# LimpBunion22/VIT-FPGA

Measured on AMD Instinct MI355X. Metric: images/sec ViT-B/16 224x224, batch 512 per GPU, higher is better.
Workload: dtype bf16; 1 GPU; vit_base 224x224x3 inference, 512 images per GPU resident in HBM, random-init weights (seed 0); global_batch=512, per_gpu_batch=512

## Files before the change

### include/vithip.h

```cpp
#ifndef VITHIP_H
#define VITHIP_H

#include <stddef.h>
#include <stdint.h>

#ifdef __cplusplus
extern "C" {
#endif

#define VH_ABI_VERSION 1

#define VH_OK 0
#define VH_ERR_INVALID 1
#define VH_ERR_HIP 2
#define VH_ERR_STATE 3
#define VH_ERR_UNSUPPORTED 4
#define VH_ERR_NO_DEVICE 5
#define VH_ERR_RING_FULL 6
#define VH_ERR_RING_EMPTY 7

#define VH_DTYPE_BF16 0
#define VH_DTYPE_FP16 1
#define VH_DTYPE_FP8 2

// ... 158 lines not shown
#define VH_444_BGR VH_444(2, 1, 0, 0, 0)
#define VH_444_RGBA VH_444(0, 1, 2, 1, 0)
#define VH_444_BGRA VH_444(2, 1, 0, 1, 0)
#define VH_444_ARGB VH_444(1, 2, 3, 1, 0)
#define VH_444_ABGR VH_444(3, 2, 1, 1, 0)
#define VH_444_YUV24 VH_444(0, 1, 2, 0, 1)
#define VH_444_VUYA VH_444(2, 1, 0, 1, 1)
#define VH_444_AYUV VH_444(1, 2, 3, 1, 1)
#define VH_444_Y416 VH_444(1, 0, 2, 1, 1)
#define VH_444_AYUV64 VH_444(1, 2, 3, 1, 1)
#define VH_444_Y410 (VH_444(1, 0, 2, 1, 1) | 256)
#define VH_444_V410 (VH_444(1, 0, 2, 1, 1) | 256 | 512)
typedef struct vh_frame_bgra {
    uint64_t offset;
    int32_t height, width, row_stride;
    int32_t layout;
    float box[4];
} vh_frame_bgra;
int vh_forward_frames_bgra(vh_ctx* ctx, const uint8_t* frames_host, size_t nbytes, const vh_frame_bgra* desc, int batch, float* logits_host);
int vh_forward_device_frames_bgra(vh_ctx* ctx, const uint8_t* frames_dev, size_t nbytes, const vh_frame_bgra* desc, int batch, float* logits_dev);
int vh_forward_frames_y410(vh_ctx* ctx, const uint8_t* frames_host, size_t nbytes, const vh_frame_bgra* desc, int batch, float* logits_host);
int vh_forward_device_frames_y410(vh_ctx* ctx, const uint8_t* frames_dev, size_t nbytes, const vh_frame_bgra* desc, int batch, float* logits_dev);
int vh_fill_input_seeded(vh_ctx* ctx, uint64_t seed, int batch, float* in_nhwc_dev);

int vh_ring_create(vh_ctx* ctx, int slots, int batch_per_slot);
int vh_ring_destroy(vh_ctx* ctx);
int vh_ring_free_slots(const vh_ctx* ctx, int* n);
int vh_ring_input(vh_ctx* ctx, float** pinned_in_nhwc);
int vh_ring_submit(vh_ctx* ctx, const float* in_nhwc_host, int batch);
int vh_ring_collect(vh_ctx* ctx, float* logits_host, int* batch);
int vh_ring_create_u8(vh_ctx* ctx, int slots, int batch_per_slot);
int vh_ring_input_u8(vh_ctx* ctx, uint8_t** pinned_in_nhwc);
int vh_ring_submit_u8(vh_ctx* ctx, const uint8_t* in_nhwc_host, int batch);
int vh_ring_create_frames(vh_ctx* ctx, int slots, int batch_per_slot, size_t slot_bytes);
int vh_ring_input_frames(vh_ctx* ctx, uint8_t** pinned, size_t* capacity);
int vh_ring_submit_frames(vh_ctx* ctx, const uint8_t* frames_host, size_t nbytes, const vh_frame* desc, int batch);
int vh_ring_submit_frames_nv12(vh_ctx* ctx, const uint8_t* frames_host, size_t nbytes, const vh_frame_nv12* desc, int batch);
int vh_ring_submit_frames_yuv(vh_ctx* ctx, const uint8_t* frames_host, size_t nbytes, const vh_frame_yuv* desc, int batch);
int vh_ring_submit_frames_p016(vh_ctx* ctx, const uint8_t* frames_host, size_t nbytes, const vh_frame_nv12* desc, int batch);
int vh_ring_submit_frames_yuv16(vh_ctx* ctx, const uint8_t* frames_host, size_t nbytes, const vh_frame_yuv* desc, int batch);
int vh_ring_submit_frames_yuy2(vh_ctx* ctx, const uint8_t* frames_host, size_t nbytes, const vh_frame_yuy2* desc, int batch);
int vh_ring_submit_frames_y210(vh_ctx* ctx, const uint8_t* frames_host, size_t nbytes, const vh_frame_yuy2* desc, int batch);
int vh_ring_submit_frames_bgra(vh_ctx* ctx, const uint8_t* frames_host, size_t nbytes, const vh_frame_bgra* desc, int batch);
int vh_ring_submit_frames_y410(vh_ctx* ctx, const uint8_t* frames_host, size_t nbytes, const vh_frame_bgra* desc, int batch);
int vh_ring_create_tensor(vh_ctx* ctx, int slots, int batch_per_slot, int elem, int layout);
int vh_ring_input_tensor(vh_ctx* ctx, void** pinned, size_t* capacity_bytes);
int vh_ring_submit_tensor(vh_ctx* ctx, const void* in_host, int batch);

int vh_set_graph(vh_ctx* ctx, int enable);
int vh_get_graph(const vh_ctx* ctx, int* enabled, int* cached_graphs);

int vh_set_streams(vh_ctx* ctx, int n);
int vh_get_streams(const vh_ctx* ctx, int* n);

int vh_last_forward_us(const vh_ctx* ctx, int64_t* us);
int vh_last_kernel_ms(vh_ctx* ctx, double* ms);
int vh_profile_forward(vh_ctx* ctx, const float* in_nhwc_dev, int batch, float* logits_dev,
                       double* stage_ms, int n_stage_slots, int* n_stages_written);
const char* vh_stage_name(int stage_index);
int vh_set_stage_timing(vh_ctx* ctx, int stage_index);
int vh_get_stage_timing(vh_ctx* ctx, double* avg_ms, double* min_ms, int* launches);
int vh_set_step_timing(vh_ctx* ctx, int enable);
int vh_get_step_timing(vh_ctx* ctx, double* step_ms, int max_steps, int* steps);

int vh_debug_read(vh_ctx* ctx, int what, float* host_out, size_t n_floats);
int vh_debug_set_layers(vh_ctx* ctx, int n_layers);

#define VH_FEAT_NORM 0
#define VH_FEAT_RAW  1
typedef struct vh_features {
    void* cls;
    void* patch;
    void* mean;
    int32_t elem;
    int32_t norm;
} vh_features;
int vh_features_dims(const vh_ctx* ctx, int* batch, int* tokens, int* patches, int* dim);
int vh_read_features(vh_ctx* ctx, const vh_features* out_host);
int vh_read_features_device(vh_ctx* ctx, const vh_features* out_dev);
int vh_read_features_device_async(vh_ctx* ctx, const vh_features* out_dev);

#define VH_MAX_FEATURE_LAYERS 8
#define VH_FEAT_ROWS 0
#define VH_FEAT_NCHW 1
typedef struct vh_layer_features {
    void* cls;
    void* patch;
    void* mean;
    void* reg;
    int32_t elem;
    int32_t norm;
    int32_t layer;
    int32_t patch_layout;
} vh_layer_features;
int vh_set_feature_layers(vh_ctx* ctx, const int* layers, int n);
int vh_get_feature_layers(const vh_ctx* ctx, int* layers, int* n);
int vh_read_layer_features(vh_ctx* ctx, const vh_layer_features* out_host);
int vh_read_layer_features_device(vh_ctx* ctx, const vh_layer_features* out_dev);
int vh_read_layer_features_device_async(vh_ctx* ctx, const vh_layer_features* out_dev);

#define VH_MAX_ATTENTION_LAYERS 64
#define VH_ATTN_Q_CLS 0
#define VH_ATTN_Q_LEAD 1
#define VH_ATTN_KEYS_ALL 0
#define VH_ATTN_KEYS_PATCH 1
typedef struct vh_attention_maps {
// ... 191 lines not shown
```

### vit-fpga_amd/csrc/vithip_api.hip

```cpp
#include <dlfcn.h>

#include <chrono>
#include <cmath>
#include <condition_variable>
#include <cstdarg>
#include <cstdio>
#include <cstdlib>
#include <cstring>
#include <functional>
#include <memory>
#include <mutex>
#include <string>
#include <thread>
#include <vector>

#include "vh_kernels.h"

using namespace vh;

namespace {

thread_local std::string g_err;

int fail(std::string* ctx_err, int code, const char* fmt, ...) {
// ... 124 lines not shown
    if (c.max_batch <= 0) return "max_batch must be positive";
    if (!(c.ln_eps > 0.f)) return "ln_eps must be positive";
    if (c.flags & ~(VH_FLAG_LN_FOLD_OFF | VH_FLAG_LN_FOLD_ON | VH_FLAG_W8_E4M3 | VH_FLAG_CLS_TAIL | VH_FLAG_PRE_LN | VH_FLAG_QUICK_GELU | VH_FLAG_REGISTERS_MASK |
                    VH_FLAG_NO_CLS | VH_FLAG_POOL_MASK | VH_FLAG_MAP_HEAD | VH_FLAG_TANH_GELU | VH_FLAG_ROPE)) return "unknown bits in flags";
    if ((c.flags & VH_FLAG_ROPE) && (c.flags & VH_FLAG_CLS_TAIL)) return "flags: VH_FLAG_ROPE excludes VH_FLAG_CLS_TAIL (the tail's one-query attention kernel reads unrotated q and k)";
    if ((c.flags & VH_FLAG_TANH_GELU) && (c.flags & VH_FLAG_QUICK_GELU)) return "flags: VH_FLAG_TANH_GELU and VH_FLAG_QUICK_GELU exclude each other (one MLP activation)";
    if (c.flags & VH_FLAG_MAP_HEAD) {
        if (!(c.flags & VH_FLAG_NO_CLS)) return "flags: VH_FLAG_MAP_HEAD needs VH_FLAG_NO_CLS (the head pools the patch rows; its towers have no class token)";
        if (VH_FLAG_POOL_OF(c.flags)) return "flags: VH_FLAG_MAP_HEAD excludes VH_FLAG_POOL (the attention pooling is the head's input)";
        if (VH_FLAG_REGISTERS_OF(c.flags)) return "flags: VH_FLAG_MAP_HEAD excludes VH_FLAG_REGISTERS";
        if (c.flags & VH_FLAG_CLS_TAIL) return "flags: VH_FLAG_MAP_HEAD excludes VH_FLAG_CLS_TAIL (there is no class token)";
        if (c.heads > VH_MAP_MAX_HEADS) return "flags: VH_FLAG_MAP_HEAD takes at most 16 heads";
    }
    const int R = VH_FLAG_REGISTERS_OF(c.flags);
    if (R > VH_MAX_REGISTERS) return "flags: VH_FLAG_REGISTERS takes 0 .. 16 register tokens";
    const int ncls = (c.flags & VH_FLAG_NO_CLS) ? 0 : 1, pool = VH_FLAG_POOL_OF(c.flags);
    if (!ncls && !(c.flags & VH_FLAG_MAP_HEAD) && (pool == VH_POOL_CLS || pool == VH_POOL_CLS_AVG))
        return pool == VH_POOL_CLS ? "flags: VH_FLAG_NO_CLS needs VH_FLAG_POOL(VH_POOL_AVG_NORM) or VH_FLAG_POOL(VH_POOL_AVG_FCNORM): VH_POOL_CLS reads the class token"
                                   : "flags: VH_FLAG_NO_CLS excludes VH_POOL_CLS_AVG: its first half is the class token";
    if ((c.flags & VH_FLAG_CLS_TAIL) && !ncls) return "flags: VH_FLAG_CLS_TAIL excludes VH_FLAG_NO_CLS (its last layer computes the class-token rows only)";
    if ((c.flags & VH_FLAG_CLS_TAIL) && pool != VH_POOL_CLS) return "flags: VH_FLAG_CLS_TAIL excludes VH_FLAG_POOL (its last layer does not update the patch rows)";
    if ((c.flags & VH_FLAG_W8_E4M3) && c.dtype == VH_DTYPE_FP8) return "flags: VH_FLAG_W8_E4M3 is for the 16-bit dtypes (VH_DTYPE_FP8 quantises both operands)";
    if ((c.flags & VH_FLAG_W8_E4M3) && (c.dim % 4 || c.mlp_dim % 4)) return "flags: VH_FLAG_W8_E4M3 needs dim and mlp_dim multiples of 4";
    if ((c.flags & VH_FLAG_LN_FOLD_OFF) && (c.flags & VH_FLAG_LN_FOLD_ON)) return "flags: VH_FLAG_LN_FOLD_OFF and VH_FLAG_LN_FOLD_ON exclude each other";
    if (c.image_size > 4096 || c.patch_size > 256 || c.channels > 64) return "image_size <= 4096, patch_size <= 256, channels <= 64";
    if (c.layers > 4096 || c.classes > (1 << 20) || c.mlp_dim > (1 << 16) || c.max_batch > (1 << 20)) return "layers <= 4096, classes <= 2^20, mlp_dim <= 2^16, max_batch <= 2^20";
    const int g = c.image_size / c.patch_size;
    if (g > 64) return "tokens <= 4097 (image_size / patch_size <= 64)";
    if (g * g + ncls + R > 4097)
        return ncls ? "tokens <= 4097: a 64 x 64 patch grid + the class token leaves no room for register tokens"
                    : "tokens <= 4097: a 64 x 64 patch grid without a class token leaves room for one register token";
    if ((int64_t)c.max_batch * (g * g + ncls + R) > (640ll << 20)) return "max_batch x tokens <= 640 x 2^20";
    return nullptr;
}

enum Stage { ST_IM2COL, ST_PATCH, ST_CLS, ST_LN, ST_QKV, ST_ATTN, ST_PROJ, ST_FC1, ST_FC2, ST_LNF, ST_HEAD, ST_LNSTATS, ST_PRELN, ST_RESIZE, ST_COUNT };
constexpr int kProfiledStages = ST_RESIZE;
const char* kStageNames[ST_COUNT] = {"im2col", "patch_gemm", "cls_rows", "layernorm", "qkv_gemm", "attention",
                                     "proj_gemm", "fc1_gemm", "fc2_gemm", "final_layernorm", "head_gemm", "ln_stats", "pre_layernorm", "resize"};

}

struct ImgIn {
    const void* p;
    int kind = VH_ELEM_F32;
    int layout = VH_LAYOUT_NHWC;
    bool u8() const { return kind == VH_ELEM_U8; }
    bool nhwc_f32() const { return kind == VH_ELEM_F32 && layout == VH_LAYOUT_NHWC; }
    size_t elem() const { return kind == VH_ELEM_F32 ? 4 : kind == VH_ELEM_U8 ? 1 : 2; }
    ImgIn skip(size_t elements) const { return ImgIn{(const char*)p + elements * elem(), kind, layout}; }
    bool operator==(const ImgIn& o) const { return p == o.p && kind == o.kind && layout == o.layout; }
};
constexpr int kU8 = VH_ELEM_U8;

struct vh_ctx {
    vh_config cfg;
    int device;
    Layout L;
    hipStream_t stream = nullptr;
    static constexpr int kMaxStreams = 4;
    hipStream_t xstream[kMaxStreams - 1] = {nullptr, nullptr, nullptr};
    hipEvent_t ev_fork = nullptr, ev_join[kMaxStreams - 1] = {nullptr, nullptr, nullptr};
    int nstreams = 1;
    hipEvent_t ev0 = nullptr, ev1 = nullptr;
    bool weights_ready = false;
    int run_layers = -1;
    char* blob = nullptr;
    float* params = nullptr;
    char* w16 = nullptr;
    void* wp16 = nullptr;
    std::vector<void*> wqkv16, wo16, w1_16, w2_16;
    std::vector<void*> w2t_16, wot_16;
    bool h_tiled = false;
    bool att_tiled = true;
    bool qkv_hm = true;
    bool weights_ready_tiled = false;
    float* bqkv = nullptr;
    bool fp8 = false;
    int dt16 = VH_DTYPE_BF16;
    std::vector<float*> sqkv, so, s1, s2;
    bool ln_fold = false;
    float* fold_cd = nullptr;
    float* stats = nullptr;
    float* partials = nullptr;
    bool split = false;
    bool cls_tail = false;
    int head_dim = 64;
    float q_scale = kAttnQScale;
    void* xlo16 = nullptr;
    bool ln_fold_cfg = false, split_cfg = false;
    unsigned int* guard_dev = nullptr;
    float* guard_host = nullptr;
    float guard_thresh = 0.5f;
    bool guard_auto = false, guard_tripped = false;
    char* arena = nullptr;
    unsigned int* tickets = nullptr;
    float* x = nullptr;
    void* xn16 = nullptr;
    void* qkv16 = nullptr;
    void* att16 = nullptr;
    void* h16 = nullptr;
    void* col16 = nullptr;
    float* clsn32 = nullptr;
    float* pool32 = nullptr;
    float* mapz32 = nullptr;
    float* maph32 = nullptr;
    float* mapa32 = nullptr;
    float* in_dev = nullptr;
    float in_scale[kMaxChannels], in_shift[kMaxChannels];
    float* logits_dev = nullptr;
    uint8_t* rz_u8 = nullptr;
    uint32_t *rz_plan_dev = nullptr, *rz_plan_host = nullptr;
    size_t rz_plan_dev_cap = 0, rz_plan_host_cap = 0;
    uint8_t* rz_frames = nullptr;
    size_t rz_frames_cap = 0;
    std::vector<uint32_t> rz_words;
    struct FrameColour { float m[12]; int site = VH_CHROMA_LEFT; };
    FrameColour colour[2];
    int64_t last_us = 0;
    bool timed = false;
    int last_batch = 0;
    int feat_layers[VH_MAX_FEATURE_LAYERS] = {0}, feat_n = 0;
    char* feat_store = nullptr;
    size_t feat_slot = 0;
    int cap_layers[VH_MAX_FEATURE_LAYERS] = {0}, cap_n = 0, cap_nl = -1, cap_form = VH_FEAT_FORM_F32;
    int attn_layers[VH_MAX_ATTENTION_LAYERS] = {0}, attn_n = 0, attn_q = 0, attn_mode = VH_ATTN_Q_CLS;
    char* attn_store = nullptr;
    size_t attn_slot = 0;
    int acap_layers[VH_MAX_ATTENTION_LAYERS] = {0}, acap_n = 0, acap_nl = -1;
    struct RingSlot {
        float *h_in = nullptr, *h_out = nullptr, *d_in = nullptr, *d_out = nullptr;
        hipEvent_t in_done = nullptr, fwd_done = nullptr, out_done = nullptr;
        int batch = 0;
        uint32_t* h_plan = nullptr;
        size_t plan_cap = 0;
    };
    std::vector<RingSlot> ring;
    enum RingKind { RING_F32, RING_U8, RING_FRAMES, RING_TENSOR };
    RingKind ring_kind = RING_F32;
    int ring_elem = VH_ELEM_F32, ring_layout = VH_LAYOUT_NHWC;
    size_t ring_slot_bytes = 0;
    hipStream_t copy_in = nullptr, copy_out = nullptr;
    int ring_batch = 0, ring_wr = 0, ring_rd = 0, ring_used = 0;
    bool last_h_tiled = false;
    bool last_qkv_hm = false;
    int num_cu = 256;
    bool use_graph = false;
    struct GraphEntry { ImgIn in; float* out; int batch; hipGraph_t graph; hipGraphExec_t exec; };
    std::vector<GraphEntry> graphs;
    std::vector<int> graph_warm;
    int timing_stage = -1;
    std::vector<hipEvent_t> tev;
    size_t tev_used = 0;
    bool step_timing = false;
    std::vector<hipEvent_t> sev;
    size_t sev_used = 0;
    std::string err;
};

struct vh_filter {
// ... 65 lines not shown
        const size_t dd = (size_t)D * D;
        HIPCHK(&c->err, launch_quantize_rows(P + o.qw, D, D, c->q_scale, wq, c->sqkv[l], s));
        HIPCHK(&c->err, launch_quantize_rows(P + o.kw, D, D, 1.0f, wq + dd, c->sqkv[l] + D, s));
        HIPCHK(&c->err, launch_quantize_rows(P + o.vw, D, D, 1.0f, wq + 2 * dd, c->sqkv[l] + 2 * D, s));
        HIPCHK(&c->err, launch_quantize_rows(P + o.ow, D, D, 1.0f, c->wo16[l], c->so[l], s));
        HIPCHK(&c->err, launch_quantize_rows(P + o.f1w, M, D, 1.0f, c->w1_16[l], c->s1[l], s));
        HIPCHK(&c->err, launch_quantize_rows(P + o.f2w, D, M, 1.0f, c->w2_16[l], c->s2[l], s));
    }
    float* w8tmp = nullptr;
    struct FreeOnExit { float*& p; ~FreeOnExit() { if (p) { hipFree(p); p = nullptr; } } } w8tmp_guard{w8tmp};
    const size_t dd1 = (size_t)D * D, md1 = (size_t)M * D;
    if (!c->fp8 && (f.flags & VH_FLAG_W8_E4M3)) { HIPCHK(&c->err, hipMalloc((void**)&w8tmp, (4 * dd1 + 2 * md1) * sizeof(float))); }
    for (int l = 0; l < f.layers && !c->fp8; ++l) {
        LayerOff o = L.layer[l];
        const float* P = c->params;
        if (w8tmp) {
            const size_t src[6] = {o.qw, o.kw, o.vw, o.ow, o.f1w, o.f2w};
            const int rows[6] = {D, D, D, D, M, D}, cols[6] = {D, D, D, D, D, M};
            size_t at = 0;
            for (int i = 0; i < 6; ++i) {
                HIPCHK(&c->err, launch_fake_quant_rows(c->params + src[i], rows[i], cols[i], w8tmp + at, s));
                at += (size_t)rows[i] * cols[i];
            }
            P = w8tmp;
            o.qw = 0; o.kw = dd1; o.vw = 2 * dd1; o.ow = 3 * dd1; o.f1w = 4 * dd1; o.f2w = 4 * dd1 + md1;
        }
        const float* B = c->params;
        if (c->ln_fold) {
            float* cd = c->fold_cd + (size_t)l * (6 * D + 2 * M);
            char* wq = (char*)c->wqkv16[l];
            const size_t dd2 = (size_t)D * D * 2;
            HIPCHK(&c->err, launch_fold_ln(P + o.qw, B + o.qb, B + o.ln1w, B + o.ln1b, D, D, c->q_scale, wq, cd, cd + 3 * D, f.dtype, s));
            HIPCHK(&c->err, launch_fold_ln(P + o.kw, B + o.kb, B + o.ln1w, B + o.ln1b, D, D, 1.0f, wq + dd2, cd + D, cd + 4 * D, f.dtype, s));
            HIPCHK(&c->err, launch_fold_ln(P + o.vw, B + o.vb, B + o.ln1w, B + o.ln1b, D, D, 1.0f, wq + 2 * dd2, cd + 2 * D, cd + 5 * D, f.dtype, s));
            HIPCHK(&c->err, launch_fold_ln(P + o.f1w, B + o.f1b, B + o.ln2w, B + o.ln2b, M, D, 1.0f, c->w1_16[l], cd + 6 * D, cd + 6 * D + M, f.dtype, s));
        } else {
            HIPCHK(&c->err, launch_pack_qkv(P + o.qw, B + o.qb, P + o.kw, B + o.kb, P + o.vw, B + o.vb, D, c->q_scale,
                                            c->wqkv16[l], c->bqkv + (size_t)l * 3 * D, f.dtype, s));
            HIPCHK(&c->err, launch_cast(P + o.f1w, c->w1_16[l], (int64_t)M * D, f.dtype, s));
        }
        HIPCHK(&c->err, launch_cast(P + o.ow, c->wo16[l], (int64_t)D * D, f.dtype, s));
        HIPCHK(&c->err, launch_cast(P + o.f2w, c->w2_16[l], (int64_t)D * M, f.dtype, s));
        if (c->h_tiled && c->w2t_16[l]) HIPCHK(&c->err, launch_cast_tiled_w(P + o.f2w, D, M, c->w2t_16[l], f.dtype, s));
        if (c->h_tiled && c->wot_16[l]) HIPCHK(&c->err, launch_cast_tiled_w(P + o.ow, D, D, c->wot_16[l], f.dtype, s));
        if (w8tmp) { HIPCHK(&c->err, hipStreamSynchronize(s)); }
    }
    HIPCHK(&c->err, hipStreamSynchronize(s));
    c->weights_ready = true;
    c->weights_ready_tiled = c->h_tiled && (!c->fp8 || c->ln_fold);
    return VH_OK;
}

void drop_graphs(vh_ctx* c);
int guard_reset(vh_ctx* c) {
    HIPCHK(&c->err, hipStreamSynchronize(c->stream));
    HIPCHK(&c->err, hipMemsetAsync(c->guard_dev, 0, 2 * sizeof(unsigned int), c->stream));
    c->guard_host[0] = c->guard_host[1] = 0.f;
    c->guard_tripped = false;
    c->ln_fold = c->ln_fold_cfg;
    c->split = c->split_cfg;
    drop_graphs(c);
    return VH_OK;
}

int check_blob_header(vh_ctx* c, const BlobHeader& h) {
    const vh_config& f = c->cfg;
    if (memcmp(h.magic, "VHBLOB1", 8) != 0) return fail(&c->err, VH_ERR_INVALID, "weight blob: bad magic");
    if (h.image_size != f.image_size || h.patch_size != f.patch_size || h.channels != f.channels || h.dim != f.dim ||
        h.heads != f.heads || h.mlp_dim != f.mlp_dim || h.layers != f.layers || h.classes != f.classes)
        return fail(&c->err, VH_ERR_INVALID, "weight blob: shape differs from the context's vh_config");
    const uint32_t want = blob_model_bits(f);
    if ((h.flags ^ want) & kBlobPreLn)
        return fail(&c->err, VH_ERR_INVALID, "weight blob: header bit 1 (pre-LayerNorm) is %d, the context's VH_FLAG_PRE_LN is %d",
                    (h.flags & kBlobPreLn) != 0, (want & kBlobPreLn) != 0);
    if ((h.flags ^ want) & kBlobQuickGelu)
        return fail(&c->err, VH_ERR_INVALID, "weight blob: header bit 2 (QuickGELU) is %d, the context's VH_FLAG_QUICK_GELU is %d",
                    (h.flags & kBlobQuickGelu) != 0, (want & kBlobQuickGelu) != 0);
    if ((h.flags ^ want) & kBlobRegisters)
        return fail(&c->err, VH_ERR_INVALID, "weight blob: header bits 9..13 say %d register tokens, the context's VH_FLAG_REGISTERS says %d",
                    (int)VH_FLAG_REGISTERS_OF(h.flags), (int)VH_FLAG_REGISTERS_OF(want));
    if ((h.flags ^ want) & kBlobNoCls)
        return fail(&c->err, VH_ERR_INVALID, "weight blob: header bit 15 (no class token) is %d, the context's VH_FLAG_NO_CLS is %d",
                    (h.flags & kBlobNoCls) != 0, (want & kBlobNoCls) != 0);
    if ((h.flags ^ want) & kBlobPool)
        return fail(&c->err, VH_ERR_INVALID, "weight blob: header bits 16..17 say pooling mode %d, the context's VH_FLAG_POOL says %d",
                    (int)VH_FLAG_POOL_OF(h.flags), (int)VH_FLAG_POOL_OF(want));
    if ((h.flags ^ want) & kBlobMapHead)
        return fail(&c->err, VH_ERR_INVALID, "weight blob: header bit 19 (attention-pooling head) is %d, the context's VH_FLAG_MAP_HEAD is %d",
                    (h.flags & kBlobMapHead) != 0, (want & kBlobMapHead) != 0);
    if ((h.flags ^ want) & kBlobTanhGelu)
        return fail(&c->err, VH_ERR_INVALID, "weight blob: header bit 21 (tanh GELU) is %d, the context's VH_FLAG_TANH_GELU is %d",
                    (h.flags & kBlobTanhGelu) != 0, (want & kBlobTanhGelu) != 0);
    if ((h.flags ^ want) & kBlobRope)
        return fail(&c->err, VH_ERR_INVALID, "weight blob: header bit 23 (rotary position embedding) is %d, the context's VH_FLAG_ROPE is %d",
                    (h.flags & kBlobRope) != 0, (want & kBlobRope) != 0);
    return VH_OK;
}

int enqueue_forward(vh_ctx* c, ImgIn in, int batch, float* logits, std::vector<std::pair<int, hipEvent_t>>* ev,
                    hipStream_t s, int img0, bool may_pad = true) {
    const vh_config& f = c->cfg;
    const Layout& L = c->L;
    const int D = f.dim, M = f.mlp_dim, T = L.T;
    const int64_t rows = (int64_t)batch * T;
    const int64_t row_tiles = (rows + 255) / 256;
    const int64_t rows_g = (may_pad && c->ln_fold && row_tiles * ((D + 255) / 256) >= 2 * (int64_t)c->num_cu) ? row_tiles * 256 : rows;
    const float* P = c->params;
    const size_t r0 = (size_t)img0 * T, esz = 2, esz_op = c->fp8 ? 1 : 2;
    const int dt16 = c->dt16;
    float* const x = c->x + r0 * D;
    float* const stats_p = c->stats + r0 * 2;
    float* const partials_p = c->partials + (size_t)(D / 64) * r0 * 2;
    char* const xn16 = (char*)c->xn16 + r0 * D * esz_op;
    char* const xlo16 = (char*)c->xlo16 + r0 * D * (c->fp8 ? 2 : 1);
    char* const qkv16 = (char*)c->qkv16 + r0 * 3 * D * esz;
    char* const att16 = (char*)c->att16 + r0 * D * esz_op;
    char* const h16 = (char*)c->h16 + r0 * M * esz_op;
    char* const col16 = (char*)c->col16 + (size_t)img0 * L.NP * L.KPA * esz;
    float* const clsn32 = c->clsn32 + (size_t)img0 * L.HW;
    float* const pool32 = c->pool32 + (size_t)img0 * D;
    const float* const cls_p = L.ncls ? P + L.cls : nullptr;
    const float* const pos_p = P + L.pos - (L.ncls ? 0 : D);
    unsigned int* const tickets_part = c->tickets + (size_t)img0 * (f.layers > 0 ? f.layers : 1);
    if (f.layers > 0) HIPCHK(&c->err, hipMemsetAsync(tickets_part, 0, sizeof(unsigned int) * f.layers, s));
    unsigned int* const amax_guard = c->fp8 ? c->guard_dev + 1 : nullptr;
    auto mark = [&](int stage) -> int {
        if (!ev) return VH_OK;
        hipEvent_t e;
        HIPCHK(&c->err, hipEventCreate(&e));
        HIPCHK(&c->err, hipEventRecord(e, s));
        ev->push_back({stage, e});
        return VH_OK;
    };
    auto tmark = [&](int stage) -> int {
        if (stage != c->timing_stage) return VH_OK;
        if (c->tev_used == c->tev.size()) {
            hipEvent_t e;
            HIPCHK(&c->err, hipEventCreate(&e));
            c->tev.push_back(e);
        }
        HIPCHK(&c->err, hipEventRecord(c->tev[c->tev_used++], s));
        return VH_OK;
    };
    const int op_dt = c->fp8 ? VH_DTYPE_FP8 : dt16;
    auto gemm_args = [&](int dtype, const void* a, const void* w, const float* bias, void* out, int64_t Mr, int N, int K, int epi,
                         const float* aux = nullptr, int aux_i = 0) {
        GemmArgs g{a, w, bias, out, Mr, N, K, epi, aux, aux_i, dtype, 0};
        g.stats = stats_p;
        g.partials = partials_p;
        return g;
    };
    auto set_tiled = [](GemmArgs& g, bool out_tiled, bool ab_tiled) {
        g.out_tiled = out_tiled;
        g.ab_tiled = ab_tiled;
        if (out_tiled || ab_tiled) g.variant = 6;
    };
    auto stage = [&](int st, auto&& launch) -> int {
        int r;
        if ((r = tmark(st))) return r;
        HIPCHK(&c->err, launch());
        if ((r = tmark(st))) return r;
        return mark(st);
    };
    int rc;
    if ((rc = mark(-1))) return rc;
    const int nl = (c->run_layers < 0 || c->run_layers > f.layers) ? f.layers : c->run_layers;
    const int cap_form = c->split ? (c->fp8 ? VH_DTYPE_FP8 : dt16) : VH_FEAT_FORM_F32;
    c->cap_nl = nl;
    c->cap_form = cap_form;
    c->cap_n = c->feat_n;
    for (int i = 0; i < c->cap_n; ++i) c->cap_layers[i] = c->feat_layers[i];
    auto capture = [&](int l) -> int {
        if (!c->feat_store || l + 1 >= nl) return VH_OK;
        for (int i = 0; i < c->feat_n; ++i) {
            if (c->feat_layers[i] != l + 1) continue;
            char* const slot = c->feat_store + (size_t)i * c->feat_slot;
// ... 62 lines not shown
            if ((rc = stage(ST_PRELN, [&] {
                     return launch_pre_layernorm(x, fold0 ? rows_g : rows, D, P + L.prew, P + L.preb, f.ln_eps, fold0 && c->split ? nullptr : x,
                                                 fold0 ? xn16 : nullptr, fold0 && c->split ? xlo16 : nullptr, fold0 ? stats_p : nullptr, op_dt, s,
                                                 rows, fold0 ? c->guard_dev : nullptr, fold0 ? amax_guard : nullptr);
                 })))
                return rc;
        } else if (c->ln_fold && nl > 0) {
            if (c->split) HIPCHK(&c->err, launch_rowstats_split(x, rows_g, D, f.ln_eps, xn16, xlo16, stats_p, op_dt, s, rows, amax_guard));
            else HIPCHK(&c->err, launch_rowstats_cast(x, rows_g, D, f.ln_eps, xn16, stats_p, op_dt, s, rows, amax_guard));
            HIPCHK(&c->err, launch_ln_guard(stats_p, rows, c->guard_dev, s));
            if ((rc = mark(ST_LNSTATS))) return rc;
        }
    }
    const bool hd64 = c->head_dim == 64;
    const bool tail = c->cls_tail && hd64 && c->ln_fold && c->split && !c->fp8 && nl == f.layers && c->run_layers < 0 && T <= 1024 &&
                      (size_t)L.NP * L.KPA * esz >= 2 * ((size_t)D * esz + 256);
    const bool h_tiled = c->h_tiled && c->split && c->weights_ready_tiled && gemm_tiled_applies(rows_g, M, D, op_dt) && gemm_tiled_applies(rows_g, D, M, op_dt);
    const bool att_tiled = hd64 && h_tiled && c->att_tiled && gemm_tiled_applies(rows_g, D, D, op_dt) && attention_tiled_applies(batch, T, f.heads) && !tail;
    const bool qkv_hm = c->qkv_hm && att_tiled && gemm_tiled_applies(rows_g, 3 * D, D, op_dt);
    c->last_h_tiled = h_tiled && nl > 0 && c->ln_fold;
    c->last_qkv_hm = qkv_hm && nl > 0 && c->ln_fold;
    for (int l = 0; l < nl && c->ln_fold; ++l) {
        const LayerOff& o = L.layer[l];
        const float* cd = c->fold_cd + (size_t)l * (6 * D + 2 * M);
        const int nblk = D / 64;
        const float *sq = c->fp8 ? c->sqkv[l] : nullptr, *so = c->fp8 ? c->so[l] : nullptr;
        const float *s1 = c->fp8 ? c->s1[l] : nullptr, *s2 = c->fp8 ? c->s2[l] : nullptr;
        GemmArgs gq = gemm_args(op_dt, xn16, c->wqkv16[l], cd + 3 * D, qkv16, rows_g, 3 * D, D, VH_EPI_LNFOLD, cd);
        gq.wscale = sq;
        set_tiled(gq, qkv_hm, false);
        if ((rc = stage(ST_QKV, [&] { return launch_gemm(gq, s); }))) return rc;
        if ((rc = rope(qkv_hm ? (int64_t)rows_g : 0))) return rc;
        if ((rc = capture_attention(l, qkv_hm ? (int64_t)rows_g : 0))) return rc;
        if (tail && l + 1 == nl) {
            char* const hc = col16;
            char* const lc = col16 + (((size_t)batch * D * esz + 255) & ~(size_t)255);
            HIPCHK(&c->err, launch_attention_cls(qkv16, batch, T, f.heads, att16, dt16, s));
            if ((rc = mark(ST_ATTN))) return rc;
            HIPCHK(&c->err, hipMemcpy2DAsync(hc, (size_t)D * esz, xn16, (size_t)T * D * esz, (size_t)D * esz, batch, hipMemcpyDeviceToDevice, s));
            HIPCHK(&c->err, hipMemcpy2DAsync(lc, (size_t)D, xlo16, (size_t)T * D, (size_t)D, batch, hipMemcpyDeviceToDevice, s));
            GemmArgs gp = gemm_args(op_dt, att16, c->wo16[l], P + o.ob, hc, batch, D, D, VH_EPI_RESID_SPLIT);
            gp.out16 = lc;
            HIPCHK(&c->err, launch_gemm(gp, s));
            if ((rc = mark(ST_PROJ))) return rc;
            HIPCHK(&c->err, launch_finalize_stats(partials_p, nblk, batch, D, f.ln_eps, stats_p, s, batch, c->guard_dev));
            if ((rc = mark(ST_LNSTATS))) return rc;
            const GemmArgs g1 = gemm_args(op_dt, hc, c->w1_16[l], cd + 6 * D + M, h16, batch, M, D, epi_fc1, cd + 6 * D);
            HIPCHK(&c->err, launch_gemm(g1, s));
            if ((rc = mark(ST_FC1))) return rc;
            GemmArgs g2 = gemm_args(op_dt, h16, c->w2_16[l], P + o.f2b, hc, batch, D, M, VH_EPI_RESID_SPLIT);
            g2.out16 = lc;
            HIPCHK(&c->err, launch_gemm(g2, s));
            if ((rc = mark(ST_FC2))) return rc;
            HIPCHK(&c->err, launch_layernorm_split(hc, lc, batch, D, D, P + L.lnfw, P + L.lnfb, f.ln_eps, clsn32, dt16, s));
            if ((rc = mark(ST_LNF))) return rc;
            HIPCHK(&c->err, launch_head_f32(clsn32, P + L.headw, P + L.headb, logits, batch, f.classes, D, s));
            if ((rc = mark(ST_HEAD))) return rc;
            c->last_batch = batch;
            return VH_OK;
        }
        if ((rc = stage(ST_ATTN, [&] {
                 return hd64 ? launch_attention(qkv16, batch, T, f.heads, att16, op_dt, tickets_part + l, s, true, att_tiled, qkv_hm ? (int64_t)rows_g : 0)
                             : launch_attention_hd(qkv16, batch, T, f.heads, c->head_dim, att16, op_dt, s);
             })))
            return rc;
        GemmArgs go = gemm_args(op_dt, att16, att_tiled ? c->wot_16[l] : c->wo16[l], P + o.ob, c->split ? (void*)xn16 : x, rows_g, D, D,
                                c->split ? VH_EPI_RESID_SPLIT : VH_EPI_RESID_LN);
        go.out16 = c->split ? xlo16 : xn16;
        go.wscale = so;
        set_tiled(go, false, att_tiled);
        if ((rc = stage(ST_PROJ, [&] { return launch_gemm(go, s); }))) return rc;
        HIPCHK(&c->err, launch_finalize_stats(partials_p, nblk, rows_g, D, f.ln_eps, stats_p, s, rows, c->guard_dev, amax_guard));
        if ((rc = mark(ST_LNSTATS))) return rc;
        GemmArgs g1 = gemm_args(op_dt, xn16, c->w1_16[l], cd + 6 * D + M, h16, rows_g, M, D, epi_fc1, cd + 6 * D);
        g1.wscale = s1;
        set_tiled(g1, h_tiled, false);
        if ((rc = stage(ST_FC1, [&] { return launch_gemm(g1, s); }))) return rc;
        GemmArgs g2 = gemm_args(op_dt, h16, h_tiled ? c->w2t_16[l] : c->w2_16[l], P + o.f2b, c->split ? (void*)xn16 : x, rows_g, D, M,
                                c->split ? VH_EPI_RESID_SPLIT : (l + 1 < nl ? VH_EPI_RESID_LN : VH_EPI_BIAS_RESID));
        g2.out16 = c->split ? xlo16 : xn16;
        g2.wscale = s2;
        set_tiled(g2, false, h_tiled);
        if ((rc = stage(ST_FC2, [&] { return launch_gemm(g2, s); }))) return rc;
        if ((rc = capture(l))) return rc;
        if (l + 1 < nl) {
            HIPCHK(&c->err, launch_finalize_stats(partials_p, nblk, rows_g, D, f.ln_eps, stats_p, s, rows, c->guard_dev, amax_guard));
            if ((rc = mark(ST_LNSTATS))) return rc;
        }
    }
    const bool plain = !c->ln_fold;
    auto ln_rows = [&](const float* w, const float* b) { return launch_layernorm(x, rows, D, D, w, b, f.ln_eps, xn16, op_dt, s); };
    auto resid_gemm_ln = [&](const void* a, const void* w, const float* bias, const float* scale, int K, const float* lnw,
                             const float* lnb, int st_gemm) -> int {
        GemmArgs g = gemm_args(op_dt, a, w, bias, x, rows, D, K, VH_EPI_BIAS_RESID);
        g.wscale = scale;
        if (int r = stage(st_gemm, [&] { return launch_gemm(g, s); })) return r;
        return lnw ? stage(ST_LN, [&] { return ln_rows(lnw, lnb); }) : VH_OK;
    };
    if (plain && nl > 0) {
        const LayerOff& o0 = L.layer[0];
        if ((rc = stage(ST_LN, [&] { return ln_rows(P + o0.ln1w, P + o0.ln1b); }))) return rc;
    }
    for (int l = 0; l < nl && plain; ++l) {
        const LayerOff& o = L.layer[l];
        const float *sq = c->fp8 ? c->sqkv[l] : nullptr, *so = c->fp8 ? c->so[l] : nullptr;
        const float *s1 = c->fp8 ? c->s1[l] : nullptr, *s2 = c->fp8 ? c->s2[l] : nullptr;
        GemmArgs gq = gemm_args(op_dt, xn16, c->wqkv16[l], c->bqkv + (size_t)l * 3 * D, qkv16, rows, 3 * D, D, VH_EPI_BIAS);
        gq.wscale = sq;
        if ((rc = stage(ST_QKV, [&] { return launch_gemm(gq, s); }))) return rc;
        if ((rc = rope(0))) return rc;
        if ((rc = capture_attention(l, 0))) return rc;
        if ((rc = stage(ST_ATTN, [&] {
                 return hd64 ? launch_attention(qkv16, batch, T, f.heads, att16, op_dt, tickets_part + l, s, true)
                             : launch_attention_hd(qkv16, batch, T, f.heads, c->head_dim, att16, op_dt, s);
             })))
            return rc;
        if ((rc = resid_gemm_ln(att16, c->wo16[l], P + o.ob, so, D, P + o.ln2w, P + o.ln2b, ST_PROJ))) return rc;
        GemmArgs g1 = gemm_args(op_dt, xn16, c->w1_16[l], P + o.f1b, h16, rows, M, D, epi_fc1_plain);
        g1.wscale = s1;
        if ((rc = stage(ST_FC1, [&] { return launch_gemm(g1, s); }))) return rc;
        const bool more = l + 1 < nl;
        if ((rc = resid_gemm_ln(h16, c->w2_16[l], P + o.f2b, s2, M, more ? P + L.layer[l + 1].ln1w : nullptr,
                                more ? P + L.layer[l + 1].ln1b : nullptr, ST_FC2))) return rc;
        if ((rc = capture(l))) return rc;
    }
    const bool planes = c->split && nl > 0;
    if (L.map) {
        const int H = f.heads, hd = D / H;
        float* const z = c->mapz32 + (size_t)img0 * H * D;
        float* const hid = c->maph32 + (size_t)img0 * (M > D ? M : D);
        float* const a32 = c->mapa32 + (size_t)img0 * D;
        float* const o32 = c->mapa32 + ((size_t)f.max_batch + img0) * D;
        float* const lnrow = z;
        const PoolArgs pa{planes ? (const void*)xn16 : (const void*)x, planes ? xlo16 : nullptr, planes ? (c->fp8 ? VH_DTYPE_FP8 : dt16) : VH_FEAT_FORM_F32,
                          batch, T, L.lead, D, P + L.lnfw, P + L.lnfb, f.ln_eps, VH_FEAT_NORM, z};
        HIPCHK(&c->err, launch_map_pool(pa, P + L.map_qk, H, s));
        HIPCHK(&c->err, launch_head_f32_groups(z, (int64_t)H * D, D, P + L.map_vw, P + L.map_vb, a32, D, nullptr, batch, hd, D, H, s));
        HIPCHK(&c->err, launch_head_f32(a32, P + L.map_ow, P + L.map_ob, o32, batch, D, D, s));
        HIPCHK(&c->err, launch_layernorm(o32, batch, D, D, P + L.map_lnw, P + L.map_lnb, f.ln_eps, lnrow, VH_DTYPE_F32_INTERNAL, s));
        HIPCHK(&c->err, launch_head_f32(lnrow, P + L.map_f1w, P + L.map_f1b, hid, batch, M, D, s));
        HIPCHK(&c->err, launch_act_f32(hid, (int64_t)batch * M, quick ? 1 : tanh_gelu ? 2 : 0, s));
        HIPCHK(&c->err, launch_head_f32_groups(hid, M, 0, P + L.map_f2w, P + L.map_f2b, clsn32, D, o32, batch, D, M, 1, s));
    } else if (L.pool == VH_POOL_CLS || L.pool == VH_POOL_CLS_AVG) {
        float* const cls_ln = L.pool == VH_POOL_CLS ? clsn32 : pool32;
        if (planes)
            HIPCHK(&c->err, launch_layernorm_split(xn16, xlo16, batch, D, (int64_t)T * D, P + L.lnfw, P + L.lnfb, f.ln_eps, cls_ln, c->fp8 ? VH_DTYPE_FP8 : dt16, s));
        else
            HIPCHK(&c->err, launch_layernorm(x, batch, D, (int64_t)T * D, P + L.lnfw, P + L.lnfb, f.ln_eps, cls_ln, VH_DTYPE_F32_INTERNAL, s));
    }
    if (!L.map && L.pool != VH_POOL_CLS) {
        PoolArgs pa{planes ? (const void*)xn16 : (const void*)x, planes ? xlo16 : nullptr, planes ? (c->fp8 ? VH_DTYPE_FP8 : dt16) : VH_FEAT_FORM_F32,
                    batch, T, L.lead, D, P + L.lnfw, P + L.lnfb, f.ln_eps, L.pool == VH_POOL_AVG_FCNORM ? VH_FEAT_RAW : VH_FEAT_NORM, clsn32};
        if (L.pool == VH_POOL_CLS_AVG) { pa.out = clsn32 + D; pa.out_stride = 2 * D; pa.cls_in = pool32; pa.cls_out = clsn32; }
        if (L.pool == VH_POOL_AVG_FCNORM) pa.out = pool32;
        HIPCHK(&c->err, launch_pool_rows(pa, s));
        if (L.pool == VH_POOL_AVG_FCNORM)
            HIPCHK(&c->err, launch_layernorm(pool32, batch, D, D, P + L.lnfw, P + L.lnfb, f.ln_eps, clsn32, VH_DTYPE_F32_INTERNAL, s));
    }
    if ((rc = mark(ST_LNF))) return rc;
    HIPCHK(&c->err, launch_head_f32(clsn32, P + L.headw, P + L.headb, logits, batch, f.classes, L.HW, s));
    if ((rc = mark(ST_HEAD))) return rc;
    c->last_batch = batch;
    return VH_OK;
}

int guard_publish(vh_ctx* c) {
    if (c->ln_fold) HIPCHK(&c->err, hipMemcpyAsync(c->guard_host, c->guard_dev, 2 * sizeof(float), hipMemcpyDeviceToHost, c->stream));
    return VH_OK;
}
constexpr float kE4M3Max = 448.f;
bool guard_exceeded(const vh_ctx* c) {
    if (!c->ln_fold || !c->guard_host) return false;
    const volatile float* g = c->guard_host;
    return !(g[0] <= c->guard_thresh) || (c->fp8 && !(g[1] <= kE4M3Max));
}
int prepare_weights(vh_ctx* c);
void drop_graphs(vh_ctx* c);
int guard_poll(vh_ctx* c) {
    if (!guard_exceeded(c)) return VH_OK;
    c->guard_tripped = true;
    if (!c->guard_auto) return VH_OK;
    c->ln_fold = false;
    c->split = false;
    drop_graphs(c);
    return prepare_weights(c);
}

int enqueue_step(vh_ctx* c, ImgIn in, int batch, float* logits) {
    const size_t img_elems = (size_t)c->cfg.image_size * c->cfg.image_size * c->cfg.channels;
    const int parts = batch < c->nstreams ? batch : c->nstreams;
    int rc;
    if (parts > 1) {
        HIPCHK(&c->err, hipEventRecord(c->ev_fork, c->stream));
        int b0 = 0;
        for (int p = 0; p < parts; ++p) {
            const int nb = batch / parts + (p < batch % parts ? 1 : 0);
            hipStream_t st = p == 0 ? c->stream : c->xstream[p - 1];
            if (p) HIPCHK(&c->err, hipStreamWaitEvent(st, c->ev_fork, 0));
            if ((rc = enqueue_forward(c, in.skip((size_t)b0 * img_elems), nb, logits + (size_t)b0 * c->cfg.classes, nullptr, st, b0,
                                       p == parts - 1))) return rc;
            if (p) {
                HIPCHK(&c->err, hipEventRecord(c->ev_join[p - 1], st));
                HIPCHK(&c->err, hipStreamWaitEvent(c->stream, c->ev_join[p - 1], 0));
            }
            b0 += nb;
        }
        c->last_batch = batch;
        return guard_publish(c);
    }
    if ((rc = enqueue_forward(c, in, batch, logits, nullptr, c->stream, 0))) return rc;
    return guard_publish(c);
}

void drop_graphs(vh_ctx* c) {
    for (auto& g : c->graphs) {
        if (g.exec) hipGraphExecDestroy(g.exec);
        if (g.graph) hipGraphDestroy(g.graph);
    }
    c->graphs.clear();
}

int run_step(vh_ctx* c, ImgIn in, int batch, float* logits) {
    if (int rc = guard_poll(c)) return rc;
    if (!c->use_graph || c->timing_stage >= 0) return enqueue_step(c, in, batch, logits);
    for (auto& g : c->graphs)
        if (g.in == in && g.out == logits && g.batch == batch) {
            HIPCHK(&c->err, hipGraphLaunch(g.exec, c->stream));
            c->last_batch = batch;
            return VH_OK;
        }
    bool warm = false;
    for (int b : c->graph_warm) warm |= b == batch;
    if (!warm) {
        c->graph_warm.push_back(batch);
        return enqueue_step(c, in, batch, logits);
    }
    if (c->graphs.size() >= 128) drop_graphs(c);
    vh_ctx::GraphEntry g{in, logits, batch, nullptr, nullptr};
    HIPCHK(&c->err, hipStreamBeginCapture(c->stream, hipStreamCaptureModeThreadLocal));
    const int rc = enqueue_step(c, in, batch, logits);
    const hipError_t e = hipStreamEndCapture(c->stream, &g.graph);
    if (rc) { if (g.graph) hipGraphDestroy(g.graph); return rc; }
    if (e != hipSuccess) return fail(&c->err, VH_ERR_HIP, "hipStreamEndCapture: %s", hipGetErrorString(e));
    const hipError_t ei = hipGraphInstantiate(&g.exec, g.graph, nullptr, nullptr, 0);
    if (ei != hipSuccess) { hipGraphDestroy(g.graph); return fail(&c->err, VH_ERR_HIP, "hipGraphInstantiate: %s", hipGetErrorString(ei)); }
    c->graphs.push_back(g);
    HIPCHK(&c->err, hipGraphLaunch(g.exec, c->stream));
    c->last_batch = batch;
    return VH_OK;
}

int guard_calibrate(vh_ctx* c) {
    if (!c->guard_auto || !c->ln_fold) return VH_OK;
    const vh_config& f = c->cfg;
    const int64_t n = (int64_t)f.image_size * f.image_size * f.channels;
    HIPCHK(&c->err, launch_fill(c->in_dev, n, 0xCA11B8A7Eull, TID_IMAGES, 0, 0.f, 0.f, c->stream));
    const int keep_stage = c->timing_stage;
    c->timing_stage = -1;
    const int rc = enqueue_step(c, ImgIn{c->in_dev}, 1, c->logits_dev);
    c->timing_stage = keep_stage;
    if (rc) return rc;
    HIPCHK(&c->err, hipStreamSynchronize(c->stream));
    return guard_poll(c);
}

int check_forward_args(vh_ctx* c, const void* in, int batch, const void* out) {
    if (!c) return fail(nullptr, VH_ERR_INVALID, "null context");
    if (!in || !out) return fail(&c->err, VH_ERR_INVALID, "null buffer");
    if (batch <= 0 || batch > c->cfg.max_batch)
        return fail(&c->err, VH_ERR_INVALID, "batch %d outside 1..max_batch=%d", batch, c->cfg.max_batch);
    if (!c->weights_ready) return fail(&c->err, VH_ERR_STATE, "forward before weights were loaded");
    return VH_OK;
}

int check_tensor_kind(std::string* err, int elem, int layout) {
    if (elem < VH_ELEM_F32 || elem > VH_ELEM_U8) return fail(err, VH_ERR_INVALID, "unknown elem %d (VH_ELEM_F32 .. VH_ELEM_U8 = 0..3)", elem);
    if (layout != VH_LAYOUT_NHWC && layout != VH_LAYOUT_NCHW) return fail(err, VH_ERR_INVALID, "unknown layout %d (VH_LAYOUT_NHWC = 0, VH_LAYOUT_NCHW = 1)", layout);
    return VH_OK;
}

int check_tensor_ptr(vh_ctx* c, const void* in_dev) {
    if ((uintptr_t)in_dev & 15) return fail(c ? &c->err : nullptr, VH_ERR_INVALID, "tensor device input %p is not 16-byte aligned", in_dev);
    return VH_OK;
}

int check_u8_ptr(vh_ctx* c, const void* in_dev) {
    if (c && ((uintptr_t)in_dev & 15)) return fail(&c->err, VH_ERR_INVALID, "8-bit device input %p is not 16-byte aligned", in_dev);
    return VH_OK;
}

struct FrameFormat {
    const char* tag;
    const char* label;
    const char* op_null;
    bool three_channels;
    int colour;
    const char* (*plan)(const void* desc, int batch, int channels, int S, size_t nbytes, uintptr_t base, int chroma_site,
                        std::vector<uint32_t>* words, int* max_tiles);
    hipError_t (*launch)(const uint8_t* frames, const uint32_t* plan_dev, int batch, int channels, int S, int max_tiles, const float* m12,
                         uint8_t* out, hipStream_t stream);
};

template <int SAMPLE_BYTES>
const char* plan_semi_planar(const void* desc, int batch, int, int S, size_t nbytes, uintptr_t base, int chroma_site, std::vector<uint32_t>* words,
                             int* max_tiles) {
    return resize_plan_build_nv12((const vh_frame_nv12*)desc, batch, S, nbytes, (unsigned)(base & 3), chroma_site, SAMPLE_BYTES, words, max_tiles);
}
template <int SAMPLE_BYTES>
const char* plan_planar(const void* desc, int batch, int, int S, size_t nbytes, uintptr_t base, int chroma_site, std::vector<uint32_t>* words,
                        int* max_tiles) {
    return resize_plan_build_yuv((const vh_frame_yuv*)desc, batch, S, nbytes, (base & 1) == 0, chroma_site, SAMPLE_BYTES, words, max_tiles);
}
template <bool PLANAR, bool WIDE>
hipError_t launch_yuv(const uint8_t* frames, const uint32_t* plan_dev, int batch, int, int S, int max_tiles, const float* m12, uint8_t* out,
                      hipStream_t stream) {
    return launch_resize_yuv_any(PLANAR, WIDE, frames, plan_dev, batch, S, max_tiles, m12, out, stream);
// ... 10 lines not shown
    return launch_resize_yuy2(WIDE, frames, plan_dev, batch, S, max_tiles, m12, out, stream);
}

template <int SAMPLE_BYTES>
const char* plan_packed444(const void* desc, int batch, int, int S, size_t nbytes, uintptr_t base, int, std::vector<uint32_t>* words, int* max_tiles) {
    return resize_plan_build_bgra((const vh_frame_bgra*)desc, batch, S, nbytes, (unsigned)(base & 7), SAMPLE_BYTES, words, max_tiles);
}
template <bool WIDE>
hipError_t launch_packed444(const uint8_t* frames, const uint32_t* plan_dev, int batch, int, int S, int max_tiles, const float* m12, uint8_t* out,
                            hipStream_t stream) {
    return launch_resize_bgra(WIDE, frames, plan_dev, batch, S, max_tiles, m12, out, stream);
}

const char* plan_rgb(const void* desc, int batch, int channels, int S, size_t nbytes, uintptr_t base, int, std::vector<uint32_t>* words, int* max_tiles) {
    return resize_plan_build((const vh_frame*)desc, batch, channels, S, nbytes, (base & 3) == 0, words, max_tiles);
}
hipError_t launch_rgb(const uint8_t* frames, const uint32_t* plan_dev, int batch, int channels, int S, int max_tiles, const float*, uint8_t* out,
                      hipStream_t stream) {
    return launch_resize_u8(frames, plan_dev, batch, channels, S, max_tiles, out, stream);
}

const FrameFormat kFramesRGB = {"resize_u8", "", "null buffer", false, -1, plan_rgb, launch_rgb};
const FrameFormat kFramesNV12 = {"resize_nv12", "NV12", "null buffer", true, 0, plan_semi_planar<1>, launch_yuv<false, false>};
const FrameFormat kFramesYUV = {"resize_yuv", "planar YUV", "resize_yuv: null buffer", true, 0, plan_planar<1>, launch_yuv<true, false>};
const FrameFormat kFramesP016 = {"resize_p016", "P016", "resize_p016: null buffer", true, 1, plan_semi_planar<2>, launch_yuv<false, true>};
const FrameFormat kFramesYUV16 = {"resize_yuv16", "planar 16-bit YUV", "resize_yuv16: null buffer", true, 1, plan_planar<2>, launch_yuv<true, true>};
const FrameFormat kFramesYUY2 = {"resize_yuy2", "packed 4:2:2", "resize_yuy2: null buffer", true, 0, plan_packed422<1>, launch_packed422<false>};
const FrameFormat kFramesY210 = {"resize_y210", "packed 16-bit 4:2:2", "resize_y210: null buffer", true, 1, plan_packed422<2>, launch_packed422<true>};
const FrameFormat kFramesBGRA = {"resize_bgra", "packed 4:4:4", "resize_bgra: null buffer", true, 0, plan_packed444<1>, launch_packed444<false>};
const FrameFormat kFramesY410 = {"resize_y410", "packed 16-bit 4:4:4", "resize_y410: null buffer", true, 1, plan_packed444<2>, launch_packed444<true>};

struct FrameJob {
    const FrameFormat& fmt;
    const uint8_t* frames_dev;
    const uint32_t* plan_host;
    size_t words;
    int max_tiles;
};

int frames_plan(vh_ctx* c, const FrameFormat& fmt, const void* desc, int batch, size_t nbytes, uintptr_t base, int* max_tiles) {
    if (!desc) return fail(&c->err, VH_ERR_INVALID, "null frame descriptors");
    if (fmt.three_channels && c->cfg.channels != 3)
        return fail(&c->err, VH_ERR_INVALID, "%s frames need a model with 3 channels, this one has %d", fmt.label, c->cfg.channels);
    const int site = fmt.colour < 0 ? 0 : c->colour[fmt.colour].site;
    const char* why = fmt.plan(desc, batch, c->cfg.channels, c->cfg.image_size, nbytes, base, site, &c->rz_words, max_tiles);
    if (why) return fail(&c->err, VH_ERR_INVALID, "%s", why);
    return VH_OK;
}

int frames_reserve(vh_ctx* c, size_t plan_words, bool host_too, size_t frame_bytes) {
    const vh_config& f = c->cfg;
    if (!c->rz_u8) HIPCHK(&c->err, hipMalloc((void**)&c->rz_u8, (size_t)f.max_batch * f.image_size * f.image_size * f.channels));
    if (plan_words > c->rz_plan_dev_cap) {
        HIPCHK(&c->err, hipStreamSynchronize(c->stream));
        if (c->rz_plan_dev) hipFree(c->rz_plan_dev);
        c->rz_plan_dev = nullptr; c->rz_plan_dev_cap = 0;
        const size_t cap = plan_words * 2 > 16384 ? plan_words * 2 : 16384;
        HIPCHK(&c->err, hipMalloc((void**)&c->rz_plan_dev, cap * 4));
        c->rz_plan_dev_cap = cap;
    }
    if (host_too && plan_words > c->rz_plan_host_cap) {
        HIPCHK(&c->err, hipStreamSynchronize(c->stream));
        if (c->rz_plan_host) hipHostFree(c->rz_plan_host);
        c->rz_plan_host = nullptr; c->rz_plan_host_cap = 0;
        const size_t cap = plan_words * 2 > 16384 ? plan_words * 2 : 16384;
        HIPCHK(&c->err, hipHostMalloc((void**)&c->rz_plan_host, cap * 4, hipHostMallocDefault));
        c->rz_plan_host_cap = cap;
    }
    if (frame_bytes > c->rz_frames_cap) {
        HIPCHK(&c->err, hipStreamSynchronize(c->stream));
        if (c->rz_frames) hipFree(c->rz_frames);
        c->rz_frames = nullptr; c->rz_frames_cap = 0;
        const size_t cap = frame_bytes + frame_bytes / 2;
        HIPCHK(&c->err, hipMalloc((void**)&c->rz_frames, cap));
        c->rz_frames_cap = cap;
    }
    return VH_OK;
}

int enqueue_resize(vh_ctx* c, const FrameJob& j, int batch) {
    auto tmark = [&]() -> int {
        if (c->timing_stage != ST_RESIZE) return VH_OK;
        if (c->tev_used == c->tev.size()) {
            hipEvent_t e;
            HIPCHK(&c->err, hipEventCreate(&e));
            c->tev.push_back(e);
        }
        HIPCHK(&c->err, hipEventRecord(c->tev[c->tev_used++], c->stream));
        return VH_OK;
    };
    int rc;
    HIPCHK(&c->err, hipMemcpyAsync(c->rz_plan_dev, j.plan_host, j.words * 4, hipMemcpyHostToDevice, c->stream));
    if ((rc = tmark())) return rc;
    HIPCHK(&c->err, j.fmt.launch(j.frames_dev, c->rz_plan_dev, batch, c->cfg.channels, c->cfg.image_size, j.max_tiles,
                                 j.fmt.colour < 0 ? nullptr : c->colour[j.fmt.colour].m, c->rz_u8, c->stream));
    return tmark();
}

int forward_device_async(vh_ctx* c, ImgIn in, int batch, float* logits, int steps, const FrameJob* job = nullptr) {
    int rc = check_forward_args(c, in.p, batch, logits);
    if (rc) return rc;
    if (steps <= 0) return fail(&c->err, VH_ERR_INVALID, "steps must be positive");
    HIPCHK(&c->err, hipSetDevice(c->device));
    c->tev_used = 0;
    c->sev_used = 0;
    auto step_mark = [&]() -> int {
        if (!c->step_timing) return VH_OK;
        if (c->sev_used == c->sev.size()) {
            hipEvent_t e;
            HIPCHK(&c->err, hipEventCreate(&e));
            c->sev.push_back(e);
        }
        HIPCHK(&c->err, hipEventRecord(c->sev[c->sev_used++], c->stream));
        return VH_OK;
    };
    HIPCHK(&c->err, hipEventRecord(c->ev0, c->stream));
    if ((rc = step_mark())) return rc;
    if (job && (rc = enqueue_resize(c, *job, batch))) return rc;
    for (int i = 0; i < steps; ++i) {
        if ((rc = run_step(c, in, batch, logits))) return rc;
        if ((rc = step_mark())) return rc;
    }
    HIPCHK(&c->err, hipEventRecord(c->ev1, c->stream));
    c->timed = true;
    return VH_OK;
}

int forward_device(vh_ctx* c, ImgIn in, int batch, float* logits, const FrameJob* job = nullptr) {
    const auto t0 = std::chrono::high_resolution_clock::now();
    int rc = forward_device_async(c, in, batch, logits, 1, job);
    if (rc) return rc;
    rc = vh_synchronize(c);
    if (rc) return rc;
    c->last_us = std::chrono::duration_cast<std::chrono::microseconds>(std::chrono::high_resolution_clock::now() - t0).count();
    return VH_OK;
}

int forward_host(vh_ctx* c, ImgIn in_host, int batch, float* logits_host, const FrameJob* job = nullptr, size_t frame_bytes = 0) {
    int rc = check_forward_args(c, in_host.p, batch, logits_host);
    if (rc) return rc;
    const vh_config& f = c->cfg;
    const auto t0 = std::chrono::high_resolution_clock::now();
    HIPCHK(&c->err, hipSetDevice(c->device));
    const size_t in_bytes = job ? frame_bytes : (size_t)batch * f.image_size * f.image_size * f.channels * in_host.elem();
    const ImgIn staged = job ? ImgIn{c->rz_u8, kU8} : ImgIn{c->in_dev, in_host.kind, in_host.layout};
    HIPCHK(&c->err, hipMemcpyAsync(job ? (void*)c->rz_frames : (void*)c->in_dev, in_host.p, in_bytes, hipMemcpyHostToDevice, c->stream));
    rc = forward_device_async(c, staged, batch, c->logits_dev, 1, job);
    if (rc) return rc;
    HIPCHK(&c->err, hipMemcpyAsync(logits_host, c->logits_dev, (size_t)batch * f.classes * 4, hipMemcpyDeviceToHost, c->stream));
    HIPCHK(&c->err, hipStreamSynchronize(c->stream));
    if (c->guard_auto && guard_exceeded(c)) {
        rc = forward_device_async(c, staged, batch, c->logits_dev, 1);
        if (rc) return rc;
        HIPCHK(&c->err, hipMemcpyAsync(logits_host, c->logits_dev, (size_t)batch * f.classes * 4, hipMemcpyDeviceToHost, c->stream));
        HIPCHK(&c->err, hipStreamSynchronize(c->stream));
    }
    c->last_us = std::chrono::duration_cast<std::chrono::microseconds>(std::chrono::high_resolution_clock::now() - t0).count();
    return VH_OK;
}

}

extern "C" {

int vh_ring_destroy(vh_ctx* c);

int vh_abi_version(void) { return VH_ABI_VERSION; }

int vh_device_count(int* count) {
    if (!count) return fail(nullptr, VH_ERR_INVALID, "null count");
    int n = 0;
    hipError_t e = hipGetDeviceCount(&n);
    if (e != hipSuccess) { *count = 0; return fail(nullptr, VH_ERR_NO_DEVICE, "hipGetDeviceCount: %s", hipGetErrorString(e)); }
    *count = n;
    return VH_OK;
}

const char* vh_last_error(const vh_ctx* ctx) { return ctx ? ctx->err.c_str() : g_err.c_str(); }

int vh_malloc(int device, size_t nbytes, void** p) {
    if (!p || !nbytes) return fail(nullptr, VH_ERR_INVALID, "vh_malloc: bad argument");
    int rc = set_device(nullptr, device);
    if (rc) return rc;
    HIPCHK(nullptr, hipMalloc(p, nbytes));
    return VH_OK;
}
int vh_free(int device, void* p) {
    int rc = set_device(nullptr, device);
    if (rc) return rc;
    HIPCHK(nullptr, hipFree(p));
    return VH_OK;
}
int vh_memcpy_h2d(int device, void* d, const void* h, size_t n) {
    int rc = set_device(nullptr, device);
    if (rc) return rc;
    HIPCHK(nullptr, hipMemcpy(d, h, n, hipMemcpyHostToDevice));
    return VH_OK;
}
int vh_memcpy_d2h(int device, void* h, const void* d, size_t n) {
    int rc = set_device(nullptr, device);
    if (rc) return rc;
    HIPCHK(nullptr, hipMemcpy(h, d, n, hipMemcpyDeviceToHost));
    return VH_OK;
}
int vh_device_mem_info(int device, size_t* free_bytes, size_t* total_bytes) {
    if (!free_bytes || !total_bytes) return fail(nullptr, VH_ERR_INVALID, "null argument");
    int rc = set_device(nullptr, device);
    if (rc) return rc;
    HIPCHK(nullptr, hipMemGetInfo(free_bytes, total_bytes));
    return VH_OK;
}
int vh_device_synchronize(int device) {
    int rc = set_device(nullptr, device);
    if (rc) return rc;
    HIPCHK(nullptr, hipDeviceSynchronize());
    return VH_OK;
}

size_t vh_weight_blob_bytes(const vh_config* cfg) {
    if (!cfg || check_config(*cfg)) return 0;
    return blob_bytes_of(*cfg);
}

int vh_create(const vh_config* cfg, int device, vh_ctx** out) {
    if (!cfg || !out) return fail(nullptr, VH_ERR_INVALID, "vh_create: null argument");
    *out = nullptr;
    if (const char* why = check_config(*cfg)) return fail(nullptr, VH_ERR_INVALID, "vh_create: %s", why);
    int rc = set_device(nullptr, device);
    if (rc) return rc;
    hipDeviceProp_t prop;
    HIPCHK(nullptr, hipGetDeviceProperties(&prop, device));
    if (strncmp(prop.gcnArchName, "gfx950", 6) != 0)
        return fail(nullptr, VH_ERR_NO_DEVICE, "device %d is %s; libvithip is built for gfx950 only", device, prop.gcnArchName);

    vh_ctx* c = nullptr;
    try {
        c = new vh_ctx();
        c->cfg = *cfg;
        c->L = make_layout(*cfg);
    } catch (const std::exception& ex) {
        delete c;
        return fail(nullptr, VH_ERR_INVALID, "vh_create: %s", ex.what());
    }
    c->device = device;
    const Layout& L = c->L;
    const size_t D = cfg->dim, M = cfg->mlp_dim, C = cfg->classes, B = cfg->max_batch;
    const size_t rows = B * (size_t)L.T;
    auto bail = [&](int code) { vh_destroy(c); return code; };
#define CK(expr) do { hipError_t e_ = (expr); if (e_ != hipSuccess) { fail(nullptr, VH_ERR_HIP, "%s failed: %s", #expr, hipGetErrorString(e_)); return bail(VH_ERR_HIP); } } while (0)
    CK(hipStreamCreateWithFlags(&c->stream, hipStreamNonBlocking));
    CK(hipEventCreateWithFlags(&c->ev_fork, hipEventDisableTiming));
    for (int i = 0; i < vh_ctx::kMaxStreams - 1; ++i) {
        CK(hipStreamCreateWithFlags(&c->xstream[i], hipStreamNonBlocking));
        CK(hipEventCreateWithFlags(&c->ev_join[i], hipEventDisableTiming));
    }
    {
        const char* e = getenv("VH_STREAMS");
        c->nstreams = e ? atoi(e) : 1;
        if (c->nstreams < 1) c->nstreams = 1;
        if (c->nstreams > vh_ctx::kMaxStreams) c->nstreams = vh_ctx::kMaxStreams;
    }
    c->num_cu = prop.multiProcessorCount;
    {
        const char* e = getenv("VH_GRAPH");
        c->use_graph = e && e[0] == '1';
    }
    CK(hipEventCreate(&c->ev0));
    CK(hipEventCreate(&c->ev1));
    CK(hipMalloc((void**)&c->blob, sizeof(BlobHeader) + 4 * L.total));
    c->params = (float*)(c->blob + sizeof(BlobHeader));
    size_t w16_bytes = 0;
    auto carve16 = [&](size_t elems) { size_t o = w16_bytes; w16_bytes += align_up(elems * 2, 256); return o; };
    const size_t o_wp = carve16(D * L.KPA);
    std::vector<size_t> o_qkv(cfg->layers), o_o(cfg->layers), o_1(cfg->layers), o_2(cfg->layers), o_2t(cfg->layers);
    const bool want_tiled_any = D % 256 == 0 && M % 256 == 0 && !(getenv("VH_H_TILED") && getenv("VH_H_TILED")[0] == '0');
    const bool want_tiled = cfg->dtype != VH_DTYPE_FP8 && want_tiled_any;
    const bool want_tiled8 = cfg->dtype == VH_DTYPE_FP8 && want_tiled_any;
    for (int l = 0; l < cfg->layers; ++l) {
        o_qkv[l] = carve16(3 * D * D); o_o[l] = carve16(D * D); o_1[l] = carve16(M * D); o_2[l] = carve16(D * M);
        o_2t[l] = want_tiled ? carve16(D * M) : want_tiled8 ? carve16((D * M + 1) / 2) : 0;
    }
    std::vector<size_t> o_ot(cfg->layers);
    for (int l = 0; l < cfg->layers; ++l) o_ot[l] = want_tiled ? carve16(D * D) : want_tiled8 ? carve16((D * D + 1) / 2) : 0;
    const size_t o_bqkv = w16_bytes;
    w16_bytes += align_up((size_t)cfg->layers * 3 * D * 4, 256);
    {
        const bool eligible = (cfg->dim % 256 == 0) && (cfg->mlp_dim % 256 == 0);
        bool want = true;
        if (cfg->flags & VH_FLAG_LN_FOLD_OFF) want = false;
        else if (!(cfg->flags & VH_FLAG_LN_FOLD_ON)) { const char* e = getenv("VH_LN_FOLD"); if (e) want = e[0] == '1'; }
        c->ln_fold = eligible && want;
        c->guard_auto = c->ln_fold && !(cfg->flags & (VH_FLAG_LN_FOLD_ON | VH_FLAG_LN_FOLD_OFF)) && !getenv("VH_LN_FOLD");
        if (const char* e = getenv("VH_LN_GUARD")) { const float t = (float)atof(e); if (t > 0.f) c->guard_thresh = t; }
    }
    c->fp8 = cfg->dtype == VH_DTYPE_FP8;
    c->dt16 = c->fp8 ? VH_DTYPE_BF16 : cfg->dtype;
    for (int i = 0; i < kMaxChannels; ++i) {
        c->in_scale[i] = i < cfg->channels ? 1.0f / 255.0f : 0.f;
        c->in_shift[i] = 0.f;
    }
    yuv_matrix(VH_YUV_BT709, 0, c->colour[0].m);
    yuv_matrix16(VH_YUV_BT709, 0, 10, 1, c->colour[1].m);
    {
        const char* e = getenv("VH_RESID_SPLIT");
        c->split = c->ln_fold && !(e && e[0] == '0');
        c->ln_fold_cfg = c->ln_fold;
        c->split_cfg = c->split;
        c->cls_tail = (cfg->flags & VH_FLAG_CLS_TAIL) != 0;
        c->head_dim = cfg->dim / cfg->heads;
        c->q_scale = attention_q_scale(c->head_dim);
        c->h_tiled = want_tiled || want_tiled8;
        { const char* e = getenv("VH_ATT_TILED"); c->att_tiled = !(e && e[0] == '0'); }
        { const char* e = getenv("VH_QKV_HM"); c->qkv_hm = !(e && e[0] == '0'); }
    }
    CK(hipHostMalloc((void**)&c->guard_host, 64, hipHostMallocDefault));
    *c->guard_host = 0.f;
    const size_t o_cd = w16_bytes;
    w16_bytes += align_up((size_t)cfg->layers * (6 * D + 2 * M) * 4, 256);
    const size_t o_sc = w16_bytes, sc_per_layer = 5 * D + M;
    if (c->fp8) w16_bytes += align_up((size_t)cfg->layers * sc_per_layer * 4, 256);
    CK(hipMalloc((void**)&c->w16, w16_bytes));
    c->wp16 = c->w16 + o_wp; c->bqkv = (float*)(c->w16 + o_bqkv);
    c->fold_cd = (float*)(c->w16 + o_cd);
    for (int l = 0; l < cfg->layers; ++l) {
        c->wqkv16.push_back(c->w16 + o_qkv[l]); c->wo16.push_back(c->w16 + o_o[l]);
        c->w1_16.push_back(c->w16 + o_1[l]); c->w2_16.push_back(c->w16 + o_2[l]);
        c->w2t_16.push_back(want_tiled || want_tiled8 ? c->w16 + o_2t[l] : nullptr);
        c->wot_16.push_back(want_tiled || want_tiled8 ? c->w16 + o_ot[l] : nullptr);
        if (c->fp8) {
            float* sc = (float*)(c->w16 + o_sc) + (size_t)l * sc_per_layer;
            c->sqkv.push_back(sc); c->so.push_back(sc + 3 * D); c->s1.push_back(sc + 4 * D); c->s2.push_back(sc + 4 * D + M);
        }
    }
    size_t a = 0;
    auto carve = [&](size_t bytes) { size_t o = a; a += align_up(bytes, 256); return o; };
    const size_t rows_p = rows + 256;
    const size_t o_x = carve(rows_p * D * 4), o_xn = carve(rows_p * D * 2), o_qkvA = carve(rows_p * 3 * D * 2),
                 o_att = carve(rows_p * D * 2), o_h = carve(rows_p * M * 2), o_col = carve(B * L.NP * (size_t)L.KPA * 2),
                 o_cls = carve(B * 2 * D * 4), o_pool = carve(B * D * 4),
                 o_in = carve(B * (size_t)cfg->image_size * cfg->image_size * cfg->channels * 4), o_lg = carve(B * C * 4),
                 o_st = carve(rows_p * 2 * 4), o_pt = carve((D / 64 + 1) * rows_p * 2 * 4), o_xlo = carve(rows_p * D * 2),
                 o_tk = carve(B * 4 * (size_t)(cfg->layers > 0 ? cfg->layers : 1)),
                 o_gd = carve(256);
    const size_t o_mz = L.map ? carve(B * (size_t)cfg->heads * D * 4) : 0, o_mh = L.map ? carve(B * (M > D ? M : D) * 4) : 0,
                 o_ma = L.map ? carve(B * 2 * D * 4) : 0;
    CK(hipMalloc((void**)&c->arena, a));
    c->guard_dev = (unsigned int*)(c->arena + o_gd);
    CK(hipMemsetAsync(c->guard_dev, 0, 256, c->stream));
    c->x = (float*)(c->arena + o_x); c->xn16 = c->arena + o_xn; c->qkv16 = c->arena + o_qkvA; c->att16 = c->arena + o_att;
    c->h16 = c->arena + o_h; c->col16 = c->arena + o_col; c->clsn32 = (float*)(c->arena + o_cls);
    c->pool32 = (float*)(c->arena + o_pool);
    c->in_dev = (float*)(c->arena + o_in); c->logits_dev = (float*)(c->arena + o_lg);
    c->stats = (float*)(c->arena + o_st); c->partials = (float*)(c->arena + o_pt); c->xlo16 = c->arena + o_xlo;
    c->tickets = (unsigned int*)(c->arena + o_tk);
    if (L.map) { c->mapz32 = (float*)(c->arena + o_mz); c->maph32 = (float*)(c->arena + o_mh); c->mapa32 = (float*)(c->arena + o_ma); }
#undef CK
    *out = c;
    return VH_OK;
}

int vh_destroy(vh_ctx* c) {
    if (!c) return VH_OK;
    hipSetDevice(c->device);
    vh_ring_destroy(c);
    if (c->stream) hipStreamSynchronize(c->stream);
    drop_graphs(c);
    if (c->guard_host) hipHostFree(c->guard_host);
    if (c->rz_plan_host) hipHostFree(c->rz_plan_host);
    if (c->rz_plan_dev) hipFree(c->rz_plan_dev);
    if (c->rz_frames) hipFree(c->rz_frames);
    if (c->rz_u8) hipFree(c->rz_u8);
    if (c->arena) hipFree(c->arena);
    if (c->feat_store) hipFree(c->feat_store);
    if (c->attn_store) hipFree(c->attn_store);
    if (c->w16) hipFree(c->w16);
    if (c->blob) hipFree(c->blob);
    for (hipEvent_t e : c->tev) hipEventDestroy(e);
    for (hipEvent_t e : c->sev) hipEventDestroy(e);
    if (c->ev0) hipEventDestroy(c->ev0);
    if (c->ev1) hipEventDestroy(c->ev1);
    for (int i = 0; i < vh_ctx::kMaxStreams - 1; ++i) {
        if (c->xstream[i]) { hipStreamSynchronize(c->xstream[i]); hipStreamDestroy(c->xstream[i]); }
        if (c->ev_join[i]) hipEventDestroy(c->ev_join[i]);
    }
    if (c->ev_fork) hipEventDestroy(c->ev_fork);
    if (c->stream) hipStreamDestroy(c->stream);
    delete c;
    return VH_OK;
}

int vh_get_config(const vh_ctx* c, vh_config* out) {
    if (!c || !out) return fail(nullptr, VH_ERR_INVALID, "null argument");
    *out = c->cfg;
    return VH_OK;
}

int vh_get_register_tokens(const vh_ctx* c) { return c ? c->L.R : -1; }
int vh_get_ln_fold(const vh_ctx* c, int* on) {
    if (!c || !on) return fail(nullptr, VH_ERR_INVALID, "null argument");
    *on = c->ln_fold ? 1 : 0;
    return VH_OK;
}

int vh_get_ln_guard(vh_ctx* c, float* max_ratio, float* threshold, int* tripped) {
    if (!c) return fail(nullptr, VH_ERR_INVALID, "null context");
    HIPCHK(&c->err, hipSetDevice(c->device));
    HIPCHK(&c->err, hipStreamSynchronize(c->stream));
    float seen[2] = {0.f, 0.f};
    HIPCHK(&c->err, hipMemcpy(seen, c->guard_dev, sizeof seen, hipMemcpyDeviceToHost));
    if ((!(seen[0] <= c->guard_thresh) || (c->fp8 && !(seen[1] <= kE4M3Max))) && c->ln_fold_cfg) c->guard_tripped = true;
    if (max_ratio) *max_ratio = seen[0];
    if (threshold) *threshold = c->guard_thresh;
    if (tripped) *tripped = c->guard_tripped ? 1 : 0;
    return VH_OK;
}

int vh_get_fp8_guard(vh_ctx* c, float* max_abs, float* limit) {
    if (!c) return fail(nullptr, VH_ERR_INVALID, "null context");
    HIPCHK(&c->err, hipSetDevice(c->device));
    HIPCHK(&c->err, hipStreamSynchronize(c->stream));
    float seen[2] = {0.f, 0.f};
    HIPCHK(&c->err, hipMemcpy(seen, c->guard_dev, sizeof seen, hipMemcpyDeviceToHost));
    if (max_abs) *max_abs = c->fp8 ? seen[1] : 0.f;
    if (limit) *limit = kE4M3Max;
    return VH_OK;
}

int vh_load_weights(vh_ctx* c, const void* host_blob, size_t nbytes) {
    if (!c || !host_blob) return fail(c ? &c->err : nullptr, VH_ERR_INVALID, "vh_load_weights: null argument");
    const size_t need = sizeof(BlobHeader) + 4 * c->L.total;
    if (nbytes != need) return fail(&c->err, VH_ERR_INVALID, "weight blob is %zu bytes, expected %zu", nbytes, need);
    BlobHeader h;
    memcpy(&h, host_blob, sizeof h);
    int rc = check_blob_header(c, h);
    if (rc) return rc;
    HIPCHK(&c->err, hipSetDevice(c->device));
    c->weights_ready = false;
    HIPCHK(&c->err, hipMemcpyAsync(c->blob, host_blob, nbytes, hipMemcpyHostToDevice, c->stream));
    if ((rc = guard_reset(c))) return rc;
    if ((rc = prepare_weights(c))) return rc;
    return guard_calibrate(c);
}

int vh_load_weights_device(vh_ctx* c, const void* dev_blob, size_t nbytes) {
    if (!c || !dev_blob) return fail(c ? &c->err : nullptr, VH_ERR_INVALID, "vh_load_weights_device: null argument");
    const size_t need = sizeof(BlobHeader) + 4 * c->L.total;
    if (nbytes != need) return fail(&c->err, VH_ERR_INVALID, "weight blob is %zu bytes, expected %zu", nbytes, need);
    HIPCHK(&c->err, hipSetDevice(c->device));
    BlobHeader h;
    HIPCHK(&c->err, hipMemcpy(&h, dev_blob, sizeof h, hipMemcpyDeviceToHost));
    int rc = check_blob_header(c, h);
    if (rc) return rc;
    c->weights_ready = false;
    if (dev_blob != c->blob) HIPCHK(&c->err, hipMemcpyAsync(c->blob, dev_blob, nbytes, hipMemcpyDeviceToDevice, c->stream));
    if ((rc = guard_reset(c))) return rc;
    if ((rc = prepare_weights(c))) return rc;
    return guard_calibrate(c);
}

int vh_init_weights_seeded(vh_ctx* c, uint64_t seed) {
    if (!c) return fail(nullptr, VH_ERR_INVALID, "null context");
    HIPCHK(&c->err, hipSetDevice(c->device));
    const vh_config& f = c->cfg;
    const Layout& L = c->L;
    BlobHeader h;
    memset(&h, 0, sizeof h);
    memcpy(h.magic, "VHBLOB1", 8);
    h.image_size = f.image_size; h.patch_size = f.patch_size; h.channels = f.channels; h.dim = f.dim;
    h.heads = f.heads; h.mlp_dim = f.mlp_dim; h.layers = f.layers; h.classes = f.classes; h.ln_eps = f.ln_eps;
    h.flags = blob_model_bits(f);
    c->weights_ready = false;
    HIPCHK(&c->err, hipMemcpy(c->blob, &h, sizeof h, hipMemcpyHostToDevice));
    const size_t D = f.dim, M = f.mlp_dim, C = f.classes;
// ... 131 lines not shown
    const size_t put = fwrite(buf.data(), 1, need, f);
    const int bad = fclose(f);
    if (put != need || bad) { remove(tmp.c_str()); return fail(&c->err, VH_ERR_INVALID, "short write to %s", tmp.c_str()); }
    if (rename(tmp.c_str(), path) != 0) { remove(tmp.c_str()); return fail(&c->err, VH_ERR_INVALID, "cannot rename %s to %s", tmp.c_str(), path); }
    return VH_OK;
}

int vh_load_weights_file(vh_ctx* c, const char* path) {
    if (!c || !path) return fail(c ? &c->err : nullptr, VH_ERR_INVALID, "null argument");
    const size_t need = sizeof(BlobHeader) + 4 * c->L.total;
    FILE* f = fopen(path, "rb");
    if (!f) return fail(&c->err, VH_ERR_INVALID, "cannot open %s", path);
    std::vector<char> buf(need + 1);
    const size_t got = fread(buf.data(), 1, need + 1, f);
    fclose(f);
    if (got != need) return fail(&c->err, VH_ERR_INVALID, "%s holds %s%zu bytes, this model's blob is %zu", path, got > need ? "more than " : "", got > need ? need : got, need);
    BlobHeader h;
    memcpy(&h, buf.data(), sizeof h);
    int rc = check_blob_header(c, h);
    if (rc) return rc;
    if (h.flags & kBlobSum) {
        const uint64_t sum = fnv1a64(buf.data() + sizeof h, need - sizeof h);
        if ((uint32_t)sum != h.sum_lo || (uint32_t)(sum >> 32) != h.sum_hi)
            return fail(&c->err, VH_ERR_INVALID, "%s: checksum mismatch (file damaged)", path);
    }
    h.sum_lo = h.sum_hi = 0;
    h.flags &= kBlobModelBits;
    memcpy(buf.data(), &h, sizeof h);
    return vh_load_weights(c, buf.data(), need);
}

int vh_export_weights_device(vh_ctx* c, void* dev_blob, size_t nbytes) {
    if (!c || !dev_blob) return fail(c ? &c->err : nullptr, VH_ERR_INVALID, "null argument");
    if (!c->weights_ready) return fail(&c->err, VH_ERR_STATE, "no weights loaded");
    const size_t need = sizeof(BlobHeader) + 4 * c->L.total;
    if (nbytes != need) return fail(&c->err, VH_ERR_INVALID, "buffer is %zu bytes, blob is %zu", nbytes, need);
    HIPCHK(&c->err, hipSetDevice(c->device));
    HIPCHK(&c->err, hipMemcpy(dev_blob, c->blob, need, hipMemcpyDeviceToDevice));
    return VH_OK;
}

int vh_forward_device_async(vh_ctx* c, const float* in, int batch, float* logits, int steps) {
    return forward_device_async(c, ImgIn{in}, batch, logits, steps);
}

int vh_forward_device_u8_async(vh_ctx* c, const uint8_t* in, int batch, float* logits, int steps) {
    if (int rc = check_u8_ptr(c, in)) return rc;
    return forward_device_async(c, ImgIn{in, kU8}, batch, logits, steps);
}

int vh_synchronize(vh_ctx* c) {
    if (!c) return fail(nullptr, VH_ERR_INVALID, "null context");
    HIPCHK(&c->err, hipSetDevice(c->device));
    HIPCHK(&c->err, hipStreamSynchronize(c->stream));
    if (c->weights_ready) return guard_poll(c);
    return VH_OK;
}

int vh_forward_device(vh_ctx* c, const float* in, int batch, float* logits) { return forward_device(c, ImgIn{in}, batch, logits); }

int vh_forward_device_u8(vh_ctx* c, const uint8_t* in, int batch, float* logits) {
    if (int rc = check_u8_ptr(c, in)) return rc;
    return forward_device(c, ImgIn{in, kU8}, batch, logits);
}

int vh_forward(vh_ctx* c, const float* in_host, int batch, float* logits_host) { return forward_host(c, ImgIn{in_host}, batch, logits_host); }

int vh_forward_u8(vh_ctx* c, const uint8_t* in_host, int batch, float* logits_host) { return forward_host(c, ImgIn{in_host, kU8}, batch, logits_host); }

int vh_forward_device_tensor_async(vh_ctx* c, const void* in, int elem, int layout, int batch, float* logits, int steps) {
    if (int rc = check_tensor_kind(c ? &c->err : nullptr, elem, layout)) return rc;
    if (int rc = check_tensor_ptr(c, in)) return rc;
    return forward_device_async(c, ImgIn{in, elem, layout}, batch, logits, steps);
}
int vh_forward_device_tensor(vh_ctx* c, const void* in, int elem, int layout, int batch, float* logits) {
    if (int rc = check_tensor_kind(c ? &c->err : nullptr, elem, layout)) return rc;
    if (int rc = check_tensor_ptr(c, in)) return rc;
    return forward_device(c, ImgIn{in, elem, layout}, batch, logits);
}
int vh_forward_tensor(vh_ctx* c, const void* in_host, int elem, int layout, int batch, float* logits_host) {
    if (int rc = check_tensor_kind(c ? &c->err : nullptr, elem, layout)) return rc;
    return forward_host(c, ImgIn{in_host, elem, layout}, batch, logits_host);
}

static int forward_frames_device(vh_ctx* c, const FrameFormat& fmt, const uint8_t* frames_dev, size_t nbytes, const void* desc, int batch,
                                 float* logits_dev) {
    int rc = check_forward_args(c, frames_dev, batch, logits_dev);
    if (rc) return rc;
    int max_tiles = 0;
    if ((rc = frames_plan(c, fmt, desc, batch, nbytes, (uintptr_t)frames_dev, &max_tiles))) return rc;
    HIPCHK(&c->err, hipSetDevice(c->device));
    if ((rc = frames_reserve(c, c->rz_words.size(), true, 0))) return rc;
    memcpy(c->rz_plan_host, c->rz_words.data(), c->rz_words.size() * 4);
    const FrameJob job{fmt, frames_dev, c->rz_plan_host, c->rz_words.size(), max_tiles};
    return forward_device(c, ImgIn{c->rz_u8, kU8}, batch, logits_dev, &job);
}

static int forward_frames_host(vh_ctx* c, const FrameFormat& fmt, const uint8_t* frames_host, size_t nbytes, const void* desc, int batch,
                               float* logits_host) {
    int rc = check_forward_args(c, frames_host, batch, logits_host);
    if (rc) return rc;
    int max_tiles = 0;
    if ((rc = frames_plan(c, fmt, desc, batch, nbytes, 0, &max_tiles))) return rc;
    HIPCHK(&c->err, hipSetDevice(c->device));
    if ((rc = frames_reserve(c, c->rz_words.size(), true, nbytes))) return rc;
    memcpy(c->rz_plan_host, c->rz_words.data(), c->rz_words.size() * 4);
    const FrameJob job{fmt, c->rz_frames, c->rz_plan_host, c->rz_words.size(), max_tiles};
// ... 63 lines not shown

int vh_yuv_matrix16(int standard, int full_range, int bits, int msb_aligned, float m[12]) {
    if (yuv_matrix16(standard, full_range, bits, msb_aligned, m))
        return fail(nullptr, VH_ERR_INVALID, "yuv matrix16: standard must be VH_YUV_BT601, _BT709 or _BT2020, full_range 0 or 1, bits 8..16, msb_aligned 0 or 1, m not NULL");
    return VH_OK;
}

static int set_frame_colour(vh_ctx* c, int which, const float m[12], int chroma_site, const float dflt[12], const char* word) {
    if (!c) return fail(nullptr, VH_ERR_INVALID, "null context");
    if (m) {
        if (chroma_site != VH_CHROMA_CENTER && chroma_site != VH_CHROMA_LEFT) return fail(&c->err, VH_ERR_INVALID, "chroma_site %d is neither VH_CHROMA_CENTER nor VH_CHROMA_LEFT", chroma_site);
        for (int i = 0; i < 12; ++i)
            if (!std::isfinite(m[i])) return fail(&c->err, VH_ERR_INVALID, "%scolour matrix entry %d is not finite", word, i);
    }
    memcpy(c->colour[which].m, m ? m : dflt, sizeof c->colour[which].m);
    c->colour[which].site = m ? chroma_site : VH_CHROMA_LEFT;
    return VH_OK;
}

static int get_frame_colour(const vh_ctx* c, int which, float m[12], int* chroma_site) {
    if (!c) return fail(nullptr, VH_ERR_INVALID, "null context");
    if (m) memcpy(m, c->colour[which].m, sizeof c->colour[which].m);
    if (chroma_site) *chroma_site = c->colour[which].site;
    return VH_OK;
}

int vh_set_frame_colour(vh_ctx* c, const float m[12], int chroma_site) {
    float dflt[12];
    yuv_matrix(VH_YUV_BT709, 0, dflt);
    return set_frame_colour(c, 0, m, chroma_site, dflt, "");
}
int vh_get_frame_colour(const vh_ctx* c, float m[12], int* chroma_site) { return get_frame_colour(c, 0, m, chroma_site); }

int vh_set_frame_colour16(vh_ctx* c, const float m[12], int chroma_site) {
    float dflt[12];
    yuv_matrix16(VH_YUV_BT709, 0, 10, 1, dflt);
    return set_frame_colour(c, 1, m, chroma_site, dflt, "16-bit ");
}
int vh_get_frame_colour16(const vh_ctx* c, float m[12], int* chroma_site) { return get_frame_colour(c, 1, m, chroma_site); }

int vh_resize_table(int n_in, double lo, double hi, int n_out, int32_t* first, int32_t* count, float* weights, int max_taps) {
    if (resize_axis_table(n_in, lo, hi, n_out, first, count, weights, max_taps))
        return fail(nullptr, VH_ERR_INVALID, "resize table: bad argument, box outside 0..n_in or empty, scale > %d, or more than max_taps taps", kResizeMaxScale);
    return VH_OK;
}

int vh_set_input_norm(vh_ctx* c, const float* scale, const float* shift) {
    if (!c) return fail(nullptr, VH_ERR_INVALID, "null context");
    if ((scale == nullptr) != (shift == nullptr)) return fail(&c->err, VH_ERR_INVALID, "scale and shift: give both, or NULL for both (the default)");
    const int ch = c->cfg.channels;
    for (int i = 0; scale && i < ch; ++i)
        if (!std::isfinite(scale[i]) || !std::isfinite(shift[i])) return fail(&c->err, VH_ERR_INVALID, "scale / shift of channel %d is not finite", i);
    HIPCHK(&c->err, hipSetDevice(c->device));
    HIPCHK(&c->err, hipStreamSynchronize(c->stream));
    for (int i = 0; i < kMaxChannels; ++i) {
        c->in_scale[i] = i < ch ? (scale ? scale[i] : 1.0f / 255.0f) : 0.f;
        c->in_shift[i] = i < ch && shift ? shift[i] : 0.f;
    }
    drop_graphs(c);
    return VH_OK;
}

int vh_get_input_norm(const vh_ctx* c, float* scale, float* shift) {
    if (!c || !scale || !shift) return fail(nullptr, VH_ERR_INVALID, "null argument");
    for (int i = 0; i < c->cfg.channels; ++i) { scale[i] = c->in_scale[i]; shift[i] = c->in_shift[i]; }
    return VH_OK;
}

int vh_fill_input_seeded(vh_ctx* c, uint64_t seed, int batch, float* in_dev) {
    if (!c || !in_dev || batch <= 0) return fail(c ? &c->err : nullptr, VH_ERR_INVALID, "bad argument");
    HIPCHK(&c->err, hipSetDevice(c->device));
    const int64_t n = (int64_t)batch * c->cfg.image_size * c->cfg.image_size * c->cfg.channels;
    HIPCHK(&c->err, launch_fill(in_dev, n, seed, TID_IMAGES, 0, 0.f, 0.f, c->stream));
    HIPCHK(&c->err, hipStreamSynchronize(c->stream));
    return VH_OK;
}

int vh_last_forward_us(const vh_ctx* c, int64_t* us) {
    if (!c || !us) return fail(nullptr, VH_ERR_INVALID, "null argument");
    *us = c->last_us;
    return VH_OK;
}

int vh_last_kernel_ms(vh_ctx* c, double* ms) {
    if (!c || !ms) return fail(nullptr, VH_ERR_INVALID, "null argument");
    if (!c->timed) return fail(&c->err, VH_ERR_STATE, "no forward has been enqueued yet");
    HIPCHK(&c->err, hipSetDevice(c->device));
    HIPCHK(&c->err, hipEventSynchronize(c->ev1));
    float t = 0.f;
    HIPCHK(&c->err, hipEventElapsedTime(&t, c->ev0, c->ev1));
    *ms = t;
    return VH_OK;
}

const char* vh_stage_name(int i) { return (i >= 0 && i < ST_COUNT) ? kStageNames[i] : ""; }

int vh_profile_forward(vh_ctx* c, const float* in, int batch, float* logits, double* stage_ms, int n_slots, int* n_written) {
    int rc = check_forward_args(c, in, batch, logits);
    if (rc) return rc;
    if (!stage_ms || n_slots < 2 * kProfiledStages) return fail(&c->err, VH_ERR_INVALID, "need %d stage slots (ms then launch counts)", 2 * kProfiledStages);
    HIPCHK(&c->err, hipSetDevice(c->device));
    std::vector<std::pair<int, hipEvent_t>> ev;
    rc = enqueue_forward(c, ImgIn{in}, batch, logits, &ev, c->stream, 0);
    if (!rc) { hipError_t e = hipStreamSynchronize(c->stream); if (e != hipSuccess) rc = fail(&c->err, VH_ERR_HIP, "sync: %s", hipGetErrorString(e)); }
    for (int i = 0; i < 2 * kProfiledStages; ++i) stage_ms[i] = 0.0;
    if (!rc)
        for (size_t i = 1; i < ev.size(); ++i) {
            float t = 0.f;
            hipEventElapsedTime(&t, ev[i - 1].second, ev[i].second);
            stage_ms[ev[i].first] += t;
            stage_ms[kProfiledStages + ev[i].first] += 1.0;
        }
    for (auto& p : ev) hipEventDestroy(p.second);
    if (n_written) *n_written = kProfiledStages;
    return rc;
}

int vh_ring_destroy(vh_ctx* c) {
    if (!c) return VH_OK;
    if (c->ring.empty() && !c->copy_in) return VH_OK;
    hipSetDevice(c->device);
    if (c->stream) hipStreamSynchronize(c->stream);
    if (c->copy_in) hipStreamSynchronize(c->copy_in);
    if (c->copy_out) hipStreamSynchronize(c->copy_out);
    for (auto& s : c->ring) {
        if (s.h_in) hipHostFree(s.h_in);
        if (s.h_out) hipHostFree(s.h_out);
        if (s.h_plan) hipHostFree(s.h_plan);
        if (s.d_in) hipFree(s.d_in);
        if (s.d_out) hipFree(s.d_out);
        if (s.in_done) hipEventDestroy(s.in_done);
        if (s.fwd_done) hipEventDestroy(s.fwd_done);
        if (s.out_done) hipEventDestroy(s.out_done);
    }
    c->ring.clear();
    if (c->copy_in) hipStreamDestroy(c->copy_in);
    if (c->copy_out) hipStreamDestroy(c->copy_out);
    c->copy_in = c->copy_out = nullptr;
    c->ring_batch = c->ring_wr = c->ring_rd = c->ring_used = 0;
    c->ring_kind = vh_ctx::RING_F32;
    c->ring_elem = VH_ELEM_F32;
    c->ring_layout = VH_LAYOUT_NHWC;
    c->ring_slot_bytes = 0;
    return VH_OK;
}

static const char* ring_kind_name(vh_ctx::RingKind k) {
    return k == vh_ctx::RING_FRAMES ? "8-bit frames" : k == vh_ctx::RING_U8 ? "8-bit images" : k == vh_ctx::RING_TENSOR ? "image tensors" : "fp32 images";
}

static int ring_create(vh_ctx* c, int slots, int batch_per_slot, vh_ctx::RingKind kind, size_t slot_bytes = 0, int elem = VH_ELEM_F32,
                       int layout = VH_LAYOUT_NHWC) {
    if (!c) return fail(nullptr, VH_ERR_INVALID, "null context");
    if (slots < 1 || slots > 64) return fail(&c->err, VH_ERR_INVALID, "slots must be 1..64");
    if (batch_per_slot < 1 || batch_per_slot > c->cfg.max_batch)
        return fail(&c->err, VH_ERR_INVALID, "batch_per_slot %d outside 1..max_batch=%d", batch_per_slot, c->cfg.max_batch);
    const bool frames = kind == vh_ctx::RING_FRAMES;
    if (frames && slot_bytes < 1) return fail(&c->err, VH_ERR_INVALID, "slot_bytes must be positive");
    vh_ring_destroy(c);
    HIPCHK(&c->err, hipSetDevice(c->device));
    const size_t in_bytes = frames ? slot_bytes : (size_t)batch_per_slot * c->cfg.image_size * c->cfg.image_size * c->cfg.channels * ImgIn{nullptr, elem, layout}.elem();
    const size_t plan_words = (size_t)batch_per_slot * kResizeFrameWords + 2 * (size_t)c->cfg.image_size * 10;
    if (frames)
        if (int rc = frames_reserve(c, plan_words, false, 0)) return rc;
    const size_t out_bytes = (size_t)batch_per_slot * c->cfg.classes * 4;
    HIPCHK(&c->err, hipStreamCreateWithFlags(&c->copy_in, hipStreamNonBlocking));
    HIPCHK(&c->err, hipStreamCreateWithFlags(&c->copy_out, hipStreamNonBlocking));
    c->ring.resize(slots);
    for (auto& s : c->ring) {
        hipError_t e = hipHostMalloc((void**)&s.h_in, in_bytes, hipHostMallocDefault);
        if (e == hipSuccess) e = hipHostMalloc((void**)&s.h_out, out_bytes, hipHostMallocDefault);
        if (e == hipSuccess) e = hipMalloc((void**)&s.d_in, in_bytes);
        if (e == hipSuccess) e = hipMalloc((void**)&s.d_out, out_bytes);
        if (e == hipSuccess && frames) {
            e = hipHostMalloc((void**)&s.h_plan, plan_words * 4, hipHostMallocDefault);
            if (e == hipSuccess) s.plan_cap = plan_words;
        }
        if (e == hipSuccess) e = hipEventCreateWithFlags(&s.in_done, hipEventDisableTiming);
        if (e == hipSuccess) e = hipEventCreateWithFlags(&s.fwd_done, hipEventDisableTiming);
        if (e == hipSuccess) e = hipEventCreateWithFlags(&s.out_done, hipEventDisableTiming);
        if (e != hipSuccess) {
            vh_ring_destroy(c);
            return fail(&c->err, VH_ERR_HIP, "vh_ring_create: %s", hipGetErrorString(e));
        }
    }
    c->ring_batch = batch_per_slot;
    c->ring_kind = kind;
    c->ring_elem = elem;
    c->ring_layout = layout;
    c->ring_slot_bytes = frames ? slot_bytes : kind == vh_ctx::RING_TENSOR ? in_bytes : 0;
    return VH_OK;
}

int vh_ring_create(vh_ctx* c, int slots, int batch_per_slot) { return ring_create(c, slots, batch_per_slot, vh_ctx::RING_F32); }
int vh_ring_create_u8(vh_ctx* c, int slots, int batch_per_slot) { return ring_create(c, slots, batch_per_slot, vh_ctx::RING_U8, 0, VH_ELEM_U8); }
int vh_ring_create_tensor(vh_ctx* c, int slots, int batch_per_slot, int elem, int layout) {
    if (!c) return fail(nullptr, VH_ERR_INVALID, "null context");
    if (int rc = check_tensor_kind(&c->err, elem, layout)) return rc;
    return ring_create(c, slots, batch_per_slot, vh_ctx::RING_TENSOR, 0, elem, layout);
}
int vh_ring_create_frames(vh_ctx* c, int slots, int batch_per_slot, size_t slot_bytes) {
    return ring_create(c, slots, batch_per_slot, vh_ctx::RING_FRAMES, slot_bytes);
}

int vh_ring_free_slots(const vh_ctx* c, int* n) {
    if (!c || !n) return fail(nullptr, VH_ERR_INVALID, "null argument");
    *n = (int)c->ring.size() - c->ring_used;
    return VH_OK;
}

static int ring_input(vh_ctx* c, void** pinned_in, vh_ctx::RingKind kind) {
    if (!c || !pinned_in) return fail(c ? &c->err : nullptr, VH_ERR_INVALID, "null argument");
    if (c->ring.empty()) return fail(&c->err, VH_ERR_STATE, "no ring: call vh_ring_create first");
    if (c->ring_kind != kind) return fail(&c->err, VH_ERR_STATE, "this ring stages %s", ring_kind_name(c->ring_kind));
    if (c->ring_used == (int)c->ring.size()) return fail(&c->err, VH_ERR_RING_FULL, "ring full (PILA LLENA)");
    *pinned_in = c->ring[c->ring_wr].h_in;
    return VH_OK;
}

int vh_ring_input(vh_ctx* c, float** pinned_in) { return ring_input(c, (void**)pinned_in, vh_ctx::RING_F32); }
int vh_ring_input_u8(vh_ctx* c, uint8_t** pinned_in) { return ring_input(c, (void**)pinned_in, vh_ctx::RING_U8); }
int vh_ring_input_tensor(vh_ctx* c, void** pinned, size_t* capacity_bytes) {
    if (!capacity_bytes) return fail(c ? &c->err : nullptr, VH_ERR_INVALID, "null argument");
    if (int rc = ring_input(c, pinned, vh_ctx::RING_TENSOR)) return rc;
    *capacity_bytes = c->ring_slot_bytes;
    return VH_OK;
}
int vh_ring_input_frames(vh_ctx* c, uint8_t** pinned, size_t* capacity) {
    if (!capacity) return fail(c ? &c->err : nullptr, VH_ERR_INVALID, "null argument");
    if (int rc = ring_input(c, (void**)pinned, vh_ctx::RING_FRAMES)) return rc;
    *capacity = c->ring_slot_bytes;
    return VH_OK;
}

static int ring_submit(vh_ctx* c, const void* in_host, int batch, vh_ctx::RingKind kind, size_t frame_bytes = 0, const void* desc = nullptr,
                       const FrameFormat& fmt = kFramesRGB) {
    if (!c) return fail(nullptr, VH_ERR_INVALID, "null context");
    if (c->ring.empty()) return fail(&c->err, VH_ERR_STATE, "no ring: call vh_ring_create first");
    if (c->ring_kind != kind) return fail(&c->err, VH_ERR_STATE, "this ring stages %s", ring_kind_name(c->ring_kind));
    if (!c->weights_ready) return fail(&c->err, VH_ERR_STATE, "submit before weights were loaded");
    if (batch < 1 || batch > c->ring_batch) return fail(&c->err, VH_ERR_INVALID, "batch %d outside 1..%d", batch, c->ring_batch);
    if (c->ring_used == (int)c->ring.size()) return fail(&c->err, VH_ERR_RING_FULL, "ring full (PILA LLENA)");
    const bool frames = kind == vh_ctx::RING_FRAMES;
    int rc, max_tiles = 0;
    if (frames) {
        if (frame_bytes < 1 || frame_bytes > c->ring_slot_bytes) return fail(&c->err, VH_ERR_INVALID, "nbytes %zu outside 1..slot_bytes=%zu", frame_bytes, c->ring_slot_bytes);
        if ((rc = frames_plan(c, fmt, desc, batch, frame_bytes, 0, &max_tiles))) return rc;
    }
    HIPCHK(&c->err, hipSetDevice(c->device));
    vh_ctx::RingSlot& s = c->ring[c->ring_wr];
    const ImgIn slot_in{s.d_in, c->ring_elem, c->ring_layout};
    const size_t in_bytes = frames ? frame_bytes : (size_t)batch * c->cfg.image_size * c->cfg.image_size * c->cfg.channels * slot_in.elem();
    if (frames) {
        const size_t words = c->rz_words.size();
        if (words > s.plan_cap) {
            if (s.h_plan) hipHostFree(s.h_plan);
            s.h_plan = nullptr; s.plan_cap = 0;
            HIPCHK(&c->err, hipHostMalloc((void**)&s.h_plan, words * 8, hipHostMallocDefault));
            s.plan_cap = words * 2;
        }
        if ((rc = frames_reserve(c, words, false, 0))) return rc;
        memcpy(s.h_plan, c->rz_words.data(), words * 4);
    }
    if (in_host && in_host != s.h_in) memcpy(s.h_in, in_host, in_bytes);
    s.batch = batch;
    HIPCHK(&c->err, hipMemcpyAsync(s.d_in, s.h_in, in_bytes, hipMemcpyHostToDevice, c->copy_in));
    HIPCHK(&c->err, hipEventRecord(s.in_done, c->copy_in));
    HIPCHK(&c->err, hipStreamWaitEvent(c->stream, s.in_done, 0));
    if (frames) {
        const FrameJob job{fmt, (const uint8_t*)s.d_in, s.h_plan, c->rz_words.size(), max_tiles};
        if ((rc = enqueue_resize(c, job, batch))) return rc;
    }
    rc = run_step(c, frames ? ImgIn{c->rz_u8, kU8} : slot_in, batch, s.d_out);
    if (rc) return rc;
    HIPCHK(&c->err, hipEventRecord(s.fwd_done, c->stream));
    HIPCHK(&c->err, hipStreamWaitEvent(c->copy_out, s.fwd_done, 0));
    HIPCHK(&c->err, hipMemcpyAsync(s.h_out, s.d_out, (size_t)batch * c->cfg.classes * 4, hipMemcpyDeviceToHost, c->copy_out));
    HIPCHK(&c->err, hipEventRecord(s.out_done, c->copy_out));
    c->ring_wr = (c->ring_wr + 1) % (int)c->ring.size();
    ++c->ring_used;
    return VH_OK;
}

int vh_ring_submit(vh_ctx* c, const float* in_host, int batch) { return ring_submit(c, in_host, batch, vh_ctx::RING_F32); }
int vh_ring_submit_u8(vh_ctx* c, const uint8_t* in_host, int batch) { return ring_submit(c, in_host, batch, vh_ctx::RING_U8); }
int vh_ring_submit_tensor(vh_ctx* c, const void* in_host, int batch) { return ring_submit(c, in_host, batch, vh_ctx::RING_TENSOR); }
int vh_ring_submit_frames(vh_ctx* c, const uint8_t* frames_host, size_t nbytes, const vh_frame* desc, int batch) {
    return ring_submit(c, frames_host, batch, vh_ctx::RING_FRAMES, nbytes, desc, kFramesRGB);
}
int vh_ring_submit_frames_nv12(vh_ctx* c, const uint8_t* frames_host, size_t nbytes, const vh_frame_nv12* desc, int batch) {
    return ring_submit(c, frames_host, batch, vh_ctx::RING_FRAMES, nbytes, desc, kFramesNV12);
}
int vh_ring_submit_frames_yuv(vh_ctx* c, const uint8_t* frames_host, size_t nbytes, const vh_frame_yuv* desc, int batch) {
    return ring_submit(c, frames_host, batch, vh_ctx::RING_FRAMES, nbytes, desc, kFramesYUV);
}
int vh_ring_submit_frames_p016(vh_ctx* c, const uint8_t* frames_host, size_t nbytes, const vh_frame_nv12* desc, int batch) {
    return ring_submit(c, frames_host, batch, vh_ctx::RING_FRAMES, nbytes, desc, kFramesP016);
}
int vh_ring_submit_frames_yuv16(vh_ctx* c, const uint8_t* frames_host, size_t nbytes, const vh_frame_yuv* desc, int batch) {
    return ring_submit(c, frames_host, batch, vh_ctx::RING_FRAMES, nbytes, desc, kFramesYUV16);
}
int vh_ring_submit_frames_yuy2(vh_ctx* c, const uint8_t* frames_host, size_t nbytes, const vh_frame_yuy2* desc, int batch) {
    return ring_submit(c, frames_host, batch, vh_ctx::RING_FRAMES, nbytes, desc, kFramesYUY2);
}
int vh_ring_submit_frames_y210(vh_ctx* c, const uint8_t* frames_host, size_t nbytes, const vh_frame_yuy2* desc, int batch) {
    return ring_submit(c, frames_host, batch, vh_ctx::RING_FRAMES, nbytes, desc, kFramesY210);
}
int vh_ring_submit_frames_bgra(vh_ctx* c, const uint8_t* frames_host, size_t nbytes, const vh_frame_bgra* desc, int batch) {
    return ring_submit(c, frames_host, batch, vh_ctx::RING_FRAMES, nbytes, desc, kFramesBGRA);
}
int vh_ring_submit_frames_y410(vh_ctx* c, const uint8_t* frames_host, size_t nbytes, const vh_frame_bgra* desc, int batch) {
    return ring_submit(c, frames_host, batch, vh_ctx::RING_FRAMES, nbytes, desc, kFramesY410);
}

int vh_ring_collect(vh_ctx* c, float* logits_host, int* batch) {
    if (!c || !logits_host) return fail(c ? &c->err : nullptr, VH_ERR_INVALID, "null argument");
    if (c->ring.empty()) return fail(&c->err, VH_ERR_STATE, "no ring: call vh_ring_create first");
    if (c->ring_used == 0) return fail(&c->err, VH_ERR_RING_EMPTY, "ring empty (PILA VACIA)");
    HIPCHK(&c->err, hipSetDevice(c->device));
    vh_ctx::RingSlot& s = c->ring[c->ring_rd];
    HIPCHK(&c->err, hipEventSynchronize(s.out_done));
    memcpy(logits_host, s.h_out, (size_t)s.batch * c->cfg.classes * 4);
    if (batch) *batch = s.batch;
    c->ring_rd = (c->ring_rd + 1) % (int)c->ring.size();
    --c->ring_used;
    return VH_OK;
}

int vh_set_streams(vh_ctx* c, int n) {
    if (!c) return fail(nullptr, VH_ERR_INVALID, "null context");
    if (n < 1 || n > vh_ctx::kMaxStreams) return fail(&c->err, VH_ERR_INVALID, "streams must be 1..%d", vh_ctx::kMaxStreams);
    HIPCHK(&c->err, hipSetDevice(c->device));
    HIPCHK(&c->err, hipStreamSynchronize(c->stream));
    c->nstreams = n;
    drop_graphs(c);
    return VH_OK;
}

int vh_set_graph(vh_ctx* c, int enable) {
    if (!c) return fail(nullptr, VH_ERR_INVALID, "null context");
    HIPCHK(&c->err, hipSetDevice(c->device));
    HIPCHK(&c->err, hipStreamSynchronize(c->stream));
    c->use_graph = enable != 0;
    if (!c->use_graph) drop_graphs(c);
    return VH_OK;
}

int vh_get_graph(const vh_ctx* c, int* enabled, int* cached) {
    if (!c || !enabled) return fail(nullptr, VH_ERR_INVALID, "null argument");
    *enabled = c->use_graph ? 1 : 0;
    if (cached) *cached = (int)c->graphs.size();
    return VH_OK;
}

int vh_get_streams(const vh_ctx* c, int* n) {
    if (!c || !n) return fail(nullptr, VH_ERR_INVALID, "null argument");
    *n = c->nstreams;
    return VH_OK;
}

int vh_set_stage_timing(vh_ctx* c, int stage) {
    if (!c) return fail(nullptr, VH_ERR_INVALID, "null context");
    if (stage < -1 || stage >= ST_COUNT) return fail(&c->err, VH_ERR_INVALID, "unknown stage %d", stage);
    c->timing_stage = stage;
    c->tev_used = 0;
    return VH_OK;
}

int vh_get_stage_timing(vh_ctx* c, double* avg_ms, double* min_ms, int* launches) {
    if (!c || !avg_ms || !launches) return fail(c ? &c->err : nullptr, VH_ERR_INVALID, "null argument");
    HIPCHK(&c->err, hipSetDevice(c->device));
    HIPCHK(&c->err, hipStreamSynchronize(c->stream));
    double sum = 0.0, mn = 1e30;
    int n = 0;
    for (size_t i = 0; i + 1 < c->tev_used; i += 2) {
        float t = 0.f;
        HIPCHK(&c->err, hipEventElapsedTime(&t, c->tev[i], c->tev[i + 1]));
        sum += t; if (t < mn) mn = t; ++n;
    }
    *avg_ms = n ? sum / n : 0.0;
    if (min_ms) *min_ms = n ? mn : 0.0;
    *launches = n;
    return VH_OK;
}

int vh_set_step_timing(vh_ctx* c, int enable) {
    if (!c) return fail(nullptr, VH_ERR_INVALID, "null context");
    c->step_timing = enable != 0;
    c->sev_used = 0;
    return VH_OK;
}

int vh_get_step_timing(vh_ctx* c, double* step_ms, int max_steps, int* steps) {
    if (!c || !steps || (max_steps > 0 && !step_ms)) return fail(c ? &c->err : nullptr, VH_ERR_INVALID, "null argument");
    HIPCHK(&c->err, hipSetDevice(c->device));
    HIPCHK(&c->err, hipStreamSynchronize(c->stream));
    int n = 0;
    for (size_t i = 0; i + 1 < c->sev_used; ++i) {
        float t = 0.f;
        HIPCHK(&c->err, hipEventElapsedTime(&t, c->sev[i], c->sev[i + 1]));
        if (n < max_steps) step_ms[n] = t;
        ++n;
    }
    *steps = n;
    return VH_OK;
}

int vh_debug_read(vh_ctx* c, int what, float* host_out, size_t n_floats) {
    if (!c || !host_out) return fail(c ? &c->err : nullptr, VH_ERR_INVALID, "null argument");
    if (c->last_batch <= 0) return fail(&c->err, VH_ERR_STATE, "no forward has run");
    HIPCHK(&c->err, hipSetDevice(c->device));
    HIPCHK(&c->err, hipStreamSynchronize(c->stream));
    const size_t D = c->cfg.dim;
    if (what == 0) {
        const size_t n = (size_t)c->last_batch * c->L.T * D;
        if (n_floats != n) return fail(&c->err, VH_ERR_INVALID, "expected %zu floats", n);
        const int nl = (c->run_layers < 0 || c->run_layers > c->cfg.layers) ? c->cfg.layers : c->run_layers;
        if (c->split && nl > 0) {
            auto f = [&](uint16_t b, int dt) {
                if (dt == VH_DTYPE_BF16) { uint32_t u = (uint32_t)b << 16; float v; memcpy(&v, &u, 4); return v; }
                _Float16 hv; memcpy(&hv, &b, 2); return (float)hv;
            };
            auto g = [&](uint8_t b) {
                const int e = (b >> 3) & 15, m = b & 7;
                float v = e ? ldexpf(1.f + m / 8.f, e - 7) : ldexpf(m / 8.f, -6);
                return (b & 0x80) ? -v : v;
            };
            if (c->fp8) {
                std::vector<uint8_t> hi(n);
                std::vector<uint16_t> lo(n);
                HIPCHK(&c->err, hipMemcpy(hi.data(), c->xn16, n, hipMemcpyDeviceToHost));
                HIPCHK(&c->err, hipMemcpy(lo.data(), c->xlo16, n * 2, hipMemcpyDeviceToHost));
                for (size_t i = 0; i < n; ++i) host_out[i] = g(hi[i]) + f(lo[i], VH_DTYPE_BF16);
                return VH_OK;
            }
            std::vector<uint16_t> hi(n);
            std::vector<uint8_t> lo(n);
            HIPCHK(&c->err, hipMemcpy(hi.data(), c->xn16, n * 2, hipMemcpyDeviceToHost));
            HIPCHK(&c->err, hipMemcpy(lo.data(), c->xlo16, n, hipMemcpyDeviceToHost));
            const float inv = c->dt16 == VH_DTYPE_BF16 ? 1.f / 32.f : 1.f / 256.f;
            for (size_t i = 0; i < n; ++i) host_out[i] = f(hi[i], c->dt16) + g(lo[i]) * inv;
            return VH_OK;
        }
        HIPCHK(&c->err, hipMemcpy(host_out, c->x, n * 4, hipMemcpyDeviceToHost));
        return VH_OK;
    }
    if (what == 1) {
        const size_t n = (size_t)c->last_batch * c->L.HW;
        if (n_floats != n) return fail(&c->err, VH_ERR_INVALID, "expected %zu floats", n);
        HIPCHK(&c->err, hipMemcpy(host_out, c->clsn32, n * 4, hipMemcpyDeviceToHost));
        return VH_OK;
    }
    if (what == 3) {
        if (n_floats != 1) return fail(&c->err, VH_ERR_INVALID, "expected 1 float");
        host_out[0] = c->last_h_tiled ? 1.f : 0.f;
        return VH_OK;
    }
    if (what == 4) {
        if (n_floats != 1) return fail(&c->err, VH_ERR_INVALID, "expected 1 float");
        host_out[0] = c->last_qkv_hm ? 1.f : 0.f;
        return VH_OK;
    }
    return fail(&c->err, VH_ERR_INVALID, "unknown tap %d", what);
}

int vh_debug_set_layers(vh_ctx* c, int n_layers) {
    if (!c) return fail(nullptr, VH_ERR_INVALID, "null context");
    c->run_layers = n_layers;
    if (c->stream) hipStreamSynchronize(c->stream);
    drop_graphs(c);
    return VH_OK;
}

static int features_check_call(vh_ctx* c, const vh_features* f, bool device) {
    if (!c) return fail(nullptr, VH_ERR_INVALID, "read_features: null context");
    if (!f) return fail(&c->err, VH_ERR_INVALID, "read_features: null descriptor");
    if (!f->cls && !f->patch && !f->mean) return fail(&c->err, VH_ERR_INVALID, "read_features: no output requested (cls, patch and mean are all NULL)");
    if (f->elem != VH_ELEM_F32 && f->elem != VH_ELEM_F16 && f->elem != VH_ELEM_BF16)
        return fail(&c->err, VH_ERR_INVALID, "read_features: elem %d is not VH_ELEM_F32, VH_ELEM_F16 or VH_ELEM_BF16", f->elem);
    if (f->norm != VH_FEAT_NORM && f->norm != VH_FEAT_RAW) return fail(&c->err, VH_ERR_INVALID, "read_features: norm %d is not VH_FEAT_NORM (0) or VH_FEAT_RAW (1)", f->norm);
    if (device && (((uintptr_t)f->cls | (uintptr_t)f->patch | (uintptr_t)f->mean) & 15))
        return fail(&c->err, VH_ERR_INVALID, "read_features: a device output pointer is not 16-byte aligned (cls %p, patch %p, mean %p)", f->cls, f->patch, f->mean);
    if (c->cfg.flags & VH_FLAG_CLS_TAIL)
        return fail(&c->err, VH_ERR_UNSUPPORTED, "read_features: a VH_FLAG_CLS_TAIL context's last layer updates the class-token rows only");
    if (f->cls && !c->L.ncls) return fail(&c->err, VH_ERR_UNSUPPORTED, "read_features: cls on a context without a class token (VH_FLAG_NO_CLS)");
    if (!c->ring.empty()) return fail(&c->err, VH_ERR_STATE, "read_features: a ring exists on this context (its forwards belong to slots); vh_ring_destroy first");
    if (c->last_batch <= 0) return fail(&c->err, VH_ERR_STATE, "read_features: no forward has run");
    return VH_OK;
}
struct FeatSource { const void* hi; const void* lo; int form; bool head_cls; };
static FeatSource features_live(const vh_ctx* c) {
    const vh_config& g = c->cfg;
    const int nl = (c->run_layers < 0 || c->run_layers > g.layers) ? g.layers : c->run_layers;
    const bool planes = c->split && nl > 0;
    return FeatSource{planes ? (const void*)c->xn16 : (const void*)c->x, planes ? c->xlo16 : nullptr,
                      planes ? (c->fp8 ? VH_DTYPE_FP8 : c->dt16) : VH_FEAT_FORM_F32, c->L.pool == VH_POOL_CLS};
}
static int features_enqueue(vh_ctx* c, const vh_layer_features& f, const FeatSource& src, const char* who) {
    const vh_config& g = c->cfg;
    const bool norm = f.norm == VH_FEAT_NORM;
    FeatureArgs a{};
    a.hi = src.hi; a.lo = src.lo; a.form = src.form;
    a.batch = c->last_batch; a.tokens = c->L.T; a.lead = c->L.lead; a.dim = g.dim;
    a.gamma = c->params + c->L.lnfw; a.beta = c->params + c->L.lnfb; a.eps = g.ln_eps;
    a.elem = f.elem; a.norm = f.norm;
    const bool copy_cls = norm && src.head_cls;
    a.cls = copy_cls ? nullptr : f.cls;
    a.patch = f.patch; a.mean = f.mean; a.stats = c->stats;
    a.reg = f.reg; a.patch_layout = f.patch_layout;
    a.no_cls = c->L.ncls ? 0 : 1;
    if (a.cls || a.patch || a.mean || a.reg) {
        if (const char* why = features_check(a)) return fail(&c->err, VH_ERR_INVALID, "%s: %s", who, why);
        HIPCHK(&c->err, launch_token_features(a, c->stream));
    }
    if (copy_cls && f.cls) {
        const int64_t n = (int64_t)c->last_batch * g.dim;
        if (f.elem == VH_ELEM_F32) HIPCHK(&c->err, hipMemcpyAsync(f.cls, c->clsn32, n * 4, hipMemcpyDeviceToDevice, c->stream));
        else HIPCHK(&c->err, launch_cast(c->clsn32, f.cls, n, f.elem == VH_ELEM_BF16 ? VH_DTYPE_BF16 : VH_DTYPE_FP16, c->stream));
    }
    return VH_OK;
}
static int features_read_host(vh_ctx* c, const vh_layer_features& f, const FeatSource& src, const char* who) {
    const size_t es = f.elem == VH_ELEM_F32 ? 4 : 2, D = c->cfg.dim, B = c->last_batch;
    const size_t n_row = B * D * es, n_patch = B * (size_t)c->L.NP * D * es, n_reg = B * (size_t)c->L.R * D * es;
    const size_t cap = ((size_t)c->cfg.max_batch * c->L.T + 256) * 3 * D * 2;
    char* const base = (char*)c->qkv16;
    size_t at = 0;
    auto take = [&](bool want, size_t bytes) -> void* { if (!want) return nullptr; void* p = base + at; at += align_up(bytes, 256); return p; };
    vh_layer_features d = f;
    d.patch = take(f.patch != nullptr, n_patch);
    d.cls = take(f.cls != nullptr, n_row);
    d.mean = take(f.mean != nullptr, n_row);
    d.reg = take(f.reg != nullptr, n_reg);
    if (at > cap) return fail(&c->err, VH_ERR_STATE, "%s: staging needs %zu bytes, the scratch holds %zu", who, at, cap);
    if (int rc = features_enqueue(c, d, src, who)) return rc;
    if (f.patch) HIPCHK(&c->err, hipMemcpyAsync(f.patch, d.patch, n_patch, hipMemcpyDeviceToHost, c->stream));
    if (f.cls) HIPCHK(&c->err, hipMemcpyAsync(f.cls, d.cls, n_row, hipMemcpyDeviceToHost, c->stream));
    if (f.mean) HIPCHK(&c->err, hipMemcpyAsync(f.mean, d.mean, n_row, hipMemcpyDeviceToHost, c->stream));
    if (f.reg) HIPCHK(&c->err, hipMemcpyAsync(f.reg, d.reg, n_reg, hipMemcpyDeviceToHost, c->stream));
    HIPCHK(&c->err, hipStreamSynchronize(c->stream));
    return VH_OK;
}
static vh_layer_features features_final(const vh_features& f) {
    return vh_layer_features{f.cls, f.patch, f.mean, nullptr, f.elem, f.norm, -1, VH_FEAT_ROWS};
}
int vh_features_dims(const vh_ctx* c, int* batch, int* tokens, int* patches, int* dim) {
    if (!c) return fail(nullptr, VH_ERR_INVALID, "features_dims: null context");
    if (batch) *batch = c->last_batch;
    if (tokens) *tokens = c->L.T;
    if (patches) *patches = c->L.NP;
    if (dim) *dim = c->cfg.dim;
    return VH_OK;
}
int vh_read_features_device_async(vh_ctx* c, const vh_features* f) {
    if (int rc = features_check_call(c, f, true)) return rc;
    HIPCHK(&c->err, hipSetDevice(c->device));
    return features_enqueue(c, features_final(*f), features_live(c), "read_features");
}
int vh_read_features_device(vh_ctx* c, const vh_features* f) {
    if (int rc = vh_read_features_device_async(c, f)) return rc;
    HIPCHK(&c->err, hipStreamSynchronize(c->stream));
    return VH_OK;
}
int vh_read_features(vh_ctx* c, const vh_features* f) {
    if (int rc = features_check_call(c, f, false)) return rc;
    HIPCHK(&c->err, hipSetDevice(c->device));
    return features_read_host(c, features_final(*f), features_live(c), "read_features");
}

int vh_set_feature_layers(vh_ctx* c, const int* layers, int n) {
    if (!c) return fail(nullptr, VH_ERR_INVALID, "set_feature_layers: null context");
    if (n < 0 || n > VH_MAX_FEATURE_LAYERS) return fail(&c->err, VH_ERR_INVALID, "set_feature_layers: %d layers, outside 0..%d", n, VH_MAX_FEATURE_LAYERS);
    if (n > 0 && !layers) return fail(&c->err, VH_ERR_INVALID, "set_feature_layers: null list");
    for (int i = 0; i < n; ++i) {
        if (layers[i] < 1 || layers[i] > c->cfg.layers)
            return fail(&c->err, VH_ERR_INVALID, "set_feature_layers: entry %d is layer %d, outside 1..%d", i, layers[i], c->cfg.layers);
        if (i && layers[i] <= layers[i - 1])
            return fail(&c->err, VH_ERR_INVALID, "set_feature_layers: the list must be strictly ascending (entry %d is %d after %d)", i, layers[i], layers[i - 1]);
    }
    if (n > 0 && (c->cfg.flags & VH_FLAG_CLS_TAIL))
        return fail(&c->err, VH_ERR_UNSUPPORTED, "set_feature_layers: a VH_FLAG_CLS_TAIL context's last layer updates the class-token rows only");
    if (!c->ring.empty()) return fail(&c->err, VH_ERR_STATE, "set_feature_layers: a ring exists on this context; vh_ring_destroy first");
    HIPCHK(&c->err, hipSetDevice(c->device));
    HIPCHK(&c->err, hipStreamSynchronize(c->stream));
    int slots = 0;
    for (int i = 0; i < n; ++i) slots += layers[i] < c->cfg.layers;
    const int eb = c->split_cfg && !c->guard_auto ? 3 : 4;
    const size_t slot = align_up((size_t)c->cfg.max_batch * c->L.T * c->cfg.dim * eb, 256);
    char* store = nullptr;
    if (slots) {
        const hipError_t e = hipMalloc((void**)&store, slot * slots);
        if (e != hipSuccess) {
            (void)hipGetLastError();
            return fail(&c->err, VH_ERR_HIP, "set_feature_layers: no room for the capture store (%d layers x %zu bytes): %s; the previous list stays",
                        slots, slot, hipGetErrorString(e));
        }
    }
    drop_graphs(c);
    if (c->feat_store) hipFree(c->feat_store);
    c->feat_store = store;
    c->feat_slot = slot;
    c->feat_n = n;
    for (int i = 0; i < n; ++i) c->feat_layers[i] = layers[i];
    c->cap_n = 0;
    return VH_OK;
}
int vh_get_feature_layers(const vh_ctx* c, int* layers, int* n) {
    if (!c || !n) return fail(nullptr, VH_ERR_INVALID, "get_feature_layers: null argument");
    *n = c->feat_n;
    for (int i = 0; layers && i < c->feat_n; ++i) layers[i] = c->feat_layers[i];
    return VH_OK;
}

static int layer_features_check_call(vh_ctx* c, const vh_layer_features* f, bool device, FeatSource* src) {
    if (!c) return fail(nullptr, VH_ERR_INVALID, "read_layer_features: null context");
    if (!f) return fail(&c->err, VH_ERR_INVALID, "read_layer_features: null descriptor");
    if (!f->cls && !f->patch && !f->mean && !f->reg)
        return fail(&c->err, VH_ERR_INVALID, "read_layer_features: no output requested (cls, patch, mean and reg are all NULL)");
    if (f->elem != VH_ELEM_F32 && f->elem != VH_ELEM_F16 && f->elem != VH_ELEM_BF16)
        return fail(&c->err, VH_ERR_INVALID, "read_layer_features: elem %d is not VH_ELEM_F32, VH_ELEM_F16 or VH_ELEM_BF16", f->elem);
    if (f->norm != VH_FEAT_NORM && f->norm != VH_FEAT_RAW)
        return fail(&c->err, VH_ERR_INVALID, "read_layer_features: norm %d is not VH_FEAT_NORM (0) or VH_FEAT_RAW (1)", f->norm);
    if (f->patch_layout != VH_FEAT_ROWS && f->patch_layout != VH_FEAT_NCHW)
        return fail(&c->err, VH_ERR_INVALID, "read_layer_features: patch_layout %d is not VH_FEAT_ROWS (0) or VH_FEAT_NCHW (1)", f->patch_layout);
    const int layers = c->cfg.layers;
    if (f->layer != -1 && (f->layer < 1 || f->layer > layers))
        return fail(&c->err, VH_ERR_INVALID, "read_layer_features: layer %d is not -1 or 1..%d", f->layer, layers);
    if (device && (((uintptr_t)f->cls | (uintptr_t)f->patch | (uintptr_t)f->mean | (uintptr_t)f->reg) & 15))
        return fail(&c->err, VH_ERR_INVALID, "read_layer_features: a device output pointer is not 16-byte aligned (cls %p, patch %p, mean %p, reg %p)",
                    f->cls, f->patch, f->mean, f->reg);
    if (f->reg && c->L.R == 0) return fail(&c->err, VH_ERR_INVALID, "read_layer_features: reg on a context without register tokens (VH_FLAG_REGISTERS)");
    if (c->cfg.flags & VH_FLAG_CLS_TAIL)
        return fail(&c->err, VH_ERR_UNSUPPORTED, "read_layer_features: a VH_FLAG_CLS_TAIL context's last layer updates the class-token rows only");
    if (f->cls && !c->L.ncls) return fail(&c->err, VH_ERR_UNSUPPORTED, "read_layer_features: cls on a context without a class token (VH_FLAG_NO_CLS)");
    if (!c->ring.empty()) return fail(&c->err, VH_ERR_STATE, "read_layer_features: a ring exists on this context (its forwards belong to slots); vh_ring_destroy first");
    if (c->last_batch <= 0) return fail(&c->err, VH_ERR_STATE, "read_layer_features: no forward has run");
    if (f->layer == -1) { *src = features_live(c); return VH_OK; }
    int slot = -1;
    for (int i = 0; i < c->cap_n; ++i) if (c->cap_layers[i] == f->layer) slot = i;
    if (f->layer < layers && slot < 0)
        return fail(&c->err, VH_ERR_STATE, "read_layer_features: layer %d was not in the list when the last forward was enqueued (vh_set_feature_layers)", f->layer);
    if (f->layer > c->cap_nl)
        return fail(&c->err, VH_ERR_STATE, "read_layer_features: the last forward ran %d layers and did not reach layer %d (vh_debug_set_layers)", c->cap_nl, f->layer);
    if (f->layer == c->cap_nl) {
        *src = features_live(c);
        src->head_cls = src->head_cls && f->layer == layers;
        return VH_OK;
    }
    const char* const base = c->feat_store + (size_t)slot * c->feat_slot;
    const size_t all = (size_t)c->cfg.max_batch * c->L.T * c->cfg.dim;
    if (c->cap_form == VH_FEAT_FORM_F32) *src = FeatSource{base, nullptr, VH_FEAT_FORM_F32, false};
    else *src = FeatSource{base, base + all * (c->cap_form == VH_DTYPE_FP8 ? 1 : 2), c->cap_form, false};
    return VH_OK;
}
int vh_read_layer_features_device_async(vh_ctx* c, const vh_layer_features* f) {
    FeatSource src{};
    if (int rc = layer_features_check_call(c, f, true, &src)) return rc;
    HIPCHK(&c->err, hipSetDevice(c->device));
    return features_enqueue(c, *f, src, "read_layer_features");
}
int vh_read_layer_features_device(vh_ctx* c, const vh_layer_features* f) {
    if (int rc = vh_read_layer_features_device_async(c, f)) return rc;
    HIPCHK(&c->err, hipStreamSynchronize(c->stream));
    return VH_OK;
}
int vh_read_layer_features(vh_ctx* c, const vh_layer_features* f) {
    FeatSource src{};
    if (int rc = layer_features_check_call(c, f, false, &src)) return rc;
    HIPCHK(&c->err, hipSetDevice(c->device));
    return features_read_host(c, *f, src, "read_layer_features");
}

int vh_set_attention_layers(vh_ctx* c, const int* layers, int n, int queries) {
    if (!c) return fail(nullptr, VH_ERR_INVALID, "set_attention_layers: null context");
    if (n < 0 || n > VH_MAX_ATTENTION_LAYERS) return fail(&c->err, VH_ERR_INVALID, "set_attention_layers: %d layers, outside 0..%d", n, VH_MAX_ATTENTION_LAYERS);
    if (n > 0 && !layers) return fail(&c->err, VH_ERR_INVALID, "set_attention_layers: null list");
    for (int i = 0; i < n; ++i) {
        if (layers[i] < 1 || layers[i] > c->cfg.layers)
            return fail(&c->err, VH_ERR_INVALID, "set_attention_layers: entry %d is layer %d, outside 1..%d", i, layers[i], c->cfg.layers);
        if (i && layers[i] <= layers[i - 1])
            return fail(&c->err, VH_ERR_INVALID, "set_attention_layers: the list must be strictly ascending (entry %d is %d after %d)", i, layers[i], layers[i - 1]);
    }
    if (queries != VH_ATTN_Q_CLS && queries != VH_ATTN_Q_LEAD)
        return fail(&c->err, VH_ERR_INVALID, "set_attention_layers: queries %d is not VH_ATTN_Q_CLS (0) or VH_ATTN_Q_LEAD (1)", queries);
    if (n > 0 && queries == VH_ATTN_Q_CLS && !c->L.ncls)
        return fail(&c->err, VH_ERR_INVALID, "set_attention_layers: VH_ATTN_Q_CLS on a context without a class token (VH_FLAG_NO_CLS)");
    if (n > 0 && queries == VH_ATTN_Q_LEAD && c->L.lead < 1)
        return fail(&c->err, VH_ERR_INVALID, "set_attention_layers: VH_ATTN_Q_LEAD on a context without leading rows (no class token, no registers)");
    const int Q = queries == VH_ATTN_Q_CLS ? 1 : c->L.lead;
    if (n > 0 && Q > kAttnMapsMaxQueries)
        return fail(&c->err, VH_ERR_INVALID, "set_attention_layers: %d leading rows, the capture kernel takes at most %d", Q, kAttnMapsMaxQueries);
    if (n > 0 && (c->cfg.flags & VH_FLAG_CLS_TAIL))
        return fail(&c->err, VH_ERR_UNSUPPORTED, "set_attention_layers: a VH_FLAG_CLS_TAIL context's last layer runs the class-token attention kernel");
    if (!c->ring.empty()) return fail(&c->err, VH_ERR_STATE, "set_attention_layers: a ring exists on this context; vh_ring_destroy first");
    HIPCHK(&c->err, hipSetDevice(c->device));
    HIPCHK(&c->err, hipStreamSynchronize(c->stream));
    const size_t slot = align_up((size_t)c->cfg.max_batch * c->cfg.heads * Q * c->L.T * sizeof(float), 256);
    char* store = nullptr;
    if (n) {
        const hipError_t e = hipMalloc((void**)&store, slot * n);
        if (e != hipSuccess) {
            (void)hipGetLastError();
            return fail(&c->err, VH_ERR_HIP, "set_attention_layers: no room for the store (%d layers x %zu bytes): %s; the previous list stays",
                        n, slot, hipGetErrorString(e));
        }
    }
    drop_graphs(c);
    if (c->attn_store) hipFree(c->attn_store);
    c->attn_store = store;
    c->attn_slot = slot;
    c->attn_n = n;
    c->attn_q = n ? Q : 0;
    c->attn_mode = queries;
    for (int i = 0; i < n; ++i) c->attn_layers[i] = layers[i];
    c->acap_n = 0;
    return VH_OK;
}
int vh_get_attention_layers(const vh_ctx* c, int* layers, int* n, int* queries) {
    if (!c || !n) return fail(nullptr, VH_ERR_INVALID, "get_attention_layers: null argument");
    *n = c->attn_n;
    if (queries) *queries = c->attn_mode;
    for (int i = 0; layers && i < c->attn_n; ++i) layers[i] = c->attn_layers[i];
    return VH_OK;
}
int vh_attention_dims(const vh_ctx* c, int* batch, int* heads, int* queries, int* tokens, int* patches) {
    if (!c) return fail(nullptr, VH_ERR_INVALID, "attention_dims: null context");
    if (batch) *batch = c->last_batch;
    if (heads) *heads = c->cfg.heads;
    if (queries) *queries = c->attn_q;
    if (tokens) *tokens = c->L.T;
    if (patches) *patches = c->L.NP;
    return VH_OK;
}
static int attention_check_call(vh_ctx* c, const vh_attention_maps* f, bool device, const float** slot) {
    if (!c) return fail(nullptr, VH_ERR_INVALID, "read_attention: null context");
    if (!f) return fail(&c->err, VH_ERR_INVALID, "read_attention: null descriptor");
    if (!f->probs && !f->head_mean) return fail(&c->err, VH_ERR_INVALID, "read_attention: no output requested (probs and head_mean are both NULL)");
    if (f->elem != VH_ELEM_F32 && f->elem != VH_ELEM_F16 && f->elem != VH_ELEM_BF16)
        return fail(&c->err, VH_ERR_INVALID, "read_attention: elem %d is not VH_ELEM_F32, VH_ELEM_F16 or VH_ELEM_BF16", f->elem);
    if (f->keys != VH_ATTN_KEYS_ALL && f->keys != VH_ATTN_KEYS_PATCH)
        return fail(&c->err, VH_ERR_INVALID, "read_attention: keys %d is not VH_ATTN_KEYS_ALL (0) or VH_ATTN_KEYS_PATCH (1)", f->keys);
    const int layers = c->cfg.layers;
    if (f->layer != -1 && (f->layer < 1 || f->layer > layers))
        return fail(&c->err, VH_ERR_INVALID, "read_attention: layer %d is not -1 or 1..%d", f->layer, layers);
    if (f->reserved != 0) return fail(&c->err, VH_ERR_INVALID, "read_attention: reserved is %d, not 0", f->reserved);
    if (device && (((uintptr_t)f->probs | (uintptr_t)f->head_mean) & 15))
        return fail(&c->err, VH_ERR_INVALID, "read_attention: a device output pointer is not 16-byte aligned (probs %p, head_mean %p)", f->probs, f->head_mean);
    if (c->cfg.flags & VH_FLAG_CLS_TAIL)
        return fail(&c->err, VH_ERR_UNSUPPORTED, "read_attention: a VH_FLAG_CLS_TAIL context's last layer runs the class-token attention kernel");
    if (!c->ring.empty()) return fail(&c->err, VH_ERR_STATE, "read_attention: a ring exists on this context (its forwards belong to slots); vh_ring_destroy first");
    if (c->last_batch <= 0) return fail(&c->err, VH_ERR_STATE, "read_attention: no forward has run");
    const int layer = f->layer == -1 ? layers : f->layer;
    int at = -1;
    for (int i = 0; i < c->acap_n; ++i) if (c->acap_layers[i] == layer) at = i;
    if (at < 0)
        return fail(&c->err, VH_ERR_STATE, "read_attention: layer %d was not in the list when the last forward was enqueued (vh_set_attention_layers)", layer);
    if (layer > c->acap_nl)
        return fail(&c->err, VH_ERR_STATE, "read_attention: the last forward ran %d layers and did not reach layer %d (vh_debug_set_layers)", c->acap_nl, layer);
    *slot = (const float*)(c->attn_store + (size_t)at * c->attn_slot);
    return VH_OK;
}
static int attention_enqueue(vh_ctx* c, const vh_attention_maps& f, const float* slot) {
    HIPCHK(&c->err, launch_attention_readout(slot, c->last_batch, c->cfg.heads, c->attn_q, c->L.T, c->L.lead, f.elem, f.keys, f.probs, f.head_mean, c->stream));
    return VH_OK;
}
int vh_read_attention_device_async(vh_ctx* c, const vh_attention_maps* f) {
    const float* slot = nullptr;
    if (int rc = attention_check_call(c, f, true, &slot)) return rc;
    HIPCHK(&c->err, hipSetDevice(c->device));
    return attention_enqueue(c, *f, slot);
}
int vh_read_attention_device(vh_ctx* c, const vh_attention_maps* f) {
    if (int rc = vh_read_attention_device_async(c, f)) return rc;
    HIPCHK(&c->err, hipStreamSynchronize(c->stream));
    return VH_OK;
}
int vh_read_attention(vh_ctx* c, const vh_attention_maps* f) {
    const float* slot = nullptr;
    if (int rc = attention_check_call(c, f, false, &slot)) return rc;
    HIPCHK(&c->err, hipSetDevice(c->device));
    const size_t es = f->elem == VH_ELEM_F32 ? 4 : 2, B = c->last_batch, Q = c->attn_q;
    const size_t K = f->keys == VH_ATTN_KEYS_PATCH ? c->L.NP : c->L.T;
    const size_t n_probs = B * c->cfg.heads * Q * K * es, n_mean = B * Q * K * es;
    const size_t cap = ((size_t)c->cfg.max_batch * c->L.T + 256) * 3 * c->cfg.dim * 2;
    vh_attention_maps d = *f;
    size_t at = 0;
    if (f->probs) { d.probs = (char*)c->qkv16 + at; at += align_up(n_probs, 256); }
    if (f->head_mean) { d.head_mean = (char*)c->qkv16 + at; at += align_up(n_mean, 256); }
    if (at > cap) return fail(&c->err, VH_ERR_STATE, "read_attention: staging needs %zu bytes, the scratch holds %zu", at, cap);
    if (int rc = attention_enqueue(c, d, slot)) return rc;
    if (f->probs) HIPCHK(&c->err, hipMemcpyAsync(f->probs, d.probs, n_probs, hipMemcpyDeviceToHost, c->stream));
    if (f->head_mean) HIPCHK(&c->err, hipMemcpyAsync(f->head_mean, d.head_mean, n_mean, hipMemcpyDeviceToHost, c->stream));
    HIPCHK(&c->err, hipStreamSynchronize(c->stream));
    return VH_OK;
}

#define OPCHK(expr) do { hipError_t e_ = (expr); if (e_ != hipSuccess) return fail(nullptr, VH_ERR_HIP, "%s failed: %s", #expr, hipGetErrorString(e_)); } while (0)

constexpr unsigned kEpiPlain8 = 1u << VH_EPI_BIAS | 1u << VH_EPI_BIAS_GELU | 1u << VH_EPI_BIAS_QGELU | 1u << VH_EPI_BIAS_TGELU | 1u << VH_EPI_BIAS_RESID | 1u << VH_EPI_BIAS_F32;
constexpr unsigned kEpiFold8 = 1u << VH_EPI_LNFOLD | 1u << VH_EPI_LNFOLD_GELU | 1u << VH_EPI_LNFOLD_QGELU | 1u << VH_EPI_LNFOLD_TGELU | 1u << VH_EPI_RESID_LN | 1u << VH_EPI_RESID_SPLIT;
static int op_gemm_run(const char* tag, const GemmArgs& g, unsigned offered8, void* stream) {
    const bool f8 = g.dtype == VH_DTYPE_FP8;
    GemmArgs h = g;
    if (f8 && !offered8) h.dtype = -1;
    const bool lacks = f8 && offered8 && (g.epilogue < 0 || g.epilogue > VH_EPI_LNFOLD_TGELU || !(offered8 >> g.epilogue & 1));
    if (lacks) { h.epilogue = VH_EPI_BIAS; h.out_tiled = h.ab_tiled = h.tile_begin = h.tile_count = 0; }
    if (const char* why = gemm_check(h))
        return f8 && offered8 ? fail(nullptr, VH_ERR_INVALID, "%s%s", tag, strchr(why, ':')) : fail(nullptr, VH_ERR_INVALID, "%s", why);
    if (lacks) return fail(nullptr, VH_ERR_UNSUPPORTED, "%s: epilogue %d not available", tag, g.epilogue);
    hipError_t e = launch_gemm(g, (hipStream_t)stream);
    if (e == hipSuccess) e = hipStreamSynchronize((hipStream_t)stream);
    if (e != hipSuccess) return fail(nullptr, e == hipErrorInvalidValue ? VH_ERR_INVALID : VH_ERR_HIP, "%s failed: %s", tag, hipGetErrorString(e));
    return VH_OK;
}
int vh_op_gemm(const void* a, const void* w, const float* bias, void* out, int64_t M, int N, int K, int epi,
               const float* aux, int aux_i, int dtype, int variant, void* stream) {
    const GemmArgs g{a, w, bias, out, M, N, K, epi, aux, aux_i, dtype, variant};
    return op_gemm_run("gemm", g, 0, stream);
}
int vh_op_gemm_ex(const void* a, const void* w, const float* bias, void* out, int64_t M, int N, int K, int epi,
                  const float* aux, int aux_i, const float* stats, void* out16, float* partials, int dtype, int variant,
                  void* stream) {
    GemmArgs g{a, w, bias, out, M, N, K, epi, aux, aux_i, dtype, variant};
    g.stats = stats; g.out16 = out16; g.partials = partials;
    return op_gemm_run("gemm_ex", g, 0, stream);
}
int vh_op_gemm_layout(const void* a, const void* w, const float* bias, void* out, int64_t M, int N, int K, int epi,
                      const float* aux, int aux_i, const float* stats, void* out16, float* partials, int dtype, int variant,
                      int out_tiled, int ab_tiled, int tile_begin, int tile_count, void* stream) {
    GemmArgs g{a, w, bias, out, M, N, K, epi, aux, aux_i, dtype, variant};
    g.stats = stats; g.out16 = out16; g.partials = partials;
    g.out_tiled = out_tiled; g.ab_tiled = ab_tiled; g.tile_begin = tile_begin; g.tile_count = tile_count;
    return op_gemm_run("gemm_layout", g, 0, stream);
}
int vh_op_gemm_lead(const void* a, const void* w, const float* bias, void* out, int64_t M, int N, int K, int epi, const float* aux,
                    int aux_i, int lead, void* out16, float* partials, int64_t prow, int dtype, int variant, void* stream) {
    if (epi != VH_EPI_PATCH && epi != VH_EPI_PATCH_SPLIT) return fail(nullptr, VH_ERR_INVALID, "gemm_lead: epilogue must be VH_EPI_PATCH or VH_EPI_PATCH_SPLIT");
    if (aux_i > 0 && M % aux_i) return fail(nullptr, VH_ERR_INVALID, "gemm_lead: M must be a whole number of images (M %% aux_i == 0)");
    GemmArgs g{a, w, bias, out, M, N, K, epi, aux, aux_i, dtype, variant};
    g.out16 = out16; g.partials = partials; g.prow = prow; g.lead = lead;
    if (epi == VH_EPI_PATCH_SPLIT && aux_i > 0 && prow && prow < (M / aux_i) * (int64_t)(aux_i + lead))
        return fail(nullptr, VH_ERR_INVALID, "gemm_lead: prow is below images x (aux_i + lead)");
    return op_gemm_run("gemm_lead", g, 0, stream);
}
int vh_op_lead_rows(void* x_or_hi, void* lo, float* partials, int64_t prow, const float* cls, const float* pos, const float* reg, int lead,
                    int batch, int tokens, int dim, int dtype, void* stream) {
// ... 1035 lines not shown
```

### vit-fpga_amd/python/vithip.py

```python
from __future__ import annotations

import ctypes as C
import os

import numpy as np

_HERE = os.path.dirname(os.path.abspath(__file__))
PKG_ROOT = os.path.dirname(_HERE)
REPO_ROOT = os.path.dirname(PKG_ROOT)
LIB_PATH = os.environ.get("VITHIP_LIB") or os.path.join(PKG_ROOT, "libvithip.so")

DTYPE_BF16, DTYPE_FP16, DTYPE_FP8 = 0, 1, 2
FLAG_LN_FOLD_OFF, FLAG_LN_FOLD_ON, FLAG_W8_E4M3, FLAG_CLS_TAIL = 1, 2, 4, 8
FLAG_PRE_LN, FLAG_QUICK_GELU = 16, 32
FLAG_REGISTERS_MASK, MAX_REGISTERS = 31 << 9, 16


def FLAG_REGISTERS(n):
    return (int(n) & 31) << 9


def registers_of(flags):
    return (int(flags) & FLAG_REGISTERS_MASK) >> 9

# ... 164 lines not shown
    "vh_forward_frames_yuv16": (_i, [_vp, _vp, _sz, _vp, _i, _vp]),
    "vh_forward_device_frames_yuv16": (_i, [_vp, _vp, _sz, _vp, _i, _vp]),
    "vh_forward_frames_yuy2": (_i, [_vp, _vp, _sz, _vp, _i, _vp]),
    "vh_forward_device_frames_yuy2": (_i, [_vp, _vp, _sz, _vp, _i, _vp]),
    "vh_forward_frames_y210": (_i, [_vp, _vp, _sz, _vp, _i, _vp]),
    "vh_forward_device_frames_y210": (_i, [_vp, _vp, _sz, _vp, _i, _vp]),
    "vh_forward_frames_bgra": (_i, [_vp, _vp, _sz, _vp, _i, _vp]),
    "vh_forward_device_frames_bgra": (_i, [_vp, _vp, _sz, _vp, _i, _vp]),
    "vh_forward_frames_y410": (_i, [_vp, _vp, _sz, _vp, _i, _vp]),
    "vh_forward_device_frames_y410": (_i, [_vp, _vp, _sz, _vp, _i, _vp]),
    "vh_fill_input_seeded": (_i, [_vp, _u64, _i, _vp]),
    "vh_last_forward_us": (_i, [_vp, C.POINTER(_i64)]),
    "vh_last_kernel_ms": (_i, [_vp, C.POINTER(C.c_double)]),
    "vh_profile_forward": (_i, [_vp, _vp, _i, _vp, C.POINTER(C.c_double), _i, _pi]),
    "vh_stage_name": (C.c_char_p, [_i]),
    "vh_filter_create": (_i, [_i, _i, _i, _i, _i, C.POINTER(C.c_void_p)]),
    "vh_filter_destroy": (_i, [_vp]),
    "vh_filter_free_slots": (_i, [_vp, _pi]),
    "vh_filter_submit": (_i, [_vp, _vp]),
    "vh_filter_collect": (_i, [_vp, _vp]),
    "vh_filter_last_error": (C.c_char_p, [_vp]),
    "vh_device_mem_info": (_i, [_i, C.POINTER(C.c_size_t), C.POINTER(C.c_size_t)]),
    "vh_blob_file_config": (_i, [C.c_char_p, C.POINTER(Config)]),
    "vh_blob_file_read": (_i, [C.c_char_p, _vp, _sz]),
    "vh_save_weights_file": (_i, [_vp, C.c_char_p]),
    "vh_load_weights_file": (_i, [_vp, C.c_char_p]),
    "vh_ring_create": (_i, [_vp, _i, _i]),
    "vh_ring_destroy": (_i, [_vp]),
    "vh_ring_free_slots": (_i, [_vp, _pi]),
    "vh_ring_input": (_i, [_vp, C.POINTER(C.POINTER(C.c_float))]),
    "vh_ring_submit": (_i, [_vp, _vp, _i]),
    "vh_ring_collect": (_i, [_vp, _vp, _pi]),
    "vh_ring_create_u8": (_i, [_vp, _i, _i]),
    "vh_ring_input_u8": (_i, [_vp, C.POINTER(C.POINTER(C.c_uint8))]),
    "vh_ring_submit_u8": (_i, [_vp, _vp, _i]),
    "vh_ring_create_tensor": (_i, [_vp, _i, _i, _i, _i]),
    "vh_ring_input_tensor": (_i, [_vp, C.POINTER(_vp), C.POINTER(_sz)]),
    "vh_ring_submit_tensor": (_i, [_vp, _vp, _i]),
    "vh_ring_create_frames": (_i, [_vp, _i, _i, _sz]),
    "vh_ring_input_frames": (_i, [_vp, C.POINTER(C.POINTER(C.c_uint8)), C.POINTER(_sz)]),
    "vh_ring_submit_frames": (_i, [_vp, _vp, _sz, _vp, _i]),
    "vh_ring_submit_frames_nv12": (_i, [_vp, _vp, _sz, _vp, _i]),
    "vh_ring_submit_frames_yuv": (_i, [_vp, _vp, _sz, _vp, _i]),
    "vh_ring_submit_frames_p016": (_i, [_vp, _vp, _sz, _vp, _i]),
    "vh_ring_submit_frames_yuv16": (_i, [_vp, _vp, _sz, _vp, _i]),
    "vh_ring_submit_frames_yuy2": (_i, [_vp, _vp, _sz, _vp, _i]),
    "vh_ring_submit_frames_y210": (_i, [_vp, _vp, _sz, _vp, _i]),
    "vh_ring_submit_frames_bgra": (_i, [_vp, _vp, _sz, _vp, _i]),
    "vh_ring_submit_frames_y410": (_i, [_vp, _vp, _sz, _vp, _i]),
    "vh_set_graph": (_i, [_vp, _i]),
    "vh_get_graph": (_i, [_vp, _pi, _pi]),
    "vh_set_streams": (_i, [_vp, _i]),
    "vh_get_streams": (_i, [_vp, _pi]),
    "vh_set_stage_timing": (_i, [_vp, _i]),
    "vh_get_stage_timing": (_i, [_vp, C.POINTER(C.c_double), C.POINTER(C.c_double), _pi]),
    "vh_set_step_timing": (_i, [_vp, _i]),
    "vh_get_step_timing": (_i, [_vp, C.POINTER(C.c_double), _i, _pi]),
    "vh_debug_read": (_i, [_vp, _i, _vp, _sz]),
    "vh_debug_set_layers": (_i, [_vp, _i]),
    "vh_features_dims": (_i, [_vp, _pi, _pi, _pi, _pi]),
    "vh_read_features": (_i, [_vp, _vp]),
    "vh_read_features_device": (_i, [_vp, _vp]),
    "vh_read_features_device_async": (_i, [_vp, _vp]),
    "vh_set_feature_layers": (_i, [_vp, _pi, _i]),
    "vh_get_feature_layers": (_i, [_vp, _pi, _pi]),
    "vh_read_layer_features": (_i, [_vp, _vp]),
    "vh_read_layer_features_device": (_i, [_vp, _vp]),
    "vh_read_layer_features_device_async": (_i, [_vp, _vp]),
    "vh_set_attention_layers": (_i, [_vp, _pi, _i, _i]),
    "vh_get_attention_layers": (_i, [_vp, _pi, _pi, _pi]),
    "vh_attention_dims": (_i, [_vp, _pi, _pi, _pi, _pi, _pi]),
    "vh_read_attention": (_i, [_vp, _vp]),
    "vh_read_attention_device": (_i, [_vp, _vp]),
    "vh_read_attention_device_async": (_i, [_vp, _vp]),
    "vh_op_gemm": (_i, [_vp, _vp, _vp, _vp, _i64, _i, _i, _i, _vp, _i, _i, _i, _vp]),
    "vh_op_gemm_fp8": (_i, [_vp, _vp, _vp, _vp, _vp, _i64, _i, _i, _i, _i, _vp]),
    "vh_op_gemm_fp8_ex": (_i, [_vp, _vp, _vp, _vp, _vp, _i64, _i, _i, _i, _vp, _vp, _vp, _vp, _i, _vp]),
    "vh_op_quantize_rows": (_i, [_vp, _i, _i, C.c_float, _vp, _vp, _vp]),
    "vh_op_gemm_ex": (_i, [_vp, _vp, _vp, _vp, _i64, _i, _i, _i, _vp, _i, _vp, _vp, _vp, _i, _i, _vp]),
    "vh_op_gemm_layout": (_i, [_vp, _vp, _vp, _vp, _i64, _i, _i, _i, _vp, _i, _vp, _vp, _vp, _i, _i, _i, _i, _i, _i, _vp]),
    "vh_op_gemm_lead": (_i, [_vp, _vp, _vp, _vp, _i64, _i, _i, _i, _vp, _i, _i, _vp, _vp, _i64, _i, _i, _vp]),
    "vh_op_lead_rows": (_i, [_vp, _vp, _vp, _i64, _vp, _vp, _vp, _i, _i, _i, _i, _i, _vp]),
    "vh_op_gemm_fp8_layout": (_i, [_vp, _vp, _vp, _vp, _vp, _i64, _i, _i, _i, _vp, _vp, _vp, _vp, _i, _i, _i, _i, _i, _vp]),
    "vh_op_tile_rows": (_i, [_vp, _i, _i, _vp, _i, _vp]),
    "vh_op_rowstats_cast": (_i, [_vp, _i64, _i, _f, _vp, _vp, _i, _vp]),
    "vh_op_finalize_stats": (_i, [_vp, _i, _i64, _i, _f, _vp, _vp]),
    "vh_op_pre_layernorm": (_i, [_vp, _i64, _i, _vp, _vp, _f, _vp, _vp, _vp, _vp, _i, _vp]),
    "vh_op_rowstats_split": (_i, [_vp, _i64, _i, _f, _vp, _vp, _vp, _i, _vp]),
    "vh_op_fold_ln": (_i, [_vp, _vp, _vp, _vp, _i, _i, _f, _vp, _vp, _vp, _i, _vp]),
    "vh_op_layernorm": (_i, [_vp, _i64, _i, _i64, _vp, _vp, _f, _vp, _i, _vp]),
    "vh_op_rowstats_guard": (_i, [_vp, _i64, _i, _f, _vp, _vp, _vp, _i, _i64, _vp, _vp]),
    "vh_op_pre_layernorm_guard": (_i, [_vp, _i64, _i, _vp, _vp, _f, _vp, _vp, _vp, _vp, _i, _i64, _vp, _vp, _vp]),
    "vh_op_finalize_stats_guard": (_i, [_vp, _i, _i64, _i, _f, _vp, _i64, _vp, _vp, _vp]),
    "vh_op_ln_guard": (_i, [_vp, _i64, _vp, _vp]),
    "vh_op_layernorm_f32": (_i, [_vp, _i64, _i, _i64, _vp, _vp, _f, _vp, _vp]),
    "vh_op_layernorm_split": (_i, [_vp, _vp, _i64, _i, _i64, _vp, _vp, _f, _vp, _i, _vp]),
    "vh_op_head_f32": (_i, [_vp, _vp, _vp, _vp, _i, _i, _i, _vp]),
    "vh_op_fold_ln_f8": (_i, [_vp, _vp, _vp, _vp, _i, _i, _f, _vp, _vp, _vp, _vp, _vp]),
    "vh_op_fake_quant_rows": (_i, [_vp, _i, _i, _vp, _vp]),
    "vh_op_attention": (_i, [_vp, _i, _i, _i, _vp, _i, _vp]),
    "vh_op_attention_stream": (_i, [_vp, _i, _i, _i, _vp, _i, _vp]),
    "vh_op_attention_hd": (_i, [_vp, _i, _i, _i, _i, _vp, _i, _vp]),
    "vh_op_attention_cls": (_i, [_vp, _i, _i, _i, _vp, _i, _vp]),
    "vh_op_attention_layout": (_i, [_vp, _i, _i, _i, _vp, _i, _i, _i64, _vp]),
    "vh_op_attention_probs": (_i, [_vp, _i, _i, _i, _i, _i, _i64, _i, _vp, _vp]),
    "vh_op_attention_readout": (_i, [_vp, _i, _i, _i, _i, _i, _i, _i, _vp, _vp, _vp]),
# ... 1202 lines not shown
        buf, desc = pack_frames_bgra(pixels, layouts, boxes)
        self.ring_submit_frames_bgra_packed(buf, buf.nbytes, desc)

    def ring_submit_frames_bgra_packed(self, buf, nbytes, desc):
        self._ring_submit_frames(lib().vh_ring_submit_frames_bgra, buf, nbytes, desc)

    def ring_submit_frames_y410(self, pixels, layouts=L444_Y410, boxes=None):
        buf, desc = pack_frames_bgra(pixels, layouts, boxes)
        self.ring_submit_frames_y410_packed(buf, buf.nbytes, desc)

    def ring_submit_frames_y410_packed(self, buf, nbytes, desc):
        self._ring_submit_frames(lib().vh_ring_submit_frames_y410, buf, nbytes, desc)

    def ring_free_slots(self):
        n = C.c_int(0)
        _check(lib().vh_ring_free_slots(self.h, C.byref(n)), self.h)
        return n.value

    def ring_input(self, batch):
        p = C.POINTER(C.c_float)()
        _check(lib().vh_ring_input(self.h, C.byref(p)), self.h)
        n = batch * self.cfg["image_size"] ** 2 * self.cfg["channels"]
        return np.ctypeslib.as_array(p, shape=(n,)).reshape(batch, self.cfg["image_size"], self.cfg["image_size"], self.cfg["channels"])

    def ring_submit(self, images=None, batch=None):
        if images is None:
            _check(lib().vh_ring_submit(self.h, None, batch), self.h)
        else:
            images = np.ascontiguousarray(images, dtype=np.float32)
            _check(lib().vh_ring_submit(self.h, images.ctypes.data, images.shape[0]), self.h)

    def ring_collect(self):
        out = np.empty((max(self._ring_batch, 1), self.cfg["classes"]), dtype=np.float32)
        nb = C.c_int(0)
        _check(lib().vh_ring_collect(self.h, out.ctypes.data, C.byref(nb)), self.h)
        return out[:nb.value]

    def set_graph(self, enable=True):
        _check(lib().vh_set_graph(self.h, 1 if enable else 0), self.h)

    def get_graph(self):
        a, b = C.c_int(0), C.c_int(0)
        _check(lib().vh_get_graph(self.h, C.byref(a), C.byref(b)), self.h)
        return bool(a.value), b.value

    def set_streams(self, n):
        _check(lib().vh_set_streams(self.h, n), self.h)

    def get_streams(self):
        n = C.c_int(0)
        _check(lib().vh_get_streams(self.h, C.byref(n)), self.h)
        return n.value

    def set_stage_timing(self, stage_name):
        _check(lib().vh_set_stage_timing(self.h, TIMED_STAGES.index(stage_name) if stage_name else -1), self.h)

    def get_stage_timing(self):
        avg, mn, n = C.c_double(0), C.c_double(0), C.c_int(0)
        _check(lib().vh_get_stage_timing(self.h, C.byref(avg), C.byref(mn), C.byref(n)), self.h)
        return avg.value, mn.value, n.value

    def set_step_timing(self, on):
        _check(lib().vh_set_step_timing(self.h, 1 if on else 0), self.h)

    def get_step_timing(self, max_steps=4096):
        buf = (C.c_double * max_steps)()
        n = C.c_int(0)
        _check(lib().vh_get_step_timing(self.h, buf, max_steps, C.byref(n)), self.h)
        return [buf[i] for i in range(min(n.value, max_steps))]

    def debug_read(self, what, n_floats):
        out = np.empty(n_floats, dtype=np.float32)
        _check(lib().vh_debug_read(self.h, what, out.ctypes.data, n_floats), self.h)
        return out

    def debug_set_layers(self, n):
        _check(lib().vh_debug_set_layers(self.h, n), self.h)

    def register_tokens(self):
        return int(lib().vh_get_register_tokens(self.h))

    def features_dims(self):
        b, t, n, d = C.c_int(0), C.c_int(0), C.c_int(0), C.c_int(0)
        _check(lib().vh_features_dims(self.h, C.byref(b), C.byref(t), C.byref(n), C.byref(d)), self.h)
        return b.value, t.value, n.value, d.value

    def read_features(self, cls=True, patch=True, mean=False, elem=ELEM_F32, norm=FEAT_NORM):
        b, _, n, d = self.features_dims()
        dt = {ELEM_F32: np.float32, ELEM_F16: np.float16, ELEM_BF16: np.uint16}.get(elem, np.float32)
        b1 = max(b, 1)
        out = {}
        if cls:
            out["cls"] = np.empty((b1, d), dtype=dt)
        if patch:
            out["patch"] = np.empty((b1, n, d), dtype=dt)
        if mean:
            out["mean"] = np.empty((b1, d), dtype=dt)
        desc = Features(*(out[k].ctypes.data if k in out else None for k in ("cls", "patch", "mean")), elem, norm)
        _check(lib().vh_read_features(self.h, C.byref(desc)), self.h)
        return out

    def read_features_device(self, desc):
        _check(lib().vh_read_features_device(self.h, C.byref(desc)), self.h)

    def read_features_device_async(self, desc):
        _check(lib().vh_read_features_device_async(self.h, C.byref(desc)), self.h)
# ... 507 lines not shown
```

Baseline: 28340 images/s.

## Run consecutive forward steps on two streams with double-buffered activations

Allocates a second activation arena and alternates consecutive forward steps between the main stream and a new second stream. Each step's final layernorm and head wait on the previous step's head event, so logits writes stay ordered. The goal is to overlap kernel tails and launch gaps between back-to-back batches. The cost is twice the activation memory and possible contention when two large forward passes run concurrently. It is disabled when graphs, multiple streams, timing or feature capture are in use.

```diff
diff --git a/include/vithip.h b/include/vithip.h
--- a/include/vithip.h
+++ b/include/vithip.h
@@ -234,6 +234,7 @@
 
 int vh_set_streams(vh_ctx* ctx, int n);
 int vh_get_streams(const vh_ctx* ctx, int* n);
+int vh_get_inflight(const vh_ctx* ctx, int* n);
 
 int vh_last_forward_us(const vh_ctx* ctx, int64_t* us);
 int vh_last_kernel_ms(vh_ctx* ctx, double* ms);
diff --git a/vit-fpga_amd/csrc/vithip_api.hip b/vit-fpga_amd/csrc/vithip_api.hip
--- a/vit-fpga_amd/csrc/vithip_api.hip
+++ b/vit-fpga_amd/csrc/vithip_api.hip
@@ -200,6 +200,24 @@
     bool operator==(const ImgIn& o) const { return p == o.p && kind == o.kind && layout == o.layout; }
 };
 constexpr int kU8 = VH_ELEM_U8;
+
+struct ActSet {
+    char* base = nullptr;
+    unsigned int* tickets = nullptr;
+    float* x = nullptr;
+    void* xn16 = nullptr;
+    void* xlo16 = nullptr;
+    void* qkv16 = nullptr;
+    void* att16 = nullptr;
+    void* h16 = nullptr;
+    void* col16 = nullptr;
+    float* clsn32 = nullptr;
+    float* pool32 = nullptr;
+    float* stats = nullptr;
+    float* partials = nullptr;
+    float *mapz32 = nullptr, *maph32 = nullptr, *mapa32 = nullptr;
+};
+struct ActSetLayout { size_t x, xn, qkv, att, h, col, cls, pool, st, pt, xlo, tk, mz, mh, ma, bytes; };
 
 struct vh_ctx {
     vh_config cfg;
@@ -229,31 +247,23 @@
     std::vector<float*> sqkv, so, s1, s2;
     bool ln_fold = false;
     float* fold_cd = nullptr;
-    float* stats = nullptr;
-    float* partials = nullptr;
     bool split = false;
     bool cls_tail = false;
     int head_dim = 64;
     float q_scale = kAttnQScale;
-    void* xlo16 = nullptr;
     bool ln_fold_cfg = false, split_cfg = false;
     unsigned int* guard_dev = nullptr;
     float* guard_host = nullptr;
     float guard_thresh = 0.5f;
     bool guard_auto = false, guard_tripped = false;
     char* arena = nullptr;
-    unsigned int* tickets = nullptr;
-    float* x = nullptr;
-    void* xn16 = nullptr;
-    void* qkv16 = nullptr;
-    void* att16 = nullptr;
-    void* h16 = nullptr;
-    void* col16 = nullptr;
-    float* clsn32 = nullptr;
-    float* pool32 = nullptr;
-    float* mapz32 = nullptr;
-    float* maph32 = nullptr;
-    float* mapa32 = nullptr;
+    ActSet act[2];
+    ActSetLayout act_layout{};
+    int last_set = 0;
+    hipStream_t stream2 = nullptr;
+    hipEvent_t ev_fork2 = nullptr, ev_join2 = nullptr, ev_head[2] = {nullptr, nullptr};
+    int inflight_max = 2, ring_flip = 0;
+    bool s2_open = false;
     float* in_dev = nullptr;
     float in_scale[kMaxChannels], in_shift[kMaxChannels];
     float* logits_dev = nullptr;
@@ -425,8 +435,9 @@
 }
 
 void drop_graphs(vh_ctx* c);
+hipError_t sync_compute(vh_ctx* c);
 int guard_reset(vh_ctx* c) {
-    HIPCHK(&c->err, hipStreamSynchronize(c->stream));
+    HIPCHK(&c->err, sync_compute(c));
     HIPCHK(&c->err, hipMemsetAsync(c->guard_dev, 0, 2 * sizeof(unsigned int), c->stream));
     c->guard_host[0] = c->guard_host[1] = 0.f;
     c->guard_tripped = false;
@@ -471,7 +482,9 @@
 }
 
 int enqueue_forward(vh_ctx* c, ImgIn in, int batch, float* logits, std::vector<std::pair<int, hipEvent_t>>* ev,
-                    hipStream_t s, int img0, bool may_pad = true) {
+                    hipStream_t s, int img0, bool may_pad = true, int set = 0, hipEvent_t head_wait = nullptr) {
+    const ActSet& A = c->act[set];
+    c->last_set = set;
     const vh_config& f = c->cfg;
     const Layout& L = c->L;
     const int D = f.dim, M = f.mlp_dim, T = L.T;
@@ -481,20 +494,20 @@
     const float* P = c->params;
     const size_t r0 = (size_t)img0 * T, esz = 2, esz_op = c->fp8 ? 1 : 2;
     const int dt16 = c->dt16;
-    float* const x = c->x + r0 * D;
-    float* const stats_p = c->stats + r0 * 2;
-    float* const partials_p = c->partials + (size_t)(D / 64) * r0 * 2;
-    char* const xn16 = (char*)c->xn16 + r0 * D * esz_op;
-    char* const xlo16 = (char*)c->xlo16 + r0 * D * (c->fp8 ? 2 : 1);
-    char* const qkv16 = (char*)c->qkv16 + r0 * 3 * D * esz;
-    char* const att16 = (char*)c->att16 + r0 * D * esz_op;
-    char* const h16 = (char*)c->h16 + r0 * M * esz_op;
-    char* const col16 = (char*)c->col16 + (size_t)img0 * L.NP * L.KPA * esz;
-    float* const clsn32 = c->clsn32 + (size_t)img0 * L.HW;
-    float* const pool32 = c->pool32 + (size_t)img0 * D;
+    float* const x = A.x + r0 * D;
+    float* const stats_p = A.stats + r0 * 2;
+    float* const partials_p = A.partials + (size_t)(D / 64) * r0 * 2;
+    char* const xn16 = (char*)A.xn16 + r0 * D * esz_op;
+    char* const xlo16 = (char*)A.xlo16 + r0 * D * (c->fp8 ? 2 : 1);
+    char* const qkv16 = (char*)A.qkv16 + r0 * 3 * D * esz;
+    char* const att16 = (char*)A.att16 + r0 * D * esz_op;
+    char* const h16 = (char*)A.h16 + r0 * M * esz_op;
+    char* const col16 = (char*)A.col16 + (size_t)img0 * L.NP * L.KPA * esz;
+    float* const clsn32 = A.clsn32 + (size_t)img0 * L.HW;
+    float* const pool32 = A.pool32 + (size_t)img0 * D;
     const float* const cls_p = L.ncls ? P + L.cls : nullptr;
     const float* const pos_p = P + L.pos - (L.ncls ? 0 : D);
-    unsigned int* const tickets_part = c->tickets + (size_t)img0 * (f.layers > 0 ? f.layers : 1);
+    unsigned int* const tickets_part = A.tickets + (size_t)img0 * (f.layers > 0 ? f.layers : 1);
     if (f.layers > 0) HIPCHK(&c->err, hipMemsetAsync(tickets_part, 0, sizeof(unsigned int) * f.layers, s));
     unsigned int* const amax_guard = c->fp8 ? c->guard_dev + 1 : nullptr;
     auto mark = [&](int stage) -> int {
@@ -663,6 +676,7 @@
             g2.out16 = lc;
             HIPCHK(&c->err, launch_gemm(g2, s));
             if ((rc = mark(ST_FC2))) return rc;
+            if (head_wait) HIPCHK(&c->err, hipStreamWaitEvent(s, head_wait, 0));
             HIPCHK(&c->err, launch_layernorm_split(hc, lc, batch, D, D, P + L.lnfw, P + L.lnfb, f.ln_eps, clsn32, dt16, s));
             if ((rc = mark(ST_LNF))) return rc;
             HIPCHK(&c->err, launch_head_f32(clsn32, P + L.headw, P + L.headb, logits, batch, f.classes, D, s));
@@ -736,12 +750,13 @@
         if ((rc = capture(l))) return rc;
     }
     const bool planes = c->split && nl > 0;
+    if (head_wait) HIPCHK(&c->err, hipStreamWaitEvent(s, head_wait, 0));
     if (L.map) {
         const int H = f.heads, hd = D / H;
-        float* const z = c->mapz32 + (size_t)img0 * H * D;
-        float* const hid = c->maph32 + (size_t)img0 * (M > D ? M : D);
-        float* const a32 = c->mapa32 + (size_t)img0 * D;
-        float* const o32 = c->mapa32 + ((size_t)f.max_batch + img0) * D;
+        float* const z = A.mapz32 + (size_t)img0 * H * D;
+        float* const hid = A.maph32 + (size_t)img0 * (M > D ? M : D);
+        float* const a32 = A.mapa32 + (size_t)img0 * D;
+        float* const o32 = A.mapa32 + ((size_t)f.max_batch + img0) * D;
         float* const lnrow = z;
         const PoolArgs pa{planes ? (const void*)xn16 : (const void*)x, planes ? xlo16 : nullptr, planes ? (c->fp8 ? VH_DTYPE_FP8 : dt16) : VH_FEAT_FORM_F32,
                           batch, T, L.lead, D, P + L.lnfw, P + L.lnfb, f.ln_eps, VH_FEAT_NORM, z};
@@ -775,8 +790,8 @@
     return VH_OK;
 }
 
-int guard_publish(vh_ctx* c) {
-    if (c->ln_fold) HIPCHK(&c->err, hipMemcpyAsync(c->guard_host, c->guard_dev, 2 * sizeof(float), hipMemcpyDeviceToHost, c->stream));
+int guard_publish(vh_ctx* c, hipStream_t s) {
+    if (c->ln_fold) HIPCHK(&c->err, hipMemcpyAsync(c->guard_host, c->guard_dev, 2 * sizeof(float), hipMemcpyDeviceToHost, s));
     return VH_OK;
 }
 constexpr float kE4M3Max = 448.f;
@@ -794,12 +809,13 @@
     c->ln_fold = false;
     c->split = false;
     drop_graphs(c);
+    if (c->stream2) HIPCHK(&c->err, hipStreamSynchronize(c->stream2));
     return prepare_weights(c);
 }
 
-int enqueue_step(vh_ctx* c, ImgIn in, int batch, float* logits) {
+int enqueue_step(vh_ctx* c, ImgIn in, int batch, float* logits, int set = 0, hipEvent_t head_wait = nullptr) {
     const size_t img_elems = (size_t)c->cfg.image_size * c->cfg.image_size * c->cfg.channels;
-    const int parts = batch < c->nstreams ? batch : c->nstreams;
+    const int parts = set ? 1 : batch < c->nstreams ? batch : c->nstreams;
     int rc;
     if (parts > 1) {
         HIPCHK(&c->err, hipEventRecord(c->ev_fork, c->stream));
@@ -817,10 +833,11 @@
             b0 += nb;
         }
         c->last_batch = batch;
-        return guard_publish(c);
-    }
-    if ((rc = enqueue_forward(c, in, batch, logits, nullptr, c->stream, 0))) return rc;
-    return guard_publish(c);
+        return guard_publish(c, c->stream);
+    }
+    hipStream_t const st = set ? c->stream2 : c->stream;
+    if ((rc = enqueue_forward(c, in, batch, logits, nullptr, st, 0, true, set, head_wait))) return rc;
+    return guard_publish(c, st);
 }
 
 void drop_graphs(vh_ctx* c) {
@@ -831,13 +848,14 @@
     c->graphs.clear();
 }
 
-int run_step(vh_ctx* c, ImgIn in, int batch, float* logits) {
+int run_step(vh_ctx* c, ImgIn in, int batch, float* logits, int set = 0, hipEvent_t head_wait = nullptr) {
     if (int rc = guard_poll(c)) return rc;
-    if (!c->use_graph || c->timing_stage >= 0) return enqueue_step(c, in, batch, logits);
+    if (!c->use_graph || c->timing_stage >= 0) return enqueue_step(c, in, batch, logits, set, head_wait);
     for (auto& g : c->graphs)
         if (g.in == in && g.out == logits && g.batch == batch) {
             HIPCHK(&c->err, hipGraphLaunch(g.exec, c->stream));
             c->last_batch = batch;
+            c->last_set = 0;
             return VH_OK;
         }
     bool warm = false;
@@ -871,8 +889,42 @@
     const int rc = enqueue_step(c, ImgIn{c->in_dev}, 1, c->logits_dev);
     c->timing_stage = keep_stage;
     if (rc) return rc;
-    HIPCHK(&c->err, hipStreamSynchronize(c->stream));
+    HIPCHK(&c->err, sync_compute(c));
     return guard_poll(c);
+}
+
+void bind_set(ActSet& a, char* base, const ActSetLayout& o, bool map) {
+    a.x = (float*)(base + o.x); a.xn16 = base + o.xn; a.qkv16 = base + o.qkv; a.att16 = base + o.att; a.h16 = base + o.h;
+    a.col16 = base + o.col; a.clsn32 = (float*)(base + o.cls); a.pool32 = (float*)(base + o.pool);
+    a.stats = (float*)(base + o.st); a.partials = (float*)(base + o.pt); a.xlo16 = base + o.xlo;
+    a.tickets = (unsigned int*)(base + o.tk);
+    if (map) { a.mapz32 = (float*)(base + o.mz); a.maph32 = (float*)(base + o.mh); a.mapa32 = (float*)(base + o.ma); }
+}
+bool second_set(vh_ctx* c) {
+    if (c->act[1].base) return true;
+    if (c->inflight_max < 2) return false;
+    char* p = nullptr;
+    if (hipMalloc((void**)&p, c->act_layout.bytes) != hipSuccess) {
+        (void)hipGetLastError();
+        c->inflight_max = 1;
+        return false;
+    }
+    c->act[1].base = p;
+    bind_set(c->act[1], p, c->act_layout, c->L.map);
+    return true;
+}
+bool two_in_flight_allowed(const vh_ctx* c) {
+    return c->inflight_max == 2 && c->timing_stage < 0 && !c->step_timing && !c->use_graph && c->nstreams == 1 && c->feat_n == 0 &&
+           c->attn_n == 0;
+}
+bool two_in_flight(vh_ctx* c) { return two_in_flight_allowed(c) && second_set(c); }
+hipError_t sync_compute(vh_ctx* c) {
+    if (c->s2_open) {
+        const hipError_t e = hipStreamSynchronize(c->stream2);
+        if (e != hipSuccess) return e;
+        c->s2_open = false;
+    }
+    return hipStreamSynchronize(c->stream);
 }
 
 int check_forward_args(vh_ctx* c, const void* in, int batch, const void* out) {
@@ -989,7 +1041,7 @@
     const vh_config& f = c->cfg;
     if (!c->rz_u8) HIPCHK(&c->err, hipMalloc((void**)&c->rz_u8, (size_t)f.max_batch * f.image_size * f.image_size * f.channels));
     if (plan_words > c->rz_plan_dev_cap) {
-        HIPCHK(&c->err, hipStreamSynchronize(c->stream));
+        HIPCHK(&c->err, sync_compute(c));
         if (c->rz_plan_dev) hipFree(c->rz_plan_dev);
         c->rz_plan_dev = nullptr; c->rz_plan_dev_cap = 0;
         const size_t cap = plan_words * 2 > 16384 ? plan_words * 2 : 16384;
@@ -997,7 +1049,7 @@
         c->rz_plan_dev_cap = cap;
     }
     if (host_too && plan_words > c->rz_plan_host_cap) {
-        HIPCHK(&c->err, hipStreamSynchronize(c->stream));
+        HIPCHK(&c->err, sync_compute(c));
         if (c->rz_plan_host) hipHostFree(c->rz_plan_host);
         c->rz_plan_host = nullptr; c->rz_plan_host_cap = 0;
         const size_t cap = plan_words * 2 > 16384 ? plan_words * 2 : 16384;
@@ -1005,7 +1057,7 @@
         c->rz_plan_host_cap = cap;
     }
     if (frame_bytes > c->rz_frames_cap) {
-        HIPCHK(&c->err, hipStreamSynchronize(c->stream));
+        HIPCHK(&c->err, sync_compute(c));
         if (c->rz_frames) hipFree(c->rz_frames);
         c->rz_frames = nullptr; c->rz_frames_cap = 0;
         const size_t cap = frame_bytes + frame_bytes / 2;
@@ -1054,9 +1106,22 @@
     HIPCHK(&c->err, hipEventRecord(c->ev0, c->stream));
     if ((rc = step_mark())) return rc;
     if (job && (rc = enqueue_resize(c, *job, batch))) return rc;
+    const bool two = steps > 1 && two_in_flight(c);
+    if (two) {
+        c->s2_open = true;
+        HIPCHK(&c->err, hipEventRecord(c->ev_fork2, c->stream));
+        HIPCHK(&c->err, hipStreamWaitEvent(c->stream2, c->ev_fork2, 0));
+    }
     for (int i = 0; i < steps; ++i) {
-        if ((rc = run_step(c, in, batch, logits))) return rc;
+        const int set = two ? i & 1 : 0;
+        if ((rc = run_step(c, in, batch, logits, set, two && i > 0 ? c->ev_head[set ^ 1] : nullptr))) return rc;
+        if (two) HIPCHK(&c->err, hipEventRecord(c->ev_head[set], set ? c->stream2 : c->stream));
         if ((rc = step_mark())) return rc;
+    }
+    if (two) {
+        HIPCHK(&c->err, hipEventRecord(c->ev_join2, c->stream2));
+        HIPCHK(&c->err, hipStreamWaitEvent(c->stream, c->ev_join2, 0));
+        c->s2_open = false;
     }
     HIPCHK(&c->err, hipEventRecord(c->ev1, c->stream));
     c->timed = true;
@@ -1085,12 +1150,12 @@
     rc = forward_device_async(c, staged, batch, c->logits_dev, 1, job);
     if (rc) return rc;
     HIPCHK(&c->err, hipMemcpyAsync(logits_host, c->logits_dev, (size_t)batch * f.classes * 4, hipMemcpyDeviceToHost, c->stream));
-    HIPCHK(&c->err, hipStreamSynchronize(c->stream));
+    HIPCHK(&c->err, sync_compute(c));
     if (c->guard_auto && guard_exceeded(c)) {
         rc = forward_device_async(c, staged, batch, c->logits_dev, 1);
         if (rc) return rc;
         HIPCHK(&c->err, hipMemcpyAsync(logits_host, c->logits_dev, (size_t)batch * f.classes * 4, hipMemcpyDeviceToHost, c->stream));
-        HIPCHK(&c->err, hipStreamSynchronize(c->stream));
+        HIPCHK(&c->err, sync_compute(c));
     }
     c->last_us = std::chrono::duration_cast<std::chrono::microseconds>(std::chrono::high_resolution_clock::now() - t0).count();
     return VH_OK;
@@ -1196,6 +1261,14 @@
         c->nstreams = e ? atoi(e) : 1;
         if (c->nstreams < 1) c->nstreams = 1;
         if (c->nstreams > vh_ctx::kMaxStreams) c->nstreams = vh_ctx::kMaxStreams;
+    }
+    CK(hipStreamCreateWithFlags(&c->stream2, hipStreamNonBlocking));
+    CK(hipEventCreateWithFlags(&c->ev_fork2, hipEventDisableTiming));
+    CK(hipEventCreateWithFlags(&c->ev_join2, hipEventDisableTiming));
+    for (hipEvent_t& e : c->ev_head) CK(hipEventCreateWithFlags(&e, hipEventDisableTiming));
+    {
+        const char* e = getenv("VH_INFLIGHT");
+        c->inflight_max = e && e[0] == '1' && !e[1] ? 1 : 2;
     }
     c->num_cu = prop.multiProcessorCount;
     {
@@ -1272,25 +1345,23 @@
     size_t a = 0;
     auto carve = [&](size_t bytes) { size_t o = a; a += align_up(bytes, 256); return o; };
     const size_t rows_p = rows + 256;
-    const size_t o_x = carve(rows_p * D * 4), o_xn = carve(rows_p * D * 2), o_qkvA = carve(rows_p * 3 * D * 2),
-                 o_att = carve(rows_p * D * 2), o_h = carve(rows_p * M * 2), o_col = carve(B * L.NP * (size_t)L.KPA * 2),
-                 o_cls = carve(B * 2 * D * 4), o_pool = carve(B * D * 4),
-                 o_in = carve(B * (size_t)cfg->image_size * cfg->image_size * cfg->channels * 4), o_lg = carve(B * C * 4),
-                 o_st = carve(rows_p * 2 * 4), o_pt = carve((D / 64 + 1) * rows_p * 2 * 4), o_xlo = carve(rows_p * D * 2),
-                 o_tk = carve(B * 4 * (size_t)(cfg->layers > 0 ? cfg->layers : 1)),
+    ActSetLayout& o = c->act_layout;
+    o.x = carve(rows_p * D * 4); o.xn = carve(rows_p * D * 2); o.qkv = carve(rows_p * 3 * D * 2);
+    o.att = carve(rows_p * D * 2); o.h = carve(rows_p * M * 2); o.col = carve(B * L.NP * (size_t)L.KPA * 2);
+    o.cls = carve(B * 2 * D * 4); o.pool = carve(B * D * 4);
+    o.st = carve(rows_p * 2 * 4); o.pt = carve((D / 64 + 1) * rows_p * 2 * 4);
+    o.xlo = carve(rows_p * D * 2);
+    o.tk = carve(B * 4 * (size_t)(cfg->layers > 0 ? cfg->layers : 1));
+    o.mz = L.map ? carve(B * (size_t)cfg->heads * D * 4) : 0; o.mh = L.map ? carve(B * (M > D ? M : D) * 4) : 0;
+    o.ma = L.map ? carve(B * 2 * D * 4) : 0;
+    o.bytes = a;
+    const size_t o_in = carve(B * (size_t)cfg->image_size * cfg->image_size * cfg->channels * 4), o_lg = carve(B * C * 4),
                  o_gd = carve(256);
-    const size_t o_mz = L.map ? carve(B * (size_t)cfg->heads * D * 4) : 0, o_mh = L.map ? carve(B * (M > D ? M : D) * 4) : 0,
-                 o_ma = L.map ? carve(B * 2 * D * 4) : 0;
     CK(hipMalloc((void**)&c->arena, a));
     c->guard_dev = (unsigned int*)(c->arena + o_gd);
     CK(hipMemsetAsync(c->guard_dev, 0, 256, c->stream));
-    c->x = (float*)(c->arena + o_x); c->xn16 = c->arena + o_xn; c->qkv16 = c->arena + o_qkvA; c->att16 = c->arena + o_att;
-    c->h16 = c->arena + o_h; c->col16 = c->arena + o_col; c->clsn32 = (float*)(c->arena + o_cls);
-    c->pool32 = (float*)(c->arena + o_pool);
+    bind_set(c->act[0], c->arena, o, L.map);
     c->in_dev = (float*)(c->arena + o_in); c->logits_dev = (float*)(c->arena + o_lg);
-    c->stats = (float*)(c->arena + o_st); c->partials = (float*)(c->arena + o_pt); c->xlo16 = c->arena + o_xlo;
-    c->tickets = (unsigned int*)(c->arena + o_tk);
-    if (L.map) { c->mapz32 = (float*)(c->arena + o_mz); c->maph32 = (float*)(c->arena + o_mh); c->mapa32 = (float*)(c->arena + o_ma); }
 #undef CK
     *out = c;
     return VH_OK;
@@ -1300,7 +1371,7 @@
     if (!c) return VH_OK;
     hipSetDevice(c->device);
     vh_ring_destroy(c);
-    if (c->stream) hipStreamSynchronize(c->stream);
+    if (c->stream) sync_compute(c);
     drop_graphs(c);
     if (c->guard_host) hipHostFree(c->guard_host);
     if (c->rz_plan_host) hipHostFree(c->rz_plan_host);
@@ -1308,6 +1379,7 @@
     if (c->rz_frames) hipFree(c->rz_frames);
     if (c->rz_u8) hipFree(c->rz_u8);
     if (c->arena) hipFree(c->arena);
+    if (c->act[1].base) hipFree(c->act[1].base);
     if (c->feat_store) hipFree(c->feat_store);
     if (c->attn_store) hipFree(c->attn_store);
     if (c->w16) hipFree(c->w16);
@@ -1321,6 +1393,10 @@
         if (c->ev_join[i]) hipEventDestroy(c->ev_join[i]);
     }
     if (c->ev_fork) hipEventDestroy(c->ev_fork);
+    if (c->ev_fork2) hipEventDestroy(c->ev_fork2);
+    if (c->ev_join2) hipEventDestroy(c->ev_join2);
+    for (hipEvent_t e : c->ev_head) if (e) hipEventDestroy(e);
+    if (c->stream2) hipStreamDestroy(c->stream2);
     if (c->stream) hipStreamDestroy(c->stream);
     delete c;
     return VH_OK;
@@ -1342,7 +1418,7 @@
 int vh_get_ln_guard(vh_ctx* c, float* max_ratio, float* threshold, int* tripped) {
     if (!c) return fail(nullptr, VH_ERR_INVALID, "null context");
     HIPCHK(&c->err, hipSetDevice(c->device));
-    HIPCHK(&c->err, hipStreamSynchronize(c->stream));
+    HIPCHK(&c->err, sync_compute(c));
     float seen[2] = {0.f, 0.f};
     HIPCHK(&c->err, hipMemcpy(seen, c->guard_dev, sizeof seen, hipMemcpyDeviceToHost));
     if ((!(seen[0] <= c->guard_thresh) || (c->fp8 && !(seen[1] <= kE4M3Max))) && c->ln_fold_cfg) c->guard_tripped = true;
@@ -1355,7 +1431,7 @@
 int vh_get_fp8_guard(vh_ctx* c, float* max_abs, float* limit) {
     if (!c) return fail(nullptr, VH_ERR_INVALID, "null context");
     HIPCHK(&c->err, hipSetDevice(c->device));
-    HIPCHK(&c->err, hipStreamSynchronize(c->stream));
+    HIPCHK(&c->err, sync_compute(c));
     float seen[2] = {0.f, 0.f};
     HIPCHK(&c->err, hipMemcpy(seen, c->guard_dev, sizeof seen, hipMemcpyDeviceToHost));
     if (max_abs) *max_abs = c->fp8 ? seen[1] : 0.f;
@@ -1593,7 +1669,7 @@
 int vh_synchronize(vh_ctx* c) {
     if (!c) return fail(nullptr, VH_ERR_INVALID, "null context");
     HIPCHK(&c->err, hipSetDevice(c->device));
-    HIPCHK(&c->err, hipStreamSynchronize(c->stream));
+    HIPCHK(&c->err, sync_compute(c));
     if (c->weights_ready) return guard_poll(c);
     return VH_OK;
 }
@@ -1763,7 +1839,7 @@
     for (int i = 0; scale && i < ch; ++i)
         if (!std::isfinite(scale[i]) || !std::isfinite(shift[i])) return fail(&c->err, VH_ERR_INVALID, "scale / shift of channel %d is not finite", i);
     HIPCHK(&c->err, hipSetDevice(c->device));
-    HIPCHK(&c->err, hipStreamSynchronize(c->stream));
+    HIPCHK(&c->err, sync_compute(c));
     for (int i = 0; i < kMaxChannels; ++i) {
         c->in_scale[i] = i < ch ? (scale ? scale[i] : 1.0f / 255.0f) : 0.f;
         c->in_shift[i] = i < ch && shift ? shift[i] : 0.f;
@@ -1783,7 +1859,7 @@
     HIPCHK(&c->err, hipSetDevice(c->device));
     const int64_t n = (int64_t)batch * c->cfg.image_size * c->cfg.image_size * c->cfg.channels;
     HIPCHK(&c->err, launch_fill(in_dev, n, seed, TID_IMAGES, 0, 0.f, 0.f, c->stream));
-    HIPCHK(&c->err, hipStreamSynchronize(c->stream));
+    HIPCHK(&c->err, sync_compute(c));
     return VH_OK;
 }
 
@@ -1813,7 +1889,7 @@
     HIPCHK(&c->err, hipSetDevice(c->device));
     std::vector<std::pair<int, hipEvent_t>> ev;
     rc = enqueue_forward(c, ImgIn{in}, batch, logits, &ev, c->stream, 0);
-    if (!rc) { hipError_t e = hipStreamSynchronize(c->stream); if (e != hipSuccess) rc = fail(&c->err, VH_ERR_HIP, "sync: %s", hipGetErrorString(e)); }
+    if (!rc) { hipError_t e = sync_compute(c); if (e != hipSuccess) rc = fail(&c->err, VH_ERR_HIP, "sync: %s", hipGetErrorString(e)); }
     for (int i = 0; i < 2 * kProfiledStages; ++i) stage_ms[i] = 0.0;
     if (!rc)
         for (size_t i = 1; i < ev.size(); ++i) {
@@ -1831,7 +1907,7 @@
     if (!c) return VH_OK;
     if (c->ring.empty() && !c->copy_in) return VH_OK;
     hipSetDevice(c->device);
-    if (c->stream) hipStreamSynchronize(c->stream);
+    if (c->stream) sync_compute(c);
     if (c->copy_in) hipStreamSynchronize(c->copy_in);
     if (c->copy_out) hipStreamSynchronize(c->copy_out);
     for (auto& s : c->ring) {
@@ -1895,6 +1971,8 @@
             return fail(&c->err, VH_ERR_HIP, "vh_ring_create: %s", hipGetErrorString(e));
         }
     }
+    if (!frames && two_in_flight_allowed(c)) second_set(c);
+    c->ring_flip = 0;
     c->ring_batch = batch_per_slot;
     c->ring_kind = kind;
     c->ring_elem = elem;
@@ -1977,14 +2055,18 @@
     s.batch = batch;
     HIPCHK(&c->err, hipMemcpyAsync(s.d_in, s.h_in, in_bytes, hipMemcpyHostToDevice, c->copy_in));
     HIPCHK(&c->err, hipEventRecord(s.in_done, c->copy_in));
-    HIPCHK(&c->err, hipStreamWaitEvent(c->stream, s.in_done, 0));
+    const int set = !frames && two_in_flight(c) ? c->ring_flip : 0;
+    hipStream_t const st = set ? c->stream2 : c->stream;
+    c->ring_flip = set ^ 1;
+    if (set) c->s2_open = true;
+    HIPCHK(&c->err, hipStreamWaitEvent(st, s.in_done, 0));
     if (frames) {
         const FrameJob job{fmt, (const uint8_t*)s.d_in, s.h_plan, c->rz_words.size(), max_tiles};
         if ((rc = enqueue_resize(c, job, batch))) return rc;
     }
-    rc = run_step(c, frames ? ImgIn{c->rz_u8, kU8} : slot_in, batch, s.d_out);
+    rc = run_step(c, frames ? ImgIn{c->rz_u8, kU8} : slot_in, batch, s.d_out, set);
     if (rc) return rc;
-    HIPCHK(&c->err, hipEventRecord(s.fwd_done, c->stream));
+    HIPCHK(&c->err, hipEventRecord(s.fwd_done, st));
     HIPCHK(&c->err, hipStreamWaitEvent(c->copy_out, s.fwd_done, 0));
     HIPCHK(&c->err, hipMemcpyAsync(s.h_out, s.d_out, (size_t)batch * c->cfg.classes * 4, hipMemcpyDeviceToHost, c->copy_out));
     HIPCHK(&c->err, hipEventRecord(s.out_done, c->copy_out));
@@ -2042,7 +2124,7 @@
     if (!c) return fail(nullptr, VH_ERR_INVALID, "null context");
     if (n < 1 || n > vh_ctx::kMaxStreams) return fail(&c->err, VH_ERR_INVALID, "streams must be 1..%d", vh_ctx::kMaxStreams);
     HIPCHK(&c->err, hipSetDevice(c->device));
-    HIPCHK(&c->err, hipStreamSynchronize(c->stream));
+    HIPCHK(&c->err, sync_compute(c));
     c->nstreams = n;
     drop_graphs(c);
     return VH_OK;
@@ -2051,7 +2133,7 @@
 int vh_set_graph(vh_ctx* c, int enable) {
     if (!c) return fail(nullptr, VH_ERR_INVALID, "null context");
     HIPCHK(&c->err, hipSetDevice(c->device));
-    HIPCHK(&c->err, hipStreamSynchronize(c->stream));
+    HIPCHK(&c->err, sync_compute(c));
     c->use_graph = enable != 0;
     if (!c->use_graph) drop_graphs(c);
     return VH_OK;
@@ -2067,6 +2149,12 @@
 int vh_get_streams(const vh_ctx* c, int* n) {
     if (!c || !n) return fail(nullptr, VH_ERR_INVALID, "null argument");
     *n = c->nstreams;
+    return VH_OK;
+}
+
+int vh_get_inflight(const vh_ctx* c, int* n) {
+    if (!c || !n) return fail(nullptr, VH_ERR_INVALID, "null argument");
+    *n = two_in_flight_allowed(c) ? 2 : 1;
     return VH_OK;
 }
 
@@ -2081,7 +2169,7 @@
 int vh_get_stage_timing(vh_ctx* c, double* avg_ms, double* min_ms, int* launches) {
     if (!c || !avg_ms || !launches) return fail(c ? &c->err : nullptr, VH_ERR_INVALID, "null argument");
     HIPCHK(&c->err, hipSetDevice(c->device));
-    HIPCHK(&c->err, hipStreamSynchronize(c->stream));
+    HIPCHK(&c->err, sync_compute(c));
     double sum = 0.0, mn = 1e30;
     int n = 0;
     for (size_t i = 0; i + 1 < c->tev_used; i += 2) {
@@ -2105,7 +2193,7 @@
 int vh_get_step_timing(vh_ctx* c, double* step_ms, int max_steps, int* steps) {
     if (!c || !steps || (max_steps > 0 && !step_ms)) return fail(c ? &c->err : nullptr, VH_ERR_INVALID, "null argument");
     HIPCHK(&c->err, hipSetDevice(c->device));
-    HIPCHK(&c->err, hipStreamSynchronize(c->stream));
+    HIPCHK(&c->err, sync_compute(c));
     int n = 0;
     for (size_t i = 0; i + 1 < c->sev_used; ++i) {
         float t = 0.f;
@@ -2121,7 +2209,7 @@
     if (!c || !host_out) return fail(c ? &c->err : nullptr, VH_ERR_INVALID, "null argument");
     if (c->last_batch <= 0) return fail(&c->err, VH_ERR_STATE, "no forward has run");
     HIPCHK(&c->err, hipSetDevice(c->device));
-    HIPCHK(&c->err, hipStreamSynchronize(c->stream));
+    HIPCHK(&c->err, sync_compute(c));
     const size_t D = c->cfg.dim;
     if (what == 0) {
         const size_t n = (size_t)c->last_batch * c->L.T * D;
@@ -2140,26 +2228,26 @@
             if (c->fp8) {
                 std::vector<uint8_t> hi(n);
                 std::vector<uint16_t> lo(n);
-                HIPCHK(&c->err, hipMemcpy(hi.data(), c->xn16, n, hipMemcpyDeviceToHost));
-                HIPCHK(&c->err, hipMemcpy(lo.data(), c->xlo16, n * 2, hipMemcpyDeviceToHost));
+                HIPCHK(&c->err, hipMemcpy(hi.data(), c->act[c->last_set].xn16, n, hipMemcpyDeviceToHost));
+                HIPCHK(&c->err, hipMemcpy(lo.data(), c->act[c->last_set].xlo16, n * 2, hipMemcpyDeviceToHost));
                 for (size_t i = 0; i < n; ++i) host_out[i] = g(hi[i]) + f(lo[i], VH_DTYPE_BF16);
                 return VH_OK;
             }
             std::vector<uint16_t> hi(n);
             std::vector<uint8_t> lo(n);
-            HIPCHK(&c->err, hipMemcpy(hi.data(), c->xn16, n * 2, hipMemcpyDeviceToHost));
-            HIPCHK(&c->err, hipMemcpy(lo.data(), c->xlo16, n, hipMemcpyDeviceToHost));
+            HIPCHK(&c->err, hipMemcpy(hi.data(), c->act[c->last_set].xn16, n * 2, hipMemcpyDeviceToHost));
+            HIPCHK(&c->err, hipMemcpy(lo.data(), c->act[c->last_set].xlo16, n, hipMemcpyDeviceToHost));
             const float inv = c->dt16 == VH_DTYPE_BF16 ? 1.f / 32.f : 1.f / 256.f;
             for (size_t i = 0; i < n; ++i) host_out[i] = f(hi[i], c->dt16) + g(lo[i]) * inv;
             return VH_OK;
         }
-        HIPCHK(&c->err, hipMemcpy(host_out, c->x, n * 4, hipMemcpyDeviceToHost));
+        HIPCHK(&c->err, hipMemcpy(host_out, c->act[c->last_set].x, n * 4, hipMemcpyDeviceToHost));
         return VH_OK;
     }
     if (what == 1) {
         const size_t n = (size_t)c->last_batch * c->L.HW;
         if (n_floats != n) return fail(&c->err, VH_ERR_INVALID, "expected %zu floats", n);
-        HIPCHK(&c->err, hipMemcpy(host_out, c->clsn32, n * 4, hipMemcpyDeviceToHost));
+        HIPCHK(&c->err, hipMemcpy(host_out, c->act[c->last_set].clsn32, n * 4, hipMemcpyDeviceToHost));
         return VH_OK;
     }
     if (what == 3) {
@@ -2178,7 +2266,7 @@
 int vh_debug_set_layers(vh_ctx* c, int n_layers) {
     if (!c) return fail(nullptr, VH_ERR_INVALID, "null context");
     c->run_layers = n_layers;
-    if (c->stream) hipStreamSynchronize(c->stream);
+    if (c->stream) sync_compute(c);
     drop_graphs(c);
     return VH_OK;
 }
@@ -2204,7 +2292,8 @@
     const vh_config& g = c->cfg;
     const int nl = (c->run_layers < 0 || c->run_layers > g.layers) ? g.layers : c->run_layers;
     const bool planes = c->split && nl > 0;
-    return FeatSource{planes ? (const void*)c->xn16 : (const void*)c->x, planes ? c->xlo16 : nullptr,
+    const ActSet& A = c->act[c->last_set];
+    return FeatSource{planes ? (const void*)A.xn16 : (const void*)A.x, planes ? A.xlo16 : nullptr,
                       planes ? (c->fp8 ? VH_DTYPE_FP8 : c->dt16) : VH_FEAT_FORM_F32, c->L.pool == VH_POOL_CLS};
 }
 static int features_enqueue(vh_ctx* c, const vh_layer_features& f, const FeatSource& src, const char* who) {
@@ -2217,7 +2306,7 @@
     a.elem = f.elem; a.norm = f.norm;
     const bool copy_cls = norm && src.head_cls;
     a.cls = copy_cls ? nullptr : f.cls;
-    a.patch = f.patch; a.mean = f.mean; a.stats = c->stats;
+    a.patch = f.patch; a.mean = f.mean; a.stats = c->act[c->last_set].stats;
     a.reg = f.reg; a.patch_layout = f.patch_layout;
     a.no_cls = c->L.ncls ? 0 : 1;
     if (a.cls || a.patch || a.mean || a.reg) {
@@ -2226,8 +2315,8 @@
     }
     if (copy_cls && f.cls) {
         const int64_t n = (int64_t)c->last_batch * g.dim;
-        if (f.elem == VH_ELEM_F32) HIPCHK(&c->err, hipMemcpyAsync(f.cls, c->clsn32, n * 4, hipMemcpyDeviceToDevice, c->stream));
-        else HIPCHK(&c->err, launch_cast(c->clsn32, f.cls, n, f.elem == VH_ELEM_BF16 ? VH_DTYPE_BF16 : VH_DTYPE_FP16, c->stream));
+        if (f.elem == VH_ELEM_F32) HIPCHK(&c->err, hipMemcpyAsync(f.cls, c->act[c->last_set].clsn32, n * 4, hipMemcpyDeviceToDevice, c->stream));
+        else HIPCHK(&c->err, launch_cast(c->act[c->last_set].clsn32, f.cls, n, f.elem == VH_ELEM_BF16 ? VH_DTYPE_BF16 : VH_DTYPE_FP16, c->stream));
     }
     return VH_OK;
 }
@@ -2235,7 +2324,7 @@
     const size_t es = f.elem == VH_ELEM_F32 ? 4 : 2, D = c->cfg.dim, B = c->last_batch;
     const size_t n_row = B * D * es, n_patch = B * (size_t)c->L.NP * D * es, n_reg = B * (size_t)c->L.R * D * es;
     const size_t cap = ((size_t)c->cfg.max_batch * c->L.T + 256) * 3 * D * 2;
-    char* const base = (char*)c->qkv16;
+    char* const base = (char*)c->act[c->last_set].qkv16;
     size_t at = 0;
     auto take = [&](bool want, size_t bytes) -> void* { if (!want) return nullptr; void* p = base + at; at += align_up(bytes, 256); return p; };
     vh_layer_features d = f;
@@ -2249,7 +2338,7 @@
     if (f.cls) HIPCHK(&c->err, hipMemcpyAsync(f.cls, d.cls, n_row, hipMemcpyDeviceToHost, c->stream));
     if (f.mean) HIPCHK(&c->err, hipMemcpyAsync(f.mean, d.mean, n_row, hipMemcpyDeviceToHost, c->stream));
     if (f.reg) HIPCHK(&c->err, hipMemcpyAsync(f.reg, d.reg, n_reg, hipMemcpyDeviceToHost, c->stream));
-    HIPCHK(&c->err, hipStreamSynchronize(c->stream));
+    HIPCHK(&c->err, sync_compute(c));
     return VH_OK;
 }
 static vh_layer_features features_final(const vh_features& f) {
@@ -2270,7 +2359,7 @@
 }
 int vh_read_features_device(vh_ctx* c, const vh_features* f) {
     if (int rc = vh_read_features_device_async(c, f)) return rc;
-    HIPCHK(&c->err, hipStreamSynchronize(c->stream));
+    HIPCHK(&c->err, sync_compute(c));
     return VH_OK;
 }
 int vh_read_features(vh_ctx* c, const vh_features* f) {
@@ -2293,7 +2382,7 @@
         return fail(&c->err, VH_ERR_UNSUPPORTED, "set_feature_layers: a VH_FLAG_CLS_TAIL context's last layer updates the class-token rows only");
     if (!c->ring.empty()) return fail(&c->err, VH_ERR_STATE, "set_feature_layers: a ring exists on this context; vh_ring_destroy first");
     HIPCHK(&c->err, hipSetDevice(c->device));
-    HIPCHK(&c->err, hipStreamSynchronize(c->stream));
+    HIPCHK(&c->err, sync_compute(c));
     int slots = 0;
     for (int i = 0; i < n; ++i) slots += layers[i] < c->cfg.layers;
     const int eb = c->split_cfg && !c->guard_auto ? 3 : 4;
@@ -2372,7 +2461,7 @@
 }
 int vh_read_layer_features_device(vh_ctx* c, const vh_layer_features* f) {
     if (int rc = vh_read_layer_features_device_async(c, f)) return rc;
-    HIPCHK(&c->err, hipStreamSynchronize(c->stream));
+    HIPCHK(&c->err, sync_compute(c));
     return VH_OK;
 }
 int vh_read_layer_features(vh_ctx* c, const vh_layer_features* f) {
@@ -2405,7 +2494,7 @@
         return fail(&c->err, VH_ERR_UNSUPPORTED, "set_attention_layers: a VH_FLAG_CLS_TAIL context's last layer runs the class-token attention kernel");
     if (!c->ring.empty()) return fail(&c->err, VH_ERR_STATE, "set_attention_layers: a ring exists on this context; vh_ring_destroy first");
     HIPCHK(&c->err, hipSetDevice(c->device));
-    HIPCHK(&c->err, hipStreamSynchronize(c->stream));
+    HIPCHK(&c->err, sync_compute(c));
     const size_t slot = align_up((size_t)c->cfg.max_batch * c->cfg.heads * Q * c->L.T * sizeof(float), 256);
     char* store = nullptr;
     if (n) {
@@ -2483,7 +2572,7 @@
 }
 int vh_read_attention_device(vh_ctx* c, const vh_attention_maps* f) {
     if (int rc = vh_read_attention_device_async(c, f)) return rc;
-    HIPCHK(&c->err, hipStreamSynchronize(c->stream));
+    HIPCHK(&c->err, sync_compute(c));
     return VH_OK;
 }
 int vh_read_attention(vh_ctx* c, const vh_attention_maps* f) {
@@ -2496,13 +2585,13 @@
     const size_t cap = ((size_t)c->cfg.max_batch * c->L.T + 256) * 3 * c->cfg.dim * 2;
     vh_attention_maps d = *f;
     size_t at = 0;
-    if (f->probs) { d.probs = (char*)c->qkv16 + at; at += align_up(n_probs, 256); }
-    if (f->head_mean) { d.head_mean = (char*)c->qkv16 + at; at += align_up(n_mean, 256); }
+    if (f->probs) { d.probs = (char*)c->act[c->last_set].qkv16 + at; at += align_up(n_probs, 256); }
+    if (f->head_mean) { d.head_mean = (char*)c->act[c->last_set].qkv16 + at; at += align_up(n_mean, 256); }
     if (at > cap) return fail(&c->err, VH_ERR_STATE, "read_attention: staging needs %zu bytes, the scratch holds %zu", at, cap);
     if (int rc = attention_enqueue(c, d, slot)) return rc;
     if (f->probs) HIPCHK(&c->err, hipMemcpyAsync(f->probs, d.probs, n_probs, hipMemcpyDeviceToHost, c->stream));
     if (f->head_mean) HIPCHK(&c->err, hipMemcpyAsync(f->head_mean, d.head_mean, n_mean, hipMemcpyDeviceToHost, c->stream));
-    HIPCHK(&c->err, hipStreamSynchronize(c->stream));
+    HIPCHK(&c->err, sync_compute(c));
     return VH_OK;
 }
 
diff --git a/vit-fpga_amd/python/vithip.py b/vit-fpga_amd/python/vithip.py
--- a/vit-fpga_amd/python/vithip.py
+++ b/vit-fpga_amd/python/vithip.py
@@ -240,6 +240,7 @@
     "vh_get_graph": (_i, [_vp, _pi, _pi]),
     "vh_set_streams": (_i, [_vp, _i]),
     "vh_get_streams": (_i, [_vp, _pi]),
+    "vh_get_inflight": (_i, [_vp, _pi]),
     "vh_set_stage_timing": (_i, [_vp, _i]),
     "vh_get_stage_timing": (_i, [_vp, C.POINTER(C.c_double), C.POINTER(C.c_double), _pi]),
     "vh_set_step_timing": (_i, [_vp, _i]),
@@ -1548,6 +1549,11 @@
         _check(lib().vh_get_streams(self.h, C.byref(n)), self.h)
         return n.value
 
+    def get_inflight(self):
+        n = C.c_int(0)
+        _check(lib().vh_get_inflight(self.h, C.byref(n)), self.h)
+        return n.value
+
     def set_stage_timing(self, stage_name):
         _check(lib().vh_set_stage_timing(self.h, TIMED_STAGES.index(stage_name) if stage_name else -1), self.h)
 
```

After: 28890 images/s, median of 6. 1.9% higher.
